# arnold117/PrimeKG-RGCN-LinkPrediction

Hardware: AMD Instinct MI355X
Metric: edges/sec per RGCN layer (fwd+bwd), PrimeKG 30.9k nodes/849k edges/3 rels (higher is better)
Workload: dtype f32; 1 GPU; C2: PrimeKG-shaped synthetic graph, 30926 nodes / 849456 edge columns / 3 relations, encoder 64->128->128, 2 layers fwd+bwd, full graph per step, dropout 0; parallelism=1 GPU, launch=hipGraph replay

## Files before the change

### primekg_rgcn_linkprediction_amd/_lib.py

```python
from __future__ import annotations

import ctypes
import os
from ctypes import c_double, c_float, POINTER, c_char_p, c_int, c_int64, c_size_t, c_void_p

import torch

ABI_VERSION = 38
LIB_NAME = "librgcn_hip.so"
LIB_PATH = os.path.join(os.path.dirname(os.path.abspath(__file__)), LIB_NAME)

RGCN_OK = 0
RGCN_ERR_ARG = -1
RGCN_ERR_RANGE = -2
RGCN_ERR_HIP = -3
RGCN_ERR_UNSUPPORTED = -4
RGCN_ERR_WORKSPACE = -5
RGCN_ERR_ALIGN = -6

_P = c_void_p
_I64 = c_int64

class SlabJob(ctypes.Structure):
    _fields_ = [("slab", c_void_p), ("bias_part", c_void_p), ("splits", ctypes.c_int32), ("K1", ctypes.c_int32),
# ... 126 lines not shown

CLUSTER_PROTOTYPES = {
    "rgcn_kmeans_workspace_bytes": (c_size_t, [_I64, _I64, _I64, _I64]),
    "rgcn_kmeans_assign": (c_int, [_P, _I64, _I64, _P, _I64, _I64,
                                   _P, _P, _P, _P, _P, c_size_t, _P]),
    "rgcn_kmeans_update": (c_int, [_P, _I64, _I64, _P, _I64, _I64,
                                   _P, _P, _P, _P, _P, _P, c_float, _P, c_size_t, _P]),
    "rgcn_kmeans_inertia": (c_int, [_P, _I64, _I64, _P, _I64, _I64, _P, _P, _P, c_size_t, _P]),
    "rgcn_silhouette_workspace_bytes": (c_size_t, [_I64, _I64, _I64, _I64]),
    "rgcn_silhouette_samples": (c_int, [_P, _P, _P, _P, _P, _P, _I64, _I64, _I64, _I64, _I64, _P, _P, _P, c_size_t, _P]),
}

TSNE_PROTOTYPES = {
    "rgcn_knn_refine": (c_int, [_P, _I64, _I64, _P, _I64, _P, _P, _P]),
    "rgcn_tsne_affinities": (c_int, [_P, _I64, _I64, c_double, _P, _P, _P]),
    "rgcn_tsne_workspace_bytes": (c_size_t, [_I64, _I64]),
    "rgcn_tsne_gradient": (c_int, [_P, _I64, _P, _P, _P, _I64, c_float, _I64, c_int,
                                   _P, _P, _P, _P, c_size_t, _P]),
    "rgcn_tsne_update": (c_int, [_P, _I64, c_float, c_float, c_float, _P, _P, _P, _P, _P, c_size_t, _P]),
}

NEIGHBORHOOD_PROTOTYPES = {
    "rgcn_neighborhood_max_nodes": (_I64, []),
    "rgcn_pair_neighborhood": (c_int, [_P, _P, _P, _P, _I64, _I64,
                                       _P, _P, _I64, c_int,
                                       _P, c_int, c_int,
                                       _P, _P, _P, _P, _P, _P, _P, _P]),
}

TRANSE_PROTOTYPES = {
    "rgcn_transe_step_workspace_bytes": (c_size_t, [_I64, _I64, _I64]),
    "rgcn_transe_step": (c_int, [_P, _I64, _P, _I64, _I64,
                                 _P, _P, _P, _I64, c_float, c_float,
                                 _P, _P, _P, _P, c_size_t, _P]),
}

RESAMPLE_PROTOTYPES = {
    "rgcn_resample_weights": (c_int, [_I64, _I64, _I64, _P, _P]),
    "rgcn_resample_curves": (c_int, [_P, _P, _P, _I64, _I64, _I64, _I64, _I64,
                                     _P, _P, _P, _P, _P, _P, _P]),
    "rgcn_resample_ranks": (c_int, [_P, _P, _I64, _P, c_int, _I64, _I64, _I64,
                                    _P, _P, _P, _P, _P]),
}
RESAMPLE_TILE = 1024
RESAMPLE_MAX_SAMPLES = 1 << 28
RESAMPLE_MAX_REPLICATES = 65535
RESAMPLE_MAX_K = 8

COMPLEX_PROTOTYPES = {
    "complex_fwd": (c_int, [_P, _P, _I64, _P, _P, _I64, _P, _P, _I64, _I64, _I64, _P, _P]),
    "complex_bce_fwd": (c_int, [_P, _P, _I64, _P, _P, _I64, _P, _P, _I64, _P, _I64, _I64, _P, _P, _P]),
    "complex_bwd_workspace_bytes": (c_size_t, [_I64, _I64, _I64]),
    "complex_bwd": (c_int, [_P, _P, _P, _I64, _P, _P, _I64, _P, _P, _I64, _I64, _I64, _P, _P, _P, _P, c_size_t, c_int, _P]),
    "complex_bce_bwd": (c_int, [_P, _P, _P, _P, _P, _I64, _P, _P, _I64, _P, _P, _I64, _I64, _I64, _P, _P, _P, _P,
                                c_size_t, c_int, _P]),
    "rgcn_complex_query": (c_int, [c_int, _P, _P, _I64, _P, _P, _I64, _I64, _I64, _P, _P]),
}

SOFTMAX_PROTOTYPES = {
    "rgcn_softmax_workspace_bytes": (c_size_t, [_I64, _I64, _I64, _I64]),
    "rgcn_softmax_lse": (c_int, [_P, _P, _P, _P, _P, _I64, _P, _I64, _I64, _I64, _I64,
                                 _P, _P, _P, _P, _P, _P, c_size_t, _P]),
    "rgcn_softmax_grad": (c_int, [_P, _P, _P, _P, _P, _P, _I64, _P, _P, _I64, _I64, _I64, _I64,
                                  _P, _P, c_int, _P, c_size_t, _P]),
}
SOFTMAX_MAX_D = 256

EDGE_DROPOUT_PROTOTYPES = {
    "rgcn_edge_dropout_create": (c_int, [c_void_p, _P, POINTER(c_void_p)]),
    "rgcn_edge_dropout_destroy": (None, [c_void_p]),
    "rgcn_edge_dropout_graph": (c_void_p, [c_void_p]),
    "rgcn_edge_dropout_kept": (c_void_p, [c_void_p]),
    "rgcn_edge_dropout_kept_export": (c_int, [c_void_p, _P, _P]),
    "rgcn_edge_dropout_draw": (c_int, [c_void_p, c_double, _P, _P, _I64, _P, _P, _P]),
}
EDGE_DROPOUT_STREAM = 0x45444F50

SPARSE_PROTOTYPES = {
    "rgcn_graph_row_mask": (c_void_p, [c_void_p, c_int, POINTER(c_int64)]),
    "rgcn_occupancy_host": (_I64, [_P, _I64, _I64, _P, POINTER(c_int64)]),
}
MODE_SPARSE_ROWS = 2

_lib = None


class RGCNLibraryError(RuntimeError):
    """The HIP library is missing / unloadable / of the wrong ABI."""


def load() -> ctypes.CDLL:
    global _lib
    if _lib is not None:
        return _lib
    if not os.path.exists(LIB_PATH):
        raise RGCNLibraryError(
            f"{LIB_PATH} not found: build it with `python -c 'import __graft_entry__ as g; "
            f"g.build()'` (or `make -C primekg_rgcn_linkprediction_amd/csrc`). There is no "
            f"CPU/PyTorch fallback for the R-GCN path.")
    try:
        lib = ctypes.CDLL(LIB_PATH, mode=ctypes.RTLD_GLOBAL)
    except OSError as exc:
        raise RGCNLibraryError(f"cannot load {LIB_PATH}: {exc}") from exc
    for name, (restype, argtypes) in list(PROTOTYPES.items()) + list(SAMPLING_PROTOTYPES.items()) + list(PATHS_PROTOTYPES.items()) + list(CLUSTER_PROTOTYPES.items()) + list(TSNE_PROTOTYPES.items()) + list(NEIGHBORHOOD_PROTOTYPES.items()) + list(TRANSE_PROTOTYPES.items()) + list(RESAMPLE_PROTOTYPES.items()) + list(COMPLEX_PROTOTYPES.items()) + list(SPARSE_PROTOTYPES.items()) + list(SOFTMAX_PROTOTYPES.items()) + list(EDGE_DROPOUT_PROTOTYPES.items()):
        try:
            fn = getattr(lib, name)
        except AttributeError as exc:
            raise RGCNLibraryError(f"{LIB_PATH} does not export {name}") from exc
        fn.restype = restype
        fn.argtypes = argtypes
    got = lib.rgcn_abi_version()
    if got != ABI_VERSION:
        raise RGCNLibraryError(f"{LIB_PATH} has ABI version {got}, host code expects {ABI_VERSION}")
    _lib = lib
    return lib


def available() -> bool:
    try:
        load()
        return True
    except RGCNLibraryError:
        return False


def strerror(code: int) -> str:
    return load().rgcn_strerror(code).decode()


def check(code: int, what: str) -> None:
    if code == RGCN_OK:
        return
    msg = f"{what}: {strerror(code)} (code {code})"
    if code == RGCN_ERR_RANGE:
        raise IndexError(msg)
    if code in (RGCN_ERR_ARG, RGCN_ERR_UNSUPPORTED):
        raise ValueError(msg)
    if code == RGCN_ERR_ALIGN:
        raise ValueError(f"{what}: a tensor's base address is not aligned: {strerror(code)} (code {code}). Every tensor "
                         f"torch allocates qualifies, and so do row slices of a table whose width is a multiple of 4; a "
                         f"view that starts some elements into a flat buffer does not - pass tensor.clone()")
    raise RuntimeError(msg)
```

### primekg_rgcn_linkprediction_amd/conv.py

```python
from __future__ import annotations

import math
from typing import Optional, Tuple, Union

import torch
import torch.nn as nn
from torch import Tensor

from . import ops


def _glorot(t: Optional[Tensor]) -> None:
    if t is not None:
        bound = math.sqrt(6.0 / (t.size(-2) + t.size(-1)))
        with torch.no_grad():
            t.uniform_(-bound, bound)


def _table(x: Tensor, gather_dtype) -> Tensor:
    if gather_dtype in (None, torch.float32):
        return x
    ops.guard_torch_op("fp16 copy of the feature table")
    return x.to(gather_dtype)


class _BasisCompose(torch.autograd.Function):

    @staticmethod
    def forward(ctx, comp: Tensor, basis: Tensor) -> Tensor:
        comp, basis = comp.contiguous(), basis.contiguous()
        ctx.save_for_backward(comp, basis)
        return ops.basis_compose(comp, basis)

    @staticmethod
    def backward(ctx, gw: Tensor):
        comp, basis = ctx.saved_tensors
        return ops.basis_compose_bwd(gw.contiguous(), comp, basis, ctx.needs_input_grad[0], ctx.needs_input_grad[1])


class _Scales:

    def __init__(self, t: Tensor, slots: int = 2, layers=(), given=None):
        self._own, self._next, self.first = None, 0, None
        self.packed = [None] * len(layers)
        if ops.GEMM_PRECISION == "split":
            if given is not None:
                self.first = given[0]
                if slots > 1:
                    self._own = ops._empty(slots - 1, ops.AMAX_FLOATS, dtype=torch.float32, device=t.device)
                self.packed = ops.split_weights_many(list(layers), amax=list(given[1]), clear=self._own)
                return
            buf = ops._empty(slots, ops.AMAX_FLOATS, dtype=torch.float32, device=t.device)
            self.first, self._own = buf[0], buf[1:slots]
            if layers:
                self.packed = ops.absmax_and_split(t, self.first, self._own, list(layers))
            else:
                ops.absmax(t, self.first, self._own)

    def slot(self) -> Optional[Tensor]:
        if self._own is None:
            return None
        self._next += 1
        return self._own[self._next - 1]


import os as _os
_TRANSFORM_FIRST_RATIO = 2.0


def _fused_backward(graph, g, r, d_in, d_out, g_amax, packed, precision) -> bool:
    fused = _TRAIN_FUSED == "1" or (_TRAIN_FUSED == "auto" and g.size(0) * r * d_out * 4 >= _TRAIN_FUSED_MIN_BYTES)
    return (fused and precision is None and packed is not None and g_amax is not None and not graph.bipartite
            and not graph.edge_dropout
            and ops.GEMM_PRECISION == "split" and ops.fused_bwd_supported(r, d_in, d_out))


def _from_packed(weight: Tensor, packed, precision) -> bool:
    return packed is not None and ops.GEMM_PRECISION == "split" and precision is None and weight.size(2) % 32 == 0


def _transform_first(graph: "ops.BucketedGraph", weight: Tensor, root: Optional[Tensor], packed, precision) -> bool:
    r, d_in, d_out = weight.shape
    ratio = _TRANSFORM_FIRST_RATIO if _from_packed(weight, packed, precision) else max(_TRANSFORM_FIRST_RATIO, 4.0)
    return d_out >= ratio * d_in and root is not None and not graph.bipartite and not graph.edge_dropout


_SPARSE_AGG = True


def _sparse_agg(graph: "ops.BucketedGraph", transposed: bool, half: bool, packed, amax, d: int, precision=None) -> bool:
    return bool(_SPARSE_AGG and not half and packed is not None and amax is not None and ops.GEMM_PRECISION == "split"
                and precision in (None, "half") and d % 64 == 0 and d <= 256 and not graph.bipartite
                and not graph.weighted_shard and graph.num_relations <= 32
                and graph.row_mask_ptr(transposed) is not None)


def _gagg_scale(graph: "ops.BucketedGraph", gagg_amax: Optional[Tensor], g_amax: Optional[Tensor]):
    if gagg_amax is not None:
        return (gagg_amax, g_amax), 1.0
    return (g_amax, g_amax), graph.weight_bound(True)


def _input_grad(graph: "ops.BucketedGraph", g: Tensor, weight: Tensor, root: Optional[Tensor],
                tail: Optional["ops.PendingParamGrads"] = None, g_amax: Optional[Tensor] = None,
                scales: Optional[_Scales] = None, packed: Optional["ops.SplitWeights"] = None,
                precision: Optional[str] = None, t_first: Optional[Tensor] = None, *,
                relu_mask: Optional[Tensor] = None, out_scale: float = 1.0, amax_out: Optional[Tensor] = None,
                lower=None):
    r, d_in, d_out = weight.shape
    extras = relu_mask is not None or amax_out is not None or out_scale != 1.0
    merged = (graph.merged_transposed()
              if not extras and _transform_first(graph, weight, root, packed, precision) else None)
    t = None
    if merged is not None:
        if t_first is None and _from_packed(weight, packed, precision):
            t_first = ops.transform_first(g.contiguous(), packed, g_amax)
        elif t_first is None:
            ops.guard_torch_op("weight concatenation of the transform-first input gradient")
            wcat = torch.cat([weight.reshape(r * d_in, d_out), root]).view(1, (r + 1) * d_in, d_out)
            t_first = ops.transform_bwd_input(g, g, wcat, None, amax=(g_amax, None), precision=precision)
        gx = ops.aggregate(merged, t_first.view(-1, d_in), tail=tail)
    else:
        gagg_amax = scales.slot() if scales is not None else None
        if _fused_backward(graph, g, r, d_in, d_out, g_amax, packed, precision):
            gx = ops.layer_bwd_input_fused(graph, g, packed, relu_mask, g_amax, amax_out=amax_out, tail=tail,
                                           inline_limit=_EVAL_INLINE_LIMIT, out_scale=out_scale, gagg_amax=gagg_amax)
        else:
            sparse = gagg_amax is not None and _sparse_agg(graph, True, False, packed, g_amax, d_out, precision)
            if sparse:
                gagg = ops.aggregate_sparse(graph, g, transposed=True, tail=tail, amax_out=gagg_amax)[0]
            else:
                gagg = ops.aggregate(graph, g, transposed=True, tail=tail, amax_out=gagg_amax)
            amax, mul = _gagg_scale(graph, gagg_amax, g_amax)
            if (lower is not None and packed is not None and g_amax is not None
                    and _from_packed(lower[0], lower[2], precision) and _transform_first(graph, *lower, precision)
                    and ops.chain_supported(weight, lower[0])):
                gx, t = ops.transform_bwd_input_chain(gagg, g, weight, root, relu_mask, packed, lower[2], graph=graph,
                                                      amax=amax, amax_mul=mul, amax_out=amax_out, out_scale=out_scale,
                                                      sparse=sparse)
            else:
                gx = ops.transform_bwd_input(gagg, g, weight, root, relu_mask=relu_mask, graph=graph, amax=amax,
                                             amax_mul=mul, amax_out=amax_out, packed=packed, precision=precision,
                                             out_scale=out_scale, sparse=sparse)
    return (gx, t) if lower is not None else gx


def _backward_scales(g: Tensor, layers: int) -> _Scales:
    return _Scales(g, slots=2 * layers)


def _deferred_params(graph: "ops.BucketedGraph", agg, x, g, x_amax, g_amax, has_root: bool, has_bias: bool, prec,
                     packed=None):
    sparse = _sparse_agg(graph, False, False, packed, x_amax, x.size(1), prec)
    return ops.transform_bwd_params(agg, x, g, graph.num_relations, want_root=has_root, want_bias=has_bias, graph=graph,
                                    defer=True, amax=(x_amax, x_amax, g_amax), precision=prec, sparse=sparse,
                                    amax_mul=_agg_bound(graph))


_TRAIN_FUSED = _os.environ.get("RGCN_TRAIN_FUSED", "auto")
_TRAIN_FUSED_MIN_BYTES = 256 << 20


def _defer_hubs(half: bool, packed, amax, k: int, n_out: int, graph=None) -> bool:
    return (_DEFER_HUBS and not half and packed is not None and amax is not None and ops.GEMM_PRECISION == "split"
            and k in (64, 128) and n_out <= 128 and not (graph is not None and graph.edge_dropout))


_DEFER_HUBS = True


def _agg_bound(graph: "ops.BucketedGraph") -> float:
    return graph.weight_bound(False) if graph.edge_dropout else 1.0


def _train_fused(graph, n, r, d_in, d_out, half) -> bool:
    fused = _TRAIN_FUSED == "1" or (_TRAIN_FUSED == "auto" and n * r * d_in * 4 >= _TRAIN_FUSED_MIN_BYTES)
    return bool(fused and not half and not graph.weighted_shard and n == graph.num_other_nodes
                and ops.GEMM_PRECISION == "split" and ops.fused_supported(r, d_in, d_out))


def _layer_train_forward(graph: "ops.BucketedGraph", x: Tensor, gather_dtype, weight, root, bias, relu: bool,
                         half: bool, x_amax, amax_out, packed):
    n, r, d_in, d_out = x.size(0), graph.num_relations, x.size(1), weight.size(2)
    if (_train_fused(graph, n, r, d_in, d_out, half) and packed is not None and x_amax is not None):
        agg = ops._empty(n, r * d_in, dtype=torch.float32, device=x.device)
        out = ops.layer_fwd_fused(graph, x, packed, bias, relu, x_amax, amax_out, inline_limit=_EVAL_INLINE_LIMIT,
                                  agg_out=agg)
        return agg, out
    sparse = n == graph.num_other_nodes and _sparse_agg(graph, False, half, packed, x_amax, d_in)
    if sparse:
        agg, hubs = ops.aggregate_sparse(graph, x, defer=_defer_hubs(half, packed, x_amax, d_in, d_out, graph))
    elif _defer_hubs(half, packed, x_amax, d_in, d_out, graph):
        agg, hubs = ops.aggregate_deferred(graph, x)
    else:
        agg, hubs = ops.aggregate(graph, _table(x, gather_dtype)), None
    out = ops.transform_fwd(agg, x, weight, root, bias, relu=relu, graph=graph, half=half, amax=(x_amax, x_amax),
                            amax_out=amax_out, packed=packed, hubs=hubs, sparse=sparse, amax_mul=_agg_bound(graph))
    return agg, out


def _packs(bufs, layers):
    return [ops.SplitWeights(b, w, root) if b is not None else None for b, (w, root) in zip(bufs, layers)]


def _conv_forward(x, weight, root, bias, *, graph, relu, gather_dtype, half):
    scales = _Scales(x, slots=1, layers=[(weight, root)])
    x_amax = scales.first
    packed = scales.packed[0]
    agg, out = _layer_train_forward(graph, x, gather_dtype, weight, root, bias, relu, half, x_amax, None,
                                    packed)
    return out, agg, x_amax, (packed.buf if packed is not None else None)


def _conv_backward(x, agg, weight, root, x_amax, pkbuf, g, *, graph, has_root, has_bias, need_x, need_p, prec):
    packed = _packs([pkbuf], [(weight, root)])[0]
    scales = _backward_scales(g, 1)
    pending = (_deferred_params(graph, agg, x, g, x_amax, scales.first, has_root, has_bias, prec, packed)
               if need_p else None)
    gx = _input_grad(graph, g, weight, root, pending, scales.first, scales, packed, prec) if need_x else None
    if pending is None:
        return gx, None, None, None
    pending.finish()
    return (gx, *pending.grads)


_R_CONV_FORWARD = ops.Region("conv.forward", _conv_forward)
_R_CONV_BACKWARD = ops.Region("conv.backward", _conv_backward)


def _contiguous(*tensors):
    return tuple(t.contiguous() if t is not None else None for t in tensors)


def _bwd_precision(gather_dtype, half_backward: bool) -> Optional[str]:
    return "half" if (gather_dtype == torch.float16 and half_backward and ops.GEMM_PRECISION == "split") else None


class _RGCNConvFunction(torch.autograd.Function):

    @staticmethod
    def forward(ctx, x: Tensor, weight: Tensor, root: Optional[Tensor], bias: Optional[Tensor],
                graph: ops.BucketedGraph, relu: bool = False, gather_dtype=None, half_backward: bool = False) -> Tensor:
        x, weight, root, bias = _contiguous(x, weight, root, bias)
        ctx.bwd_precision = _bwd_precision(gather_dtype, half_backward)
        key = (tuple(x.shape), tuple(weight.shape), root is not None, bias is not None, gather_dtype, bool(relu),
               _policy_key())
        out, agg, x_amax, pkbuf = _R_CONV_FORWARD.run(graph, key, (x, weight, root, bias),
                                                      dict(graph=graph, relu=relu, gather_dtype=gather_dtype,
                                                           half=gather_dtype == torch.float16), want={0})
        ctx.graph, ctx.relu, ctx.key = graph, relu, key
        ctx.has_root, ctx.has_bias = root is not None, bias is not None
        ctx.save_for_backward(x, weight, root, out if relu else None)
        ctx.kept = (agg, x_amax, pkbuf)
        return out

    @staticmethod
    def backward(ctx, g: Tensor):
        x, weight, root, out = ctx.saved_tensors
        agg, x_amax, pkbuf = ctx.kept
        if ctx.relu:
            g = g * (out > 0)
        g = g.contiguous()
        need_x, need_w, need_root, need_bias = ctx.needs_input_grad[:4]
        need_p = bool(need_w or (need_root and ctx.has_root) or (need_bias and ctx.has_bias))
        static = dict(graph=ctx.graph, has_root=ctx.has_root, has_bias=ctx.has_bias, need_x=bool(need_x), need_p=need_p,
                      prec=ctx.bwd_precision)
        gx, gw, groot, gbias = _R_CONV_BACKWARD.run(ctx.graph, (ctx.key, bool(need_x), need_p, ctx.bwd_precision),
                                                    (x, agg, weight, root, x_amax, pkbuf, g), static,
                                                    want={0, 1, 2, 3})
        return gx, gw, groot, gbias, None, None, None, None


def _enc2_layer1(x, w1, root1, b1, w2, root2, xa=None, w1a=None, r1a=None, w2a=None, r2a=None, *, graph, gather_dtype, half):
    given = (xa, [(w1a, r1a), (w2a, r2a)]) if xa is not None else None
    scales = _Scales(x, layers=[(w1, root1), (w2, root2)], given=given)
    x_amax, h_amax = scales.first, scales.slot()
    pk1, pk2 = scales.packed
    agg1, h = _layer_train_forward(graph, x, gather_dtype, w1, root1, b1, True, half, x_amax, h_amax, pk1)
    return h, agg1, x_amax, h_amax, (pk1.buf if pk1 is not None else None), (pk2.buf if pk2 is not None else None)


def _enc2_layer2(h, w2, root2, b2, h_amax, pk2buf, *, graph, gather_dtype, half):
    pk2 = _packs([pk2buf], [(w2, root2)])[0]
    agg2, out = _layer_train_forward(graph, h, gather_dtype, w2, root2, b2, False, half, h_amax, None, pk2)
    return out, agg2


def _enc2_forward(x, w1, root1, b1, w2, root2, b2, xa=None, w1a=None, r1a=None, w2a=None, r2a=None, *, graph, gather_dtype,
                  half):
    h, agg1, x_amax, h_amax, pk1buf, pk2buf = _enc2_layer1(x, w1, root1, b1, w2, root2, xa, w1a, r1a, w2a, r2a, graph=graph,
                                                           gather_dtype=gather_dtype, half=half)
    out, agg2 = _enc2_layer2(h, w2, root2, b2, h_amax, pk2buf, graph=graph, gather_dtype=gather_dtype, half=half)
    return out, h, agg1, agg2, x_amax, h_amax, pk1buf, pk2buf


def _enc2_backward(x, agg1, h, agg2, w1, root1, w2, root2, x_amax, h_amax, pk1buf, pk2buf, g, *, graph, flags, p,
                   prec, need_x):
    has_root1, has_b1, has_root2, has_b2 = flags
    pk1, pk2 = _packs([pk1buf, pk2buf], [(w1, root1), (w2, root2)])
    scales = _backward_scales(g, 2)
    g_amax, gz_amax = scales.first, scales.slot()
    red2 = _deferred_params(graph, agg2, h, g, h_amax, g_amax, has_root2, has_b2, prec, pk2)
    gz = _input_grad(graph, g, w2, root2, red2, g_amax, scales, pk2, prec, relu_mask=h,
                     out_scale=1.0 / (1.0 - p) if p > 0 else 1.0, amax_out=gz_amax,
                     lower=(w1, root1, pk1) if need_x else None)
    gz, t_first = gz if need_x else (gz, None)
    red1 = _deferred_params(graph, agg1, x, gz, x_amax, gz_amax, has_root1, has_b1, prec, pk1)
    gx = _input_grad(graph, gz, w1, root1, red1, gz_amax, scales, pk1, prec, t_first) if need_x else None
    red2.finish()
    red1.finish()
    return (gx, *red1.grads, *red2.grads)


_R_LAYER1 = ops.Region("encoder2.layer1", _enc2_layer1)
_R_LAYER2 = ops.Region("encoder2.layer2", _enc2_layer2)
_R_FORWARD = ops.Region("encoder2.forward", _enc2_forward)
_R_BACKWARD = ops.Region("encoder2.backward", _enc2_backward)


def _policy_key():
    return (_TRAIN_FUSED, _DEFER_HUBS, _TRANSFORM_FIRST_RATIO, _EVAL_INLINE_LIMIT, _TRAIN_FUSED_MIN_BYTES, _SPARSE_AGG)


def _enc2_train_forward(graph, params, gather_dtype, half_backward: bool, hints, p: float = 0.0):
    x, w1, root1, b1, w2, root2, b2 = params = _contiguous(*params)
    hinted = hints is not None and ops.GEMM_PRECISION == "split"
    hint_list = list(hints) if hinted else []
    key = (tuple(x.shape), tuple(w1.shape), tuple(w2.shape), root1 is not None, b1 is not None, root2 is not None,
           b2 is not None, gather_dtype, hinted, _policy_key())
    static = dict(graph=graph, gather_dtype=gather_dtype, half=gather_dtype == torch.float16)
    if p > 0:
        h, agg1, x_amax, h_amax, pk1buf, pk2buf = _R_LAYER1.run(graph, key, [x, w1, root1, b1, w2, root2] + hint_list,
                                                                static, want={0, 3})
        h = torch.native_dropout(h, p, True)[0]
        h_amax = ops.materialize(h_amax) * (1.0 / (1.0 - p)) if h_amax is not None else None
        out, agg2 = _R_LAYER2.run(graph, key, (h, w2, root2, b2, h_amax, pk2buf), static, want={0})
    else:
        out, h, agg1, agg2, x_amax, h_amax, pk1buf, pk2buf = _R_FORWARD.run(graph, key, list(params) + hint_list, static,
                                                                            want={0})
    flags = (root1 is not None, b1 is not None, root2 is not None, b2 is not None)
    kept = (agg1, h, agg2, x_amax, h_amax, pk1buf, pk2buf)
    return out, params, (graph, key, flags, p, _bwd_precision(gather_dtype, half_backward), kept)


def _enc2_train_backward(state, inputs, g: Tensor, need_x: bool):
    graph, key, flags, p, prec, (agg1, h, agg2, x_amax, h_amax, pk1buf, pk2buf) = state
    x, w1, root1, w2, root2 = inputs
    return _R_BACKWARD.run(graph, (key, p, need_x, prec),
                           (x, agg1, h, agg2, w1, root1, w2, root2, x_amax, h_amax, pk1buf, pk2buf, g.contiguous()),
                           dict(graph=graph, flags=flags, p=p, prec=prec, need_x=need_x), want={0, 1, 2, 3, 4, 5, 6})


class _Encoder2Function(torch.autograd.Function):

    @staticmethod
    def forward(ctx, x, w1, root1, b1, w2, root2, b2, graph, gather_dtype=None, p: float = 0.0,
                half_backward: bool = False, hints=None):
        out, (x, w1, root1, _, w2, root2, _), ctx.state = _enc2_train_forward(
            graph, (x, w1, root1, b1, w2, root2, b2), gather_dtype, half_backward, hints, p)
        ctx.save_for_backward(x, w1, root1, w2, root2)
        return out

    @staticmethod
    def backward(ctx, g):
        grads = _enc2_train_backward(ctx.state, ctx.saved_tensors, g, bool(ctx.needs_input_grad[0]))
        return (*grads, None, None, None, None, None)


_EVAL_BLOCK_BYTES = 1 << 30


_EVAL_FUSED = _os.environ.get("RGCN_EVAL_FUSED", "auto")


def _eval_fused(n: int, r: int, d_in: int) -> bool:
    if _EVAL_FUSED in (True, "1"):
        return True
    if _EVAL_FUSED in (False, "0"):
        return False
    return n * r * d_in * 4 >= _TRAIN_FUSED_MIN_BYTES
_EVAL_INLINE_LIMIT = 16


def _layer_eval_blocked(graph: "ops.BucketedGraph", x: Tensor, table: Tensor, weight: Tensor, root, bias, relu: bool,
                        half: bool, amax, amax_out, packed) -> Tensor:
    n, r, d_in, d_out = x.size(0), graph.num_relations, x.size(1), weight.size(2)
    if (_eval_fused(n, r, d_in) and not half and packed is not None and amax[1] is not None and not graph.weighted_shard
            and x.size(0) == graph.num_other_nodes and ops.fused_supported(r, d_in, d_out)):
        return ops.layer_fwd_fused(graph, x, packed, bias, relu, amax[1], amax_out, inline_limit=_EVAL_INLINE_LIMIT)
    rows = max(32, _EVAL_BLOCK_BYTES // max(1, r * d_in * 4))
    out = ops._empty(n, d_out, dtype=torch.float32, device=x.device)
    if rows >= n:
        agg = ops.aggregate(graph, table)
        return ops.transform_fwd(agg, x, weight, root, bias, relu=relu, graph=graph, half=half, amax=amax,
                                 amax_out=amax_out, packed=packed, out=out)
    blocks = graph.row_blocks(rows)
    buf = ops._empty(blocks[0][1] - blocks[0][0], r * d_in, dtype=torch.float32, device=x.device)
    for lo, hi, shard in blocks:
        agg = ops.aggregate(shard, table, out=buf[: hi - lo])
        ops.transform_fwd(agg, x[lo:hi], weight, root, bias, relu=relu, graph=shard, half=half, amax=amax,
                          amax_out=amax_out, packed=packed, out=out[lo:hi])
    return out


# ... 203 lines not shown
```

### primekg_rgcn_linkprediction_amd/csrc/rgcn_common.h

```cpp
#pragma once
#include <hip/hip_runtime.h>
#include <stddef.h>
#include <stdint.h>
#include "../../include/rgcn_hip.h"
#include "rgcn_plan.h"

#define RGCN_HIP_TRY(expr)                       \
  do {                                           \
    hipError_t err__ = (expr);                   \
    if (err__ != hipSuccess) return RGCN_ERR_HIP; \
  } while (0)

template <class... P>
static inline bool rgcn_aligned(uintptr_t a, P... p) {
  uintptr_t bits = 0;
  ((bits |= (uintptr_t)(const void*)p), ...);
  return (bits & (a - 1)) == 0;
}
#define RGCN_ALIGN_TRY(a, ...)                                       \
  do {                                                               \
    if (!rgcn_aligned((a), __VA_ARGS__)) return RGCN_ERR_ALIGN;      \
  } while (0)

constexpr int kCUs = 256;

static inline size_t align256(size_t n) { return (n + 255) & ~(size_t)255; }

struct rgcn_slicing {
  int tiles_per_slice, slices;
};
static inline rgcn_slicing rgcn_slice_tiles(int64_t tiles, int64_t want, int64_t cap) {
  const int64_t most = tiles < cap ? tiles : cap;
  want = want < most ? want : most;
  want = want > 1 ? want : 1;
  const int64_t per = (tiles + want - 1) / want;
  return {(int)per, (int)((tiles + per - 1) / per)};
}

template <class K>
static inline int raise_lds(K kernel, int bytes, bool (&raised)[64]) {
  int dev = 0;
  RGCN_HIP_TRY(hipGetDevice(&dev));
  if (dev < 0 || dev >= 64 || !raised[dev]) {
    RGCN_HIP_TRY(hipFuncSetAttribute(reinterpret_cast<const void*>(kernel), hipFuncAttributeMaxDynamicSharedMemorySize, bytes));
    if (dev >= 0 && dev < 64) raised[dev] = true;
  }
  return RGCN_OK;
}

static inline int rgcn_zero_param_grads(float* grad_weight, float* grad_root, float* grad_bias, int64_t R, int64_t d_in,
                                        int64_t d_out, hipStream_t stream) {
  RGCN_HIP_TRY(hipMemsetAsync(grad_weight, 0, (size_t)(R * d_in) * d_out * sizeof(float), stream));
  if (grad_root) RGCN_HIP_TRY(hipMemsetAsync(grad_root, 0, (size_t)d_in * d_out * sizeof(float), stream));
  if (grad_bias) RGCN_HIP_TRY(hipMemsetAsync(grad_bias, 0, (size_t)d_out * sizeof(float), stream));
  return RGCN_OK;
}

constexpr int RGCN_HEAD = 8;

struct rgcn_csr {
  int32_t* rowptr = nullptr;
  int32_t* col = nullptr;
  int64_t* perm = nullptr;
  float* val = nullptr;
  bool weighted = false;
  int64_t n_key = 0;
  int64_t n_other = 0;
  int num_levels = 0;
  int32_t empty_items0 = 0;
  rgcn_item* items[RGCN_MAX_LEVELS] = {};
  int64_t num_items[RGCN_MAX_LEVELS] = {};
  int64_t num_partials = 0;
  int32_t* head_col = nullptr;
  float* head_w = nullptr;
  uint32_t* tile_mask = nullptr;
  int64_t num_row_tiles = 0;
  int32_t* fin_ptr = nullptr;
  int64_t num_fin_tiles = 0;
  float weight_bound = 1.f;
};

static_assert(offsetof(rgcn_csr, items) == offsetof(rgcn_csr, num_levels) + 8, "empty_items0 sits behind num_levels");

constexpr int64_t RGCN_ROW_MASK_PAD = 96;
static inline int64_t rgcn_row_mask_offset(int64_t n_key) { return ((n_key + 31) / 32 + 3) / 4 * 4; }
static inline int64_t rgcn_occupancy_words(int64_t n_key) { return rgcn_row_mask_offset(n_key) + n_key + RGCN_ROW_MASK_PAD; }
static inline void rgcn_fill_occupancy(const int32_t* rowptr, int64_t n_key, int64_t R, uint32_t* words) {
  const int64_t off = rgcn_row_mask_offset(n_key), total = rgcn_occupancy_words(n_key);
  for (int64_t i = 0; i < total; ++i) words[i] = 0u;
  for (int64_t i = 0; i < n_key; ++i) {
    uint32_t m = 0u;
    for (int64_t r = 0; r < R; ++r)
      if (rowptr[i * R + r + 1] > rowptr[i * R + r]) m |= 1u << r;
    words[off + i] = m;
    words[i >> 5] |= m;
  }
}

struct rgcn_graph {
  int64_t E = 0, N = 0, R = 0;
  rgcn_csr dir[2];
};

__attribute__((visibility("hidden"))) int* rgcn_index_error_flag();

constexpr int RGCN_AMAX_SLOTS = 64, RGCN_AMAX_STRIDE = 32;
constexpr int RGCN_AMAX_HEADS = 256, RGCN_AMAX_HEAD_STRIDE = 8;
static_assert(RGCN_AMAX_SLOTS * RGCN_AMAX_STRIDE == RGCN_AMAX_FLOATS, "amax buffer layout (include/rgcn_hip.h)");
static_assert(RGCN_AMAX_HEADS * RGCN_AMAX_HEAD_STRIDE == RGCN_AMAX_FLOATS && RGCN_AMAX_STRIDE % RGCN_AMAX_HEAD_STRIDE == 0,
              "amax buffer layout");

#if defined(__HIPCC__)
__device__ inline int64_t clamp64(int64_t v, int64_t lo, int64_t hi) { return v < lo ? lo : (v > hi ? hi : v); }
__device__ inline int lane_int(int v, int src) { return __builtin_amdgcn_readfirstlane(__shfl(v, src)); }
__device__ inline float lane_float(float v, int src) { return __int_as_float(lane_int(__float_as_int(v), src)); }
__device__ inline int64_t lane_i64(int64_t v, int src) {
  const unsigned lo = (unsigned)lane_int((int)(unsigned)(v & 0xffffffffll), src);
  const int hi = lane_int((int)(v >> 32), src);
  return ((int64_t)hi << 32) | (int64_t)lo;
}
__device__ inline float rgcn_relu(float v) {
  const float r = fmaxf(v, 0.f);
  return v != v ? v : r;
}
extern "C" __device__ unsigned __ockl_wfred_max_u32(unsigned);
__device__ inline unsigned rgcn_amax_peek(const unsigned* __restrict__ amax) {
  return amax ? amax[(blockIdx.x & (RGCN_AMAX_SLOTS - 1)) * RGCN_AMAX_STRIDE] : 0u;
}
__device__ inline void rgcn_amax_publish(unsigned* __restrict__ amax, float lane_max, unsigned seen = 0u) {
  const unsigned m = __ockl_wfred_max_u32(__float_as_uint(fmaxf(lane_max, 0.f)));
  if (m <= seen) return;
  unsigned* slot = amax + (blockIdx.x & (RGCN_AMAX_SLOTS - 1)) * RGCN_AMAX_STRIDE;
  const unsigned long long act = __ballot(1);
  if ((int)(threadIdx.x & 63) == __ffsll((long long)act) - 1) atomicMax(slot, m);
}
__device__ inline float rgcn_amax_value(const float* __restrict__ amax, int lane) {
  float v[RGCN_AMAX_HEADS / 64];
#pragma unroll
  for (int j = 0; j < RGCN_AMAX_HEADS / 64; ++j) v[j] = amax[(lane + 64 * j) * RGCN_AMAX_HEAD_STRIDE];
  float m = v[0];
#pragma unroll
  for (int j = 1; j < RGCN_AMAX_HEADS / 64; ++j) m = fmaxf(m, v[j]);
#pragma unroll
  for (int o = 32; o > 0; o >>= 1) m = fmaxf(m, __shfl_xor(m, o));
  return m;
}
__device__ inline float rgcn_partials_max(const float* __restrict__ p, int count, int lane) {
  float v[4];
#pragma unroll
  for (int j = 0; j < 4; ++j) v[j] = (lane + 64 * j < count) ? p[lane + 64 * j] : 0.f;
  float m = fmaxf(fmaxf(v[0], v[1]), fmaxf(v[2], v[3]));
#pragma unroll
  for (int o = 32; o > 0; o >>= 1) m = fmaxf(m, __shfl_xor(m, o));
  return m;
}
#endif
```

### primekg_rgcn_linkprediction_amd/csrc/rgcn_graph.hip

```cpp
#include <hipcub/hipcub.hpp>

#include <algorithm>
#include <cmath>
#include <new>
#include <vector>

#include "rgcn_common.h"
#include "../../include/rgcn_sparse.h"

namespace {

constexpr int kThreads = 256;

__global__ void k_validate(const int64_t* __restrict__ key_node, const int64_t* __restrict__ other_node,
                           const int64_t* __restrict__ edge_type, int64_t E, int64_t n_key, int64_t n_other,
                           int64_t R, int* __restrict__ flag) {
  int64_t e = (int64_t)blockIdx.x * blockDim.x + threadIdx.x;
  if (e >= E) return;
  int64_t k = key_node[e], o = other_node[e], t = edge_type[e];
  if (k < 0 || k >= n_key || o < 0 || o >= n_other || t < 0 || t >= R) atomicOr(flag, 1);
}

__global__ void k_make_keys(const int64_t* __restrict__ key_node, const int64_t* __restrict__ edge_type,
                            int64_t E, int64_t R, uint32_t* __restrict__ keys, uint32_t* __restrict__ ids) {
  int64_t e = (int64_t)blockIdx.x * blockDim.x + threadIdx.x;
  if (e >= E) return;
  keys[e] = (uint32_t)(key_node[e] * R + edge_type[e]);
  ids[e] = (uint32_t)e;
}

__global__ void k_rowptr(const uint32_t* __restrict__ skeys, int64_t E, int64_t NR,
                         int32_t* __restrict__ rowptr) {
  int64_t e = (int64_t)blockIdx.x * blockDim.x + threadIdx.x;
  if (e > E) return;
  int64_t lo = (e == 0) ? 0 : (int64_t)skeys[e - 1] + 1;
  int64_t hi = (e == E) ? NR : (int64_t)skeys[e];
  for (int64_t k = lo; k <= hi; ++k) rowptr[k] = (int32_t)e;
}

__global__ void k_fill_edges(const int64_t* __restrict__ other_node, int64_t E,
                             const uint32_t* __restrict__ sids, int32_t* __restrict__ col,
                             int64_t* __restrict__ perm) {
  int64_t e = (int64_t)blockIdx.x * blockDim.x + threadIdx.x;
  if (e >= E) return;
  uint32_t p = sids[e];
  perm[e] = (int64_t)p;
  col[e] = (int32_t)other_node[p];
}

__global__ void k_counts(const int32_t* __restrict__ rowptr, int64_t NR, float* __restrict__ cnt) {
  int64_t s = (int64_t)blockIdx.x * blockDim.x + threadIdx.x;
  if (s >= NR) return;
  int deg = rowptr[s + 1] - rowptr[s];
  cnt[s] = (float)(deg < 1 ? 1 : deg);
}

__global__ void k_edge_weights(const uint32_t* __restrict__ skeys_t, const int32_t* __restrict__ col_t,
                               const float* __restrict__ cnt, int64_t E, int64_t R,
                               float* __restrict__ w) {
  int64_t e = (int64_t)blockIdx.x * blockDim.x + threadIdx.x;
  if (e >= E) return;
  int64_t rel = (int64_t)(skeys_t[e] % (uint32_t)R);
  w[e] = 1.0f / cnt[(int64_t)col_t[e] * R + rel];
}

__global__ void k_permute_weights(const float* __restrict__ w_in, const int64_t* __restrict__ perm, int64_t E,
                                  float* __restrict__ w) {
  int64_t e = (int64_t)blockIdx.x * blockDim.x + threadIdx.x;
  if (e < E) w[e] = w_in[perm[e]];
}

inline unsigned grid_for(int64_t n) { return (unsigned)std::max<int64_t>(1, ceil_div64(n, kThreads)); }

int build_plan(const std::vector<int32_t>& rowptr, int64_t NR, int64_t R, rgcn_csr* csr) {
  rgcn_plan plan;
  const int rc = rgcn_build_plan(rowptr, NR, R, csr->n_key, &plan);
  if (rc != RGCN_OK) return rc;
  std::vector<std::vector<rgcn_item>>& levels = plan.levels;
  const std::vector<int32_t>& fin_ptr = plan.fin_ptr;
  const int64_t partial_rows = plan.num_partials;

  csr->num_levels = (int)levels.size();
  csr->num_partials = partial_rows;
  csr->empty_items0 = 0;
  if (!levels.empty()) {
    const std::vector<rgcn_item>& v0 = levels[0];
    size_t live = v0.size();
    while (live > 0 && !(v0[live - 1].flags & RGCN_ITEM_PACK) && v0[live - 1].begin == v0[live - 1].end) --live;
    csr->empty_items0 = (int32_t)(v0.size() - live);
  }
  for (int l = 0; l < csr->num_levels; ++l) {
    auto& v = levels[l];
    csr->num_items[l] = (int64_t)v.size();
    if (v.empty()) continue;
    RGCN_HIP_TRY(hipMalloc((void**)&csr->items[l], v.size() * sizeof(rgcn_item)));
    RGCN_HIP_TRY(hipMemcpy(csr->items[l], v.data(), v.size() * sizeof(rgcn_item), hipMemcpyHostToDevice));
  }
  if (!fin_ptr.empty()) {
    RGCN_HIP_TRY(hipMalloc((void**)&csr->fin_ptr, fin_ptr.size() * sizeof(int32_t)));
    RGCN_HIP_TRY(hipMemcpy(csr->fin_ptr, fin_ptr.data(), fin_ptr.size() * sizeof(int32_t), hipMemcpyHostToDevice));
    csr->num_fin_tiles = (int64_t)fin_ptr.size() - 1;
  }
  return RGCN_OK;
}

void free_csr(rgcn_csr* c) {
  (void)hipFree(c->rowptr);
  (void)hipFree(c->col);
  (void)hipFree(c->perm);
  (void)hipFree(c->val);
  (void)hipFree(c->tile_mask);
  (void)hipFree(c->fin_ptr);
  (void)hipFree(c->head_col);
  (void)hipFree(c->head_w);
  for (int l = 0; l < RGCN_MAX_LEVELS; ++l) (void)hipFree(c->items[l]);
  *c = rgcn_csr();
}

struct Scratch {
  uint32_t *keys = nullptr, *ids = nullptr, *skeys[2] = {nullptr, nullptr}, *sids = nullptr;
  void* sort_tmp = nullptr;
  size_t sort_tmp_bytes = 0;
  int* flag = nullptr;
  int alloc(int64_t E) {
    RGCN_HIP_TRY(hipMalloc((void**)&flag, sizeof(int)));
    if (E <= 0) return RGCN_OK;
    RGCN_HIP_TRY(hipMalloc((void**)&keys, E * sizeof(uint32_t)));
    RGCN_HIP_TRY(hipMalloc((void**)&ids, E * sizeof(uint32_t)));
    RGCN_HIP_TRY(hipMalloc((void**)&skeys[0], E * sizeof(uint32_t)));
    RGCN_HIP_TRY(hipMalloc((void**)&skeys[1], E * sizeof(uint32_t)));
    RGCN_HIP_TRY(hipMalloc((void**)&sids, E * sizeof(uint32_t)));
    return RGCN_OK;
  }
  ~Scratch() {
    (void)hipFree(keys); (void)hipFree(ids); (void)hipFree(skeys[0]); (void)hipFree(skeys[1]);
    (void)hipFree(sids); (void)hipFree(sort_tmp); (void)hipFree(flag);
  }
};

int validate(const int64_t* key_node, const int64_t* other_node, const int64_t* edge_type, int64_t E, int64_t n_key,
             int64_t n_other, int64_t R, Scratch& sc, hipStream_t stream) {
  if (E <= 0) return RGCN_OK;
  RGCN_HIP_TRY(hipMemsetAsync(sc.flag, 0, sizeof(int), stream));
  k_validate<<<grid_for(E), kThreads, 0, stream>>>(key_node, other_node, edge_type, E, n_key, n_other, R, sc.flag);
  int host_flag = 0;
  RGCN_HIP_TRY(hipMemcpyAsync(&host_flag, sc.flag, sizeof(int), hipMemcpyDeviceToHost, stream));
  RGCN_HIP_TRY(hipStreamSynchronize(stream));
  return host_flag ? RGCN_ERR_RANGE : RGCN_OK;
}

int build_structure(const int64_t* key_node, const int64_t* other_node, const int64_t* edge_type, int64_t E,
                    int64_t n_key, int64_t n_other, int64_t R, int slot, Scratch& sc, hipStream_t stream,
                    rgcn_csr* c) {
  const int64_t NR = n_key * R;
  c->n_key = n_key;
  c->n_other = n_other;
  RGCN_HIP_TRY(hipMalloc((void**)&c->rowptr, (NR + 1) * sizeof(int32_t)));
  if (E <= 0) {
    RGCN_HIP_TRY(hipMemsetAsync(c->rowptr, 0, (NR + 1) * sizeof(int32_t), stream));
    return RGCN_OK;
  }
  int end_bit = 1;
  while (end_bit < 32 && ((int64_t)1 << end_bit) < NR) ++end_bit;
  RGCN_HIP_TRY(hipMalloc((void**)&c->col, E * sizeof(int32_t)));
  RGCN_HIP_TRY(hipMalloc((void**)&c->perm, E * sizeof(int64_t)));
  k_make_keys<<<grid_for(E), kThreads, 0, stream>>>(key_node, edge_type, E, R, sc.keys, sc.ids);
  size_t tmp_bytes = 0;
  RGCN_HIP_TRY(hipcub::DeviceRadixSort::SortPairs(nullptr, tmp_bytes, sc.keys, sc.skeys[slot], sc.ids, sc.sids,
                                                   (int)E, 0, end_bit, stream));
  if (tmp_bytes > sc.sort_tmp_bytes) {
    RGCN_HIP_TRY(hipStreamSynchronize(stream));
    (void)hipFree(sc.sort_tmp);
    sc.sort_tmp = nullptr;
    RGCN_HIP_TRY(hipMalloc(&sc.sort_tmp, tmp_bytes + 256));
    sc.sort_tmp_bytes = tmp_bytes;
  }
  RGCN_HIP_TRY(hipcub::DeviceRadixSort::SortPairs(sc.sort_tmp, tmp_bytes, sc.keys, sc.skeys[slot], sc.ids, sc.sids,
                                                   (int)E, 0, end_bit, stream));
  k_rowptr<<<grid_for(E + 1), kThreads, 0, stream>>>(sc.skeys[slot], E, NR, c->rowptr);
  k_fill_edges<<<grid_for(E), kThreads, 0, stream>>>(other_node, E, sc.sids, c->col, c->perm);
  return RGCN_OK;
}

#define TRY_PLAN(expr) do { int rc__ = (expr); if (rc__ != RGCN_OK) return rc__; } while (0)

__global__ void k_item_heads(const rgcn_item* __restrict__ items, int64_t nitems, const int32_t* __restrict__ col,
                             const float* __restrict__ w, int32_t* __restrict__ head_col,
                             float* __restrict__ head_w) {
  const int64_t i = (int64_t)blockIdx.x * blockDim.x + threadIdx.x;
  if (i >= nitems * RGCN_HEAD) return;
  const rgcn_item it = items[i / RGCN_HEAD];
  const int e = it.begin + (int)(i % RGCN_HEAD);
  const bool ok = e < it.end;
  head_col[i] = ok ? col[e] : -1;
  if (head_w) head_w[i] = ok ? w[e] : 0.f;
}

int plan_structure(rgcn_csr* c, int64_t R, hipStream_t stream) {
  const int64_t NR = c->n_key * R;
  std::vector<int32_t> rp((size_t)NR + 1);
  RGCN_HIP_TRY(hipMemcpyAsync(rp.data(), c->rowptr, (NR + 1) * sizeof(int32_t), hipMemcpyDeviceToHost, stream));
  RGCN_HIP_TRY(hipStreamSynchronize(stream));
  if (R <= 32 && c->n_key > 0) {
    c->num_row_tiles = ceil_div64(c->n_key, 32);
    std::vector<uint32_t> mask((size_t)rgcn_occupancy_words(c->n_key));
    rgcn_fill_occupancy(rp.data(), c->n_key, R, mask.data());
    RGCN_HIP_TRY(hipMalloc((void**)&c->tile_mask, mask.size() * sizeof(uint32_t)));
    RGCN_HIP_TRY(hipMemcpy(c->tile_mask, mask.data(), mask.size() * sizeof(uint32_t), hipMemcpyHostToDevice));
  }
  TRY_PLAN(build_plan(rp, NR, R, c));
  c->weight_bound = 1.f;
  if (c->weighted && NR > 0 && rp[(size_t)NR] > 0) {
    std::vector<float> w((size_t)rp[(size_t)NR]);
    RGCN_HIP_TRY(hipMemcpyAsync(w.data(), c->val, w.size() * sizeof(float), hipMemcpyDeviceToHost, stream));
    RGCN_HIP_TRY(hipStreamSynchronize(stream));
    double best = 0.0;
    for (int64_t s = 0; s < NR; ++s) {
      double sum = 0.0;
      for (int32_t e = rp[(size_t)s]; e < rp[(size_t)s + 1]; ++e) sum += std::fabs((double)w[(size_t)e]);
      best = std::max(best, sum);
    }
    c->weight_bound = (float)(best * (1.0 + 1e-6)) + 1e-30f;
  }
  const int64_t n0 = c->num_items[0];
  if (n0 > 0) {
    RGCN_HIP_TRY(hipMalloc((void**)&c->head_col, (size_t)n0 * RGCN_HEAD * sizeof(int32_t)));
    if (c->weighted) RGCN_HIP_TRY(hipMalloc((void**)&c->head_w, (size_t)n0 * RGCN_HEAD * sizeof(float)));
    k_item_heads<<<grid_for(n0 * RGCN_HEAD), kThreads, 0, stream>>>(c->items[0], n0, c->col,
                                                                   c->weighted ? c->val : nullptr, c->head_col,
                                                                   c->head_w);
    RGCN_HIP_TRY(hipGetLastError());
  }
  return RGCN_OK;
}

int mean_counts(rgcn_csr* c, int64_t R, hipStream_t stream) {
  const int64_t NR = c->n_key * R;
  RGCN_HIP_TRY(hipMalloc((void**)&c->val, std::max<int64_t>(NR, 1) * sizeof(float)));
  if (NR > 0) k_counts<<<grid_for(NR), kThreads, 0, stream>>>(c->rowptr, NR, c->val);
  c->weighted = false;
  return RGCN_OK;
}

#define TRY_RC(expr) do { int rc__ = (expr); if (rc__ != RGCN_OK) return rc__; } while (0)

int create_impl(const int64_t* edge_index, const int64_t* edge_type, int64_t E, int64_t N, int64_t R,
                hipStream_t stream, rgcn_graph* g) {
  g->E = E; g->N = N; g->R = R;
  const int64_t* src = edge_index;
  const int64_t* dst = edge_index + E;
  Scratch sc;
  TRY_RC(sc.alloc(E));
  TRY_RC(validate(dst, src, edge_type, E, N, N, R, sc, stream));
  TRY_RC(build_structure(dst, src, edge_type, E, N, N, R, 0, sc, stream, &g->dir[0]));
  TRY_RC(build_structure(src, dst, edge_type, E, N, N, R, 1, sc, stream, &g->dir[1]));
  TRY_RC(mean_counts(&g->dir[0], R, stream));
  g->dir[1].weighted = true;
  if (E > 0) {
    RGCN_HIP_TRY(hipMalloc((void**)&g->dir[1].val, E * sizeof(float)));
    k_edge_weights<<<grid_for(E), kThreads, 0, stream>>>(sc.skeys[1], g->dir[1].col, g->dir[0].val, E, R,
                                                         g->dir[1].val);
  }
  RGCN_HIP_TRY(hipGetLastError());
  TRY_RC(plan_structure(&g->dir[0], R, stream));
  TRY_RC(plan_structure(&g->dir[1], R, stream));
  RGCN_HIP_TRY(hipStreamSynchronize(stream));
  return RGCN_OK;
}

int create_bipartite_impl(const int64_t* key_node, const int64_t* other_node, const int64_t* edge_type, int64_t E,
                          int64_t n_key, int64_t n_other, int64_t R, const float* edge_weight, hipStream_t stream,
                          rgcn_graph* g) {
  g->E = E; g->N = n_key; g->R = R;
  Scratch sc;
  TRY_RC(sc.alloc(E));
  TRY_RC(validate(key_node, other_node, edge_type, E, n_key, n_other, R, sc, stream));
  rgcn_csr* c = &g->dir[0];
  TRY_RC(build_structure(key_node, other_node, edge_type, E, n_key, n_other, R, 0, sc, stream, c));
  if (edge_weight) {
    c->weighted = true;
    if (E > 0) {
      RGCN_HIP_TRY(hipMalloc((void**)&c->val, E * sizeof(float)));
      k_permute_weights<<<grid_for(E), kThreads, 0, stream>>>(edge_weight, c->perm, E, c->val);
    }
  } else {
    TRY_RC(mean_counts(c, R, stream));
  }
  RGCN_HIP_TRY(hipGetLastError());
  TRY_RC(plan_structure(c, R, stream));
  RGCN_HIP_TRY(hipStreamSynchronize(stream));
  return RGCN_OK;
}

// ... 106 lines not shown
}

int rgcn_graph_import(int64_t num_edges, int64_t num_nodes, int64_t num_relations, const int32_t* rowptr,
                      const int32_t* col, const int64_t* perm, const float* cnt, const int32_t* rowptr_t,
                      const int32_t* col_t, const int64_t* perm_t, const float* w_t, void* stream_,
                      rgcn_graph** out) {
  if (!out) return RGCN_ERR_ARG;
  *out = nullptr;
  if (num_edges < 0 || num_nodes < 0 || num_relations <= 0 || !rowptr || !rowptr_t) return RGCN_ERR_ARG;
  if (num_nodes * num_relations > 0 && !cnt) return RGCN_ERR_ARG;
  if (num_edges > 0 && (!col || !perm || !col_t || !perm_t || !w_t)) return RGCN_ERR_ARG;
  if (too_big(num_nodes, num_nodes, num_relations, num_edges)) return RGCN_ERR_UNSUPPORTED;
  RGCN_ALIGN_TRY(8, perm, perm_t);
  RGCN_ALIGN_TRY(4, rowptr, col, cnt, rowptr_t, col_t, w_t);
  hipStream_t stream = (hipStream_t)stream_;
  rgcn_graph* g = new (std::nothrow) rgcn_graph();
  if (!g) return RGCN_ERR_HIP;
  g->E = num_edges; g->N = num_nodes; g->R = num_relations;
  int* flag = nullptr;
  int rc = hipMalloc((void**)&flag, sizeof(int)) == hipSuccess ? RGCN_OK : RGCN_ERR_HIP;
  if (rc == RGCN_OK)
    rc = import_csr(rowptr, col, perm, cnt, false, num_edges, num_nodes, num_relations, flag, stream, &g->dir[0]);
  if (rc == RGCN_OK)
    rc = import_csr(rowptr_t, col_t, perm_t, w_t, true, num_edges, num_nodes, num_relations, flag, stream,
                    &g->dir[1]);
  if (rc == RGCN_OK && hipStreamSynchronize(stream) != hipSuccess) rc = RGCN_ERR_HIP;
  (void)hipFree(flag);
  if (rc != RGCN_OK) {
    rgcn_graph_destroy(g);
    return rc;
  }
  *out = g;
  return RGCN_OK;
}

void rgcn_graph_destroy(rgcn_graph* g) {
  if (!g) return;
  free_csr(&g->dir[0]);
  free_csr(&g->dir[1]);
  delete g;
}

int64_t rgcn_graph_num_edges(const rgcn_graph* g) { return g ? g->E : -1; }
int64_t rgcn_graph_num_nodes(const rgcn_graph* g) { return g ? g->N : -1; }
int64_t rgcn_graph_num_relations(const rgcn_graph* g) { return g ? g->R : -1; }
float rgcn_graph_weight_bound(const rgcn_graph* g, int transposed) {
  if (!g) return 0.f;
  const rgcn_csr* c = &g->dir[transposed ? 1 : 0];
  return c->rowptr ? c->weight_bound : 0.f;
}

int rgcn_graph_num_levels(const rgcn_graph* g, int transposed) {
  return g ? g->dir[transposed ? 1 : 0].num_levels : -1;
}

const uint32_t* rgcn_graph_tile_mask(const rgcn_graph* g, int transposed, int64_t* num_row_tiles) {
  if (!g) return nullptr;
  const rgcn_csr* c = &g->dir[transposed ? 1 : 0];
  if (num_row_tiles) *num_row_tiles = c->num_row_tiles;
  return c->tile_mask;
}

const uint32_t* rgcn_graph_row_mask(const rgcn_graph* g, int transposed, int64_t* num_rows) {
  if (num_rows) *num_rows = 0;
  if (!g) return nullptr;
  const rgcn_csr* c = &g->dir[transposed ? 1 : 0];
  if (!c->tile_mask) return nullptr;
  if (num_rows) *num_rows = c->n_key;
  return c->tile_mask + rgcn_row_mask_offset(c->n_key);
}

int64_t rgcn_occupancy_host(const int32_t* rowptr, int64_t num_rows, int64_t num_relations, uint32_t* words,
                            int64_t* row_offset) {
  if (num_rows < 0 || num_relations <= 0) return -1;
  if (row_offset) *row_offset = rgcn_row_mask_offset(num_rows);
  if (num_relations > 32) return 0;
  if (words) {
    if (!rowptr) return -1;
    rgcn_fill_occupancy(rowptr, num_rows, num_relations, words);
  }
  return rgcn_occupancy_words(num_rows);
}

int rgcn_graph_arrays(const rgcn_graph* g, int transposed, const int32_t** rowptr, const int32_t** col,
                      const int64_t** perm, const float** val) {
  if (!g) return RGCN_ERR_ARG;
  const rgcn_csr* c = &g->dir[transposed ? 1 : 0];
  if (rowptr) *rowptr = c->rowptr;
  if (col) *col = c->col;
  if (perm) *perm = c->perm;
  if (val) *val = c->val;
  return RGCN_OK;
}

int rgcn_graph_export(const rgcn_graph* g, int transposed, int32_t* rowptr, int32_t* col, int64_t* perm,
                      float* val, void* stream_) {
  if (!g) return RGCN_ERR_ARG;
  hipStream_t stream = (hipStream_t)stream_;
  const rgcn_csr* c = &g->dir[transposed ? 1 : 0];
  if (!c->rowptr) return RGCN_ERR_ARG;
  RGCN_ALIGN_TRY(8, perm);
  RGCN_ALIGN_TRY(4, rowptr, col, val);
  const size_t nr = (size_t)(c->n_key * g->R), e = (size_t)g->E;
  if (rowptr) RGCN_HIP_TRY(hipMemcpyAsync(rowptr, c->rowptr, (nr + 1) * sizeof(int32_t), hipMemcpyDeviceToDevice, stream));
  if (col && e) RGCN_HIP_TRY(hipMemcpyAsync(col, c->col, e * sizeof(int32_t), hipMemcpyDeviceToDevice, stream));
  if (perm && e) RGCN_HIP_TRY(hipMemcpyAsync(perm, c->perm, e * sizeof(int64_t), hipMemcpyDeviceToDevice, stream));
  const size_t nval = c->weighted ? e : nr;
  if (val && nval) RGCN_HIP_TRY(hipMemcpyAsync(val, c->val, nval * sizeof(float), hipMemcpyDeviceToDevice, stream));
  return RGCN_OK;
}

}
```

### primekg_rgcn_linkprediction_amd/csrc/rgcn_transform_split.hip

```cpp
#include <algorithm>
#include <cstdlib>
#include <type_traits>

#include <hip/hip_fp16.h>

#include "rgcn_common.h"
#include "rgcn_slab_reduce.h"
#include "rgcn_hub_finish.h"
#include "rgcn_split.h"
#include "rgcn_transform_host.h"

#ifdef RGCN_STAMPS
__device__ unsigned long long g_rgcn_stamps[8192 * 4];
#define RGCN_STAMP(i)                                                                                               \
  do {                                                                                                              \
    if (threadIdx.x == 0) g_rgcn_stamps[((blockIdx.y * gridDim.x + blockIdx.x) & 8191) * 4 + (i)] = __builtin_amdgcn_s_memrealtime(); \
  } while (0)
#else
#define RGCN_STAMP(i)
#endif

#include "rgcn_prep.h"


namespace {

typedef float float2v __attribute__((ext_vector_type(2)));
typedef _Float16 half2v __attribute__((ext_vector_type(2)));

constexpr int kThreads = 256;
constexpr int BK = 32;
constexpr int kMaxSlots = 256;

enum { EPI_NONE = 0, EPI_RELU = 1, EPI_MASK = 2 };
enum { B_KN = 0, B_BLK = 1 };

__device__ inline void glds16(const void* src, void* lds_wave_base) {
  __builtin_amdgcn_global_load_lds((const __attribute__((address_space(1))) void*)src,
                                   (__attribute__((address_space(3))) void*)lds_wave_base, 16, 0, 0);
}

constexpr int kAbsmaxSegs = 4;
struct absmax_job {
  const float* p[kAbsmaxSegs];
  int64_t n[kAbsmaxSegs];
};

__global__ __launch_bounds__(kThreads) void k_absmax(const absmax_job J, float* __restrict__ slots) {
  __shared__ float red[kThreads / 64];
  for (int seg = 0; seg < kAbsmaxSegs; ++seg) {
    float m = 0.f;
    const float* p = J.p[seg];
    if (!p) continue;
    const int64_t n = J.n[seg], n4 = n >> 2;
    const float4* p4 = reinterpret_cast<const float4*>(p);
    for (int64_t i = (int64_t)blockIdx.x * kThreads + threadIdx.x; i < n4; i += (int64_t)gridDim.x * kThreads) {
      const float4 v = p4[i];
      m = fmaxf(fmaxf(m, fmaxf(fabsf(v.x), fabsf(v.y))), fmaxf(fabsf(v.z), fabsf(v.w)));
    }
    if (blockIdx.x == 0 && threadIdx.x < (n & 3)) m = fmaxf(m, fabsf(p[n4 * 4 + threadIdx.x]));
#pragma unroll
    for (int o = 32; o > 0; o >>= 1) m = fmaxf(m, __shfl_xor(m, o));
    if ((threadIdx.x & 63) == 0) red[threadIdx.x >> 6] = m;
    __syncthreads();
    if (threadIdx.x == 0) slots[seg * kMaxSlots + blockIdx.x] = fmaxf(fmaxf(red[0], red[1]), fmaxf(red[2], red[3]));
    __syncthreads();
  }
}

struct amax_ref {
  const float* slots;
  int count;
};
__device__ inline float amax_of(const amax_ref& r, int lane) {
  return r.count == 0 ? rgcn_amax_value(r.slots, lane) : rgcn_partials_max(r.slots, r.count, lane);
}
struct amax_loads {
  float v[4];
};
__device__ inline amax_loads amax_request(const amax_ref& r, int lane) {
  amax_loads q;
  const int stride = r.count == 0 ? RGCN_AMAX_HEAD_STRIDE : 1, last = r.count == 0 ? RGCN_AMAX_HEADS - 1 : r.count - 1;
#pragma unroll
  for (int j = 0; j < 4; ++j) {
    const float* p = r.slots + min(lane + 64 * j, last) * stride;
    asm volatile("global_load_dword %0, %1, off" : "=v"(q.v[j]) : "v"(p) : "memory");
  }
  return q;
}
#define RGCN_AMAX_WAIT(a, b, c, younger)                                                                             \
  asm volatile("s_waitcnt vmcnt(%12)"                                                                                 \
               : "+v"(a.v[0]), "+v"(a.v[1]), "+v"(a.v[2]), "+v"(a.v[3]), "+v"(b.v[0]), "+v"(b.v[1]), "+v"(b.v[2]),     \
                 "+v"(b.v[3]), "+v"(c.v[0]), "+v"(c.v[1]), "+v"(c.v[2]), "+v"(c.v[3])                                  \
               : "n"(younger)                                                                                         \
               : "memory")
#define RGCN_AMAX_WAIT2(a, b, younger)                                                                                \
  asm volatile("s_waitcnt vmcnt(%8)"                                                                                  \
               : "+v"(a.v[0]), "+v"(a.v[1]), "+v"(a.v[2]), "+v"(a.v[3]), "+v"(b.v[0]), "+v"(b.v[1]), "+v"(b.v[2]),     \
                 "+v"(b.v[3])                                                                                         \
               : "n"(younger)                                                                                         \
               : "memory")
__device__ inline float amax_reduce(const amax_loads& q) {
  float m = fmaxf(fmaxf(q.v[0], q.v[1]), fmaxf(q.v[2], q.v[3]));
#pragma unroll
  for (int o = 32; o > 0; o >>= 1) m = fmaxf(m, __shfl_xor(m, o));
  return m;
}

#ifndef RGCN_PACK_THREADS
#define RGCN_PACK_THREADS 512
#endif
#ifndef RGCN_PACK_TILES
#define RGCN_PACK_TILES 1
#endif
#ifndef RGCN_SPLIT_THREADS
#define RGCN_SPLIT_THREADS 256
#endif
#ifndef RGCN_SCAN_THREADS
#define RGCN_SCAN_THREADS 1024
#endif
constexpr int kPackThreads = RGCN_PACK_THREADS, kSplitThreads = RGCN_SPLIT_THREADS, kScanThreads = RGCN_SCAN_THREADS;
constexpr int kPackTiles = RGCN_PACK_TILES;
constexpr int kPackJobs = RGCN_PACK_JOBS, kZeroMax = RGCN_PREP_ZERO_MAX;
constexpr int kPackCapScan = 64, kPackCapGiven = 256;
using pack_job = rgcn_pack_job;
using pack_jobs = rgcn_pack_jobs;

template <int THREADS, bool SCAN, int TILES>
__global__ __launch_bounds__(THREADS) void k_pack_split(const pack_jobs JJ, float* __restrict__ zero, int zero_count) {
  __shared__ __attribute__((aligned(16))) unsigned char lds[rgcn_pack_lds_bytes<TILES>()];
  if (blockIdx.y == 0)
    for (int z = (int)threadIdx.x; z < zero_count; z += THREADS)
      for (int h = (int)blockIdx.x; h < RGCN_AMAX_HEADS; h += (int)gridDim.x)
        zero[(size_t)z * RGCN_AMAX_FLOATS + h * RGCN_AMAX_HEAD_STRIDE] = 0.f;
  rgcn_pack_body<THREADS, SCAN, TILES>(JJ.j[blockIdx.y], lds, (int)blockIdx.x);
}

struct hub_fin {
  const int32_t* ptr;
  const rgcn_item* items;
  const float* cnt;
  float* partial;
  int d, tiles;
};

struct nt_chain {
  const __half* Ch;
  const __half* Cl;
  const float* c_inv_scale;
  float* T;
  int N2;
};

__device__ __attribute__((aligned(16))) float g_zero_row[128];

template <int WM, int WN, int TN, int EPI, bool LO, bool CHAIN = false>
__global__ __launch_bounds__(64 * WM * WN) void k_gemm_nt_split(const float* __restrict__ A1, int K1,
                                                            const float* __restrict__ A2, int K2,
                                                            const __half* __restrict__ Bh,
                                                            const __half* __restrict__ Bl,
                                                            const float* __restrict__ b_inv_scale,
                                                            amax_ref amax1, float a1_mul, amax_ref amax2,
                                                            const float* __restrict__ bias,
                                                            const float* __restrict__ mask, float* __restrict__ C,
                                                            int M, int N, const uint32_t* __restrict__ tile_mask,
                                                            int kseg, unsigned* __restrict__ amax_out,
                                                            const hub_fin fin, float out_scale, const nt_chain chain,
                                                            const uint32_t* __restrict__ row_mask) {
  static_assert(!CHAIN || (WM == 2 && WN == 2 && TN == 2 && LO), "the chained product is built for the 64 x 128 tile");
  constexpr int WAVES = WM * WN;
  constexpr int BM = 32 * WM, BN = 32 * TN * WN, NBUF = WM == 2 ? 3 : 4, D = NBUF - 1;
  constexpr int PARTS = LO ? 2 : 1;
  constexpr int A_BYTES = BM * BK * 4, B_BYTES = BN * BK * 2, BUF_BYTES = A_BYTES + PARTS * B_BYTES;
  constexpr int A_PW = BM / (8 * WAVES);
  constexpr int B_PW = BN / (16 * WAVES);
  constexpr int P = A_PW + PARTS * B_PW;
  static_assert(A_PW >= 1 && B_PW >= 1 && A_PW * 8 * WAVES == BM && B_PW * 16 * WAVES == BN, "tile / wave layout");
  __shared__ __attribute__((aligned(16))) char lds[NBUF * BUF_BYTES];

  const int K = K1 + K2;
  const int m0 = blockIdx.x * BM, n0 = blockIdx.y * BN;
  const int tid = threadIdx.x, lane = tid & 63;
  const int wave = __builtin_amdgcn_readfirstlane(tid >> 6);
  const int wm = wave / WN, wn = wave % WN;
  const int li = lane & 31, lh = lane >> 5;
  RGCN_STAMP(0);
  amax_loads q1 = amax_request(amax1, lane), q2 = amax_request(amax2.slots ? amax2 : amax1, lane);
  const unsigned seen = rgcn_amax_peek(amax_out);
  unsigned rel_mask = 0xffffffffu;
  if (tile_mask) {
    const int t32 = m0 >> 5;
    rel_mask = 0u;
#pragma unroll
    for (int q = 0; q < WM; ++q)
      if ((t32 + q) * 32 < M) rel_mask |= tile_mask[t32 + q];
    rel_mask = __builtin_amdgcn_readfirstlane(rel_mask);
  }
  int a_m[A_PW], a_c4[A_PW];
  unsigned a_rm[A_PW];
#pragma unroll
  for (int j = 0; j < A_PW; ++j) {
    const int row = (wave * A_PW + j) * 8 + (lane >> 3);
    a_m[j] = min(m0 + row, M - 1);
    a_c4[j] = ((lane & 7) ^ ((row >> 1) & 7)) * 4;
    a_rm[j] = row_mask ? row_mask[a_m[j]] : 0xffffffffu;
  }
  const float* a_zero = g_zero_row + (lane & 7) * 4;
  int fin_b = 0, fin_e = 0;
  if (WAVES == 4 && fin.ptr) {
    fin_b = fin.ptr[min(m0 >> 5, fin.tiles)];
    fin_e = fin.ptr[min((m0 >> 5) + WM, fin.tiles)];
  }
  RGCN_AMAX_WAIT2(q1, q2, 0);
  const float amax1_v = amax_reduce(q1) * a1_mul;
  const float amax2_v = amax2.slots ? amax_reduce(q2) : 0.f;

  if (WAVES == 4 && fin.ptr) {
    const int jb = __builtin_amdgcn_readfirstlane(fin_b), je = __builtin_amdgcn_readfirstlane(fin_e);
    if (je > jb) {
      float4* red = reinterpret_cast<float4*>(lds);
      float* agg = const_cast<float*>(A1);
      for (int j = jb; j < je; ++j) {
        float4* scratch = red + ((j - jb) & 1) * 256;
        const rgcn_item it = fin.items[j];
        if (fin.d == 64) rgcn_reduce_item<16>(it, fin.cnt, agg, fin.partial, 64, 0, scratch);
        else if (fin.d == 128) rgcn_reduce_item<32>(it, fin.cnt, agg, fin.partial, 128, 0, scratch);
        else rgcn_reduce_item<64>(it, fin.cnt, agg, fin.partial, 256, 0, scratch);
      }
      __threadfence_block();
      asm volatile("s_waitcnt vmcnt(0)" ::: "memory");
      __syncthreads();
    }
  }

  floatx16 acc[TN];
#pragma unroll
  for (int b = 0; b < TN; ++b)
#pragma unroll
    for (int r = 0; r < 16; ++r) acc[b][r] = 0.f;

  size_t b_off[B_PW];
#pragma unroll
  for (int j = 0; j < B_PW; ++j) {
    const int row = (wave * B_PW + j) * 16 + (lane >> 2);
    const int n = min(n0 + row, N - 1);
    const int chunk = (lane & 3) ^ ((row >> 1) & 3);
    b_off[j] = (size_t)n * K + chunk * 8;
  }

  auto stage = [&](int kt, int buf) {
    char* sA = lds + buf * BUF_BYTES;
    char* sBh = sA + A_BYTES;
    char* sBl = sBh + B_BYTES;
    const bool first = kt < K1;
    const float* abase = first ? A1 + kt : A2 + (kt - K1);
    const int lda = first ? K1 : K2;
    const bool masked = first && row_mask != nullptr;
    const unsigned rbit = masked ? 1u << (kt / kseg) : 0u;
#pragma unroll
    for (int j = 0; j < A_PW; ++j)
      glds16((!masked || (a_rm[j] & rbit)) ? abase + ((size_t)a_m[j] * lda + a_c4[j]) : a_zero, sA + (wave * A_PW + j) * 8 * BK * 4);
#pragma unroll
    for (int j = 0; j < B_PW; ++j) {
      glds16(Bh + kt + b_off[j], sBh + (wave * B_PW + j) * 16 * BK * 2);
      if (LO) glds16(Bl + kt + b_off[j], sBl + (wave * B_PW + j) * 16 * BK * 2);
    }
  };

  auto next_kt = [&](int kt) {
    kt += BK;
    while (kt < K1 && !((rel_mask >> (kt / kseg)) & 1u)) kt = (kt / kseg + 1) * kseg;
    return min(kt, K);
  };
  int ktq[D];
  ktq[0] = next_kt(-BK);
#pragma unroll
  for (int j = 1; j < D; ++j) ktq[j] = ktq[j - 1] < K ? next_kt(ktq[j - 1]) : K;
#pragma unroll
  for (int j = 0; j < D; ++j)
    if (ktq[j] < K) stage(ktq[j], j);

  const int ea1 = scale_exponent(amax1_v);
  const int ea2 = amax2.slots ? scale_exponent(amax2_v) : ea1;
  const float sa1 = pow2f(ea1), sa2 = pow2f(ea2);

  const int arow = wm * 32 + li;
  unsigned a_addr[2][2], b_addr[TN][2];
#pragma unroll
// ... 19 lines not shown
#pragma unroll
    for (int s = 0; s < 2; ++s) {
      asm volatile("ds_read_b128 %0, %1" : "=v"(fa[s][0]) : "v"(a_addr[s][0] + buf));
      asm volatile("ds_read_b128 %0, %1" : "=v"(fa[s][1]) : "v"(a_addr[s][1] + buf));
#pragma unroll
      for (int b = 0; b < TN; ++b) {
        asm volatile("ds_read_b128 %0, %1" : "=v"(fh[s][b]) : "v"(b_addr[b][s] + buf));
        if (LO) asm volatile("ds_read_b128 %0, %1 offset:%2" : "=v"(fl[s][b]) : "v"(b_addr[b][s] + buf), "n"(B_BYTES));
      }
    }
    const int kt_new = ktq[D - 1] < K ? next_kt(ktq[D - 1]) : K;
    if (kt_new < K) stage(kt_new, (t + D) % NBUF);
#pragma unroll
    for (int j = 0; j + 1 < D; ++j) ktq[j] = ktq[j + 1];
    ktq[D - 1] = kt_new;
    ++t;
#pragma unroll
    for (int s = 0; s < 2; ++s) {
      constexpr int kStepReads = 2 + PARTS * TN;
      if constexpr (TN == 4) {
        if (s == 0) asm volatile("s_waitcnt lgkmcnt(%6)" : "+v"(fa[0][0]), "+v"(fa[0][1]), "+v"(fh[0][0]), "+v"(fh[0][1]), "+v"(fh[0][2]), "+v"(fh[0][3]) : "n"(kStepReads));
        else asm volatile("s_waitcnt lgkmcnt(0)" : "+v"(fa[1][0]), "+v"(fa[1][1]), "+v"(fh[1][0]), "+v"(fh[1][1]), "+v"(fh[1][2]), "+v"(fh[1][3]));
        if (LO) asm volatile("" : "+v"(fl[s][0]), "+v"(fl[s][1]), "+v"(fl[s][2]), "+v"(fl[s][3]));
      } else if constexpr (TN > 1) {
        static_assert(TN <= 2 || TN == 4, "every fragment register must be tied to its wait");
        if (s == 0) asm volatile("s_waitcnt lgkmcnt(%4)" : "+v"(fa[0][0]), "+v"(fa[0][1]), "+v"(fh[0][0]), "+v"(fh[0][TN - 1]) : "n"(kStepReads));
        else asm volatile("s_waitcnt lgkmcnt(0)" : "+v"(fa[1][0]), "+v"(fa[1][1]), "+v"(fh[1][0]), "+v"(fh[1][TN - 1]));
        if (LO) asm volatile("" : "+v"(fl[s][0]), "+v"(fl[s][TN - 1]));
      } else {
        if (s == 0) asm volatile("s_waitcnt lgkmcnt(%3)" : "+v"(fa[0][0]), "+v"(fa[0][1]), "+v"(fh[0][0]) : "n"(kStepReads));
        else asm volatile("s_waitcnt lgkmcnt(0)" : "+v"(fa[1][0]), "+v"(fa[1][1]), "+v"(fh[1][0]));
        if (LO) asm volatile("" : "+v"(fl[s][0]));
      }
      half8 ah, al;
#pragma unroll
      for (int q = 0; q < 2; ++q)
#pragma unroll
        for (int c = 0; c < 4; ++c) {
          const float v = fa[s][q][c] * sa;
          const _Float16 h = (_Float16)v;
          ah[4 * q + c] = h;
          if (LO) al[4 * q + c] = (_Float16)(v - (float)h);
        }
      if (LO) {
#pragma unroll
        for (int b = 0; b < TN; ++b)
          acc[b] = __builtin_amdgcn_mfma_f32_32x32x16_f16(al, __builtin_bit_cast(half8, fh[s][b]), acc[b], 0, 0, 0);
#pragma unroll
        for (int b = 0; b < TN; ++b)
          acc[b] = __builtin_amdgcn_mfma_f32_32x32x16_f16(ah, __builtin_bit_cast(half8, fl[s][b]), acc[b], 0, 0, 0);
      }
#pragma unroll
      for (int b = 0; b < TN; ++b)
        acc[b] = __builtin_amdgcn_mfma_f32_32x32x16_f16(ah, __builtin_bit_cast(half8, fh[s][b]), acc[b], 0, 0, 0);
    }
  };
  RGCN_STAMP(1);
  while (ktq[0] < K1) k_tile(sa1);
  if (K2 > 0) {
    const float down = pow2f(-ea1);
#pragma unroll
    for (int b = 0; b < TN; ++b)
#pragma unroll
      for (int r = 0; r < 16; ++r) acc[b][r] = acc[b][r] * down * sa2;
    while (ktq[0] < K) k_tile(sa2);
  }

  RGCN_STAMP(2);
  const float ia = pow2f(K2 > 0 ? -ea2 : -ea1) * out_scale, ib = b_inv_scale[0];
  float cmax = 0.f;
  if constexpr (CHAIN) {
    constexpr int W = 64, RPR = 4, NV = 8;
    constexpr unsigned IMG = 40 * 1024, IMG_LO = IMG + 16 * 1024;
    static_assert(IMG_LO + 16 * 1024 <= NBUF * BUF_BYTES, "LDS budget of the chained product");
    __builtin_amdgcn_s_barrier();
    float* tr = reinterpret_cast<float*>(lds) + wave * (32 * W);
#pragma unroll
    for (int b = 0; b < TN; ++b)
#pragma unroll
      for (int r = 0; r < 16; ++r) tr[((r & 3) + 8 * (r >> 2) + 4 * lh) * W + b * 32 + li] = acc[b][r];
    const int trow = lane >> 4, tc4 = (lane & 15) * 4;
    const int nq = wn * W + tc4;
    float4 mk4[NV];
    if (EPI == EPI_MASK) {
#pragma unroll
      for (int q = 0; q < NV; ++q) {
        const int m = m0 + wm * 32 + q * RPR + trow;
        mk4[q] = m < M ? *reinterpret_cast<const float4*>(mask + (size_t)m * N + nq) : make_float4(0.f, 0.f, 0.f, 0.f);
      }
    }
#pragma unroll
    for (int q = 0; q < NV; ++q) {
      const int m = m0 + wm * 32 + q * RPR + trow;
      const float4 a = *reinterpret_cast<const float4*>(tr + (q * RPR + trow) * W + tc4);
      float4 v;
      v.x = a.x * ia * ib; v.y = a.y * ia * ib; v.z = a.z * ia * ib; v.w = a.w * ia * ib;
      if (EPI == EPI_MASK) {
        v.x = mk4[q].x > 0.f ? v.x : 0.f; v.y = mk4[q].y > 0.f ? v.y : 0.f;
        v.z = mk4[q].z > 0.f ? v.z : 0.f; v.w = mk4[q].w > 0.f ? v.w : 0.f;
      }
      if (m < M) *reinterpret_cast<float4*>(C + (size_t)m * N + nq) = v;
      else v = make_float4(0.f, 0.f, 0.f, 0.f);
      cmax = fmaxf(cmax, fmaxf(fmaxf(fabsf(v.x), fabsf(v.y)), fmaxf(fabsf(v.z), fabsf(v.w))));
      *reinterpret_cast<float4*>(tr + (q * RPR + trow) * W + tc4) = v;
    }
    float* wmax = reinterpret_cast<float*>(lds + 32 * 1024);
    {
      const unsigned mw = __ockl_wfred_max_u32(__float_as_uint(cmax));
      if (lane == 0) wmax[wave] = __uint_as_float(mw);
    }
    __syncthreads();
    const float tile_max = fmaxf(fmaxf(wmax[0], wmax[1]), fmaxf(wmax[2], wmax[3]));
    const int e2 = scale_exponent(tile_max);
    const float s2 = pow2f(e2);
#pragma unroll
    for (int q = 0; q < NV; ++q) {
      const int rl = wm * 32 + q * RPR + trow, col = wn * W + tc4;
      const float4 v = *reinterpret_cast<const float4*>(tr + (q * RPR + trow) * W + tc4);
      const float u[4] = {v.x * s2, v.y * s2, v.z * s2, v.w * s2};
      half4v h, l;
#pragma unroll
      for (int c = 0; c < 4; ++c) {
        const _Float16 hh = (_Float16)u[c];
        h[c] = hh;
        l[c] = (_Float16)(u[c] - (float)hh);
      }
      const unsigned at = (unsigned)(rl * 256 + ((((col >> 3) ^ (rl & 15)) << 4) | ((col & 4) << 1)));
      *reinterpret_cast<float2v*>(lds + IMG + at) = __builtin_bit_cast(float2v, h);
      *reinterpret_cast<float2v*>(lds + IMG_LO + at) = __builtin_bit_cast(float2v, l);
    }
    __syncthreads();
    const __half* __restrict__ Ch = chain.Ch;
    const __half* __restrict__ Cl = chain.Cl;
    const int N2 = chain.N2, KC = N;
    constexpr int SLOT2 = 2 * B_BYTES, NS2 = 4, D2 = NS2 - 1, P2 = 2 * B_PW, KT2 = 4;
    static_assert(NS2 * SLOT2 <= NBUF * BUF_BYTES, "B2 ring");
    f32x4 fah[8], fal[8];
#pragma unroll
    for (int ks = 0; ks < 8; ++ks) {
      const unsigned aa = (unsigned)(arow * 256 + (((2 * ks + lh) ^ (arow & 15)) << 4));
      asm volatile("ds_read_b128 %0, %1 offset:%2" : "=v"(fah[ks]) : "v"(aa), "n"(IMG));
      asm volatile("ds_read_b128 %0, %1 offset:%2" : "=v"(fal[ks]) : "v"(aa), "n"(IMG_LO));
    }
    asm volatile("s_waitcnt lgkmcnt(0)"
                 : "+v"(fah[0]), "+v"(fah[1]), "+v"(fah[2]), "+v"(fah[3]), "+v"(fah[4]), "+v"(fah[5]), "+v"(fah[6]), "+v"(fah[7]),
                   "+v"(fal[0]), "+v"(fal[1]), "+v"(fal[2]), "+v"(fal[3]), "+v"(fal[4]), "+v"(fal[5]), "+v"(fal[6]), "+v"(fal[7]));
    __builtin_amdgcn_s_barrier();
    const int col_blocks = (N2 + BN - 1) / BN, rounds = col_blocks * KT2;
    auto stage2 = [&](int r) {
      const int cb = r / KT2, kt = (r % KT2) * BK;
      char* dst = lds + (r % NS2) * SLOT2;
#pragma unroll
      for (int j = 0; j < B_PW; ++j) {
        const int row = (wave * B_PW + j) * 16 + (lane >> 2);
        const int n = min(cb * BN + row, N2 - 1);
        const int chunk = (lane & 3) ^ ((row >> 1) & 3);
        const size_t off = (size_t)n * KC + kt + chunk * 8;
        glds16(Ch + off, dst + (wave * B_PW + j) * 16 * BK * 2);
        glds16(Cl + off, dst + B_BYTES + (wave * B_PW + j) * 16 * BK * 2);
      }
    };
    unsigned b2_addr[TN][2];
#pragma unroll
    for (int s2i = 0; s2i < 2; ++s2i)
#pragma unroll
      for (int b = 0; b < TN; ++b) {
        const int brow = (wn * TN + b) * 32 + li;
        b2_addr[b][s2i] = (unsigned)(brow * BK * 2 + (((2 * s2i + lh) ^ ((brow >> 1) & 3)) << 4));
      }
    const float i2 = pow2f(-e2), ic = chain.c_inv_scale[0];
#pragma unroll
    for (int r = 0; r < D2; ++r)
      if (r < rounds) stage2(r);
    floatx16 acc2[TN];
#pragma unroll
    for (int b = 0; b < TN; ++b)
#pragma unroll
      for (int q = 0; q < 16; ++q) acc2[b][q] = 0.f;
    for (int cb2 = 0; cb2 < col_blocks; ++cb2)
#pragma unroll
    for (int kq = 0; kq < KT2; ++kq) {
      const int r = cb2 * KT2 + kq;
      if (r + 2 < rounds) asm volatile("s_waitcnt vmcnt(%0)" ::"n"(2 * P2) : "memory");
      else if (r + 1 < rounds) asm volatile("s_waitcnt vmcnt(%0)" ::"n"(P2) : "memory");
      else asm volatile("s_waitcnt vmcnt(0)" ::: "memory");
      __builtin_amdgcn_s_barrier();
      const unsigned slot = (unsigned)((r % NS2) * SLOT2);
      f32x4 fbh[2][TN], fbl[2][TN];
#pragma unroll
      for (int s2i = 0; s2i < 2; ++s2i)
#pragma unroll
        for (int b = 0; b < TN; ++b) {
          asm volatile("ds_read_b128 %0, %1" : "=v"(fbh[s2i][b]) : "v"(b2_addr[b][s2i] + slot));
          asm volatile("ds_read_b128 %0, %1 offset:%2" : "=v"(fbl[s2i][b]) : "v"(b2_addr[b][s2i] + slot), "n"(B_BYTES));
        }
      if (r + D2 < rounds) stage2(r + D2);
      asm volatile("s_waitcnt lgkmcnt(0)"
                   : "+v"(fbh[0][0]), "+v"(fbl[0][0]), "+v"(fbh[0][1]), "+v"(fbl[0][1]), "+v"(fbh[1][0]), "+v"(fbl[1][0]),
                     "+v"(fbh[1][1]), "+v"(fbl[1][1]));
#pragma unroll
      for (int s2i = 0; s2i < 2; ++s2i) {
        const half8 ah = __builtin_bit_cast(half8, fah[2 * kq + s2i]), al = __builtin_bit_cast(half8, fal[2 * kq + s2i]);
#pragma unroll
        for (int b = 0; b < TN; ++b)
          acc2[b] = __builtin_amdgcn_mfma_f32_32x32x16_f16(al, __builtin_bit_cast(half8, fbh[s2i][b]), acc2[b], 0, 0, 0);
#pragma unroll
        for (int b = 0; b < TN; ++b)
          acc2[b] = __builtin_amdgcn_mfma_f32_32x32x16_f16(ah, __builtin_bit_cast(half8, fbl[s2i][b]), acc2[b], 0, 0, 0);
#pragma unroll
        for (int b = 0; b < TN; ++b)
          acc2[b] = __builtin_amdgcn_mfma_f32_32x32x16_f16(ah, __builtin_bit_cast(half8, fbh[s2i][b]), acc2[b], 0, 0, 0);
      }
      if (kq == KT2 - 1) {
        const int cb = cb2;
#pragma unroll
        for (int b = 0; b < TN; ++b) {
          const int n = cb * BN + (wn * TN + b) * 32 + li;
#pragma unroll
          for (int q = 0; q < 16; ++q) {
            const int m = m0 + wm * 32 + (q & 3) + 8 * (q >> 2) + 4 * lh;
            if (m < M && n < N2) chain.T[(size_t)m * N2 + n] = acc2[b][q] * i2 * ic;
            acc2[b][q] = 0.f;
          }
        }
      }
    }
  } else if (m0 + BM <= M && n0 + BN <= N) {
    constexpr int W = 32 * TN;
    constexpr int RPR = 64 / (W / 4);
    constexpr int NV = 32 / RPR;
    __builtin_amdgcn_s_barrier();
    float* tr = reinterpret_cast<float*>(lds) + wave * (32 * W);
#pragma unroll
    for (int b = 0; b < TN; ++b)
#pragma unroll
      for (int r = 0; r < 16; ++r) tr[((r & 3) + 8 * (r >> 2) + 4 * lh) * W + b * 32 + li] = acc[b][r];
    const int trow = lane / (W / 4), tc4 = (lane % (W / 4)) * 4;
    const int nq = n0 + wn * W + tc4;
    float4 bv4 = make_float4(0.f, 0.f, 0.f, 0.f);
    if (bias) bv4 = *reinterpret_cast<const float4*>(bias + nq);
    float4 mk4[NV];
    if (EPI == EPI_MASK) {
#pragma unroll
      for (int q = 0; q < NV; ++q)
        mk4[q] = *reinterpret_cast<const float4*>(mask + (size_t)(m0 + wm * 32 + q * RPR + trow) * N + nq);
    }
#pragma unroll
    for (int q = 0; q < NV; ++q) {
      const float4 a = *reinterpret_cast<const float4*>(tr + (q * RPR + trow) * W + tc4);
      float4 v;
      v.x = a.x * ia * ib + bv4.x; v.y = a.y * ia * ib + bv4.y; v.z = a.z * ia * ib + bv4.z; v.w = a.w * ia * ib + bv4.w;
      if (EPI == EPI_RELU) { v.x = rgcn_relu(v.x); v.y = rgcn_relu(v.y); v.z = rgcn_relu(v.z); v.w = rgcn_relu(v.w); }
      if (EPI == EPI_MASK) {
        v.x = mk4[q].x > 0.f ? v.x : 0.f; v.y = mk4[q].y > 0.f ? v.y : 0.f;
        v.z = mk4[q].z > 0.f ? v.z : 0.f; v.w = mk4[q].w > 0.f ? v.w : 0.f;
      }
      cmax = fmaxf(cmax, fmaxf(fmaxf(fabsf(v.x), fabsf(v.y)), fmaxf(fabsf(v.z), fabsf(v.w))));
      *reinterpret_cast<float4*>(C + (size_t)(m0 + wm * 32 + q * RPR + trow) * N + nq) = v;
    }
  } else {
#pragma unroll
    for (int b = 0; b < TN; ++b) {
      const int n = n0 + (wn * TN + b) * 32 + li;
      if (n >= N) continue;
      const float bv = bias ? bias[n] : 0.f;
#pragma unroll
      for (int r = 0; r < 16; ++r) {
        const int m = m0 + wm * 32 + (r & 3) + 8 * (r >> 2) + 4 * lh;
        if (m < M) {
          float v = acc[b][r] * ia * ib + bv;
          if (EPI == EPI_RELU) v = rgcn_relu(v);
          if (EPI == EPI_MASK) v = mask[(size_t)m * N + n] > 0.f ? v : 0.f;
          cmax = fmaxf(cmax, fabsf(v));
          C[(size_t)m * N + n] = v;
        }
      }
    }
  }
  if (amax_out) rgcn_amax_publish(amax_out, cmax, seen);
#ifdef RGCN_STAMPS
  asm volatile("s_waitcnt vmcnt(0)" ::: "memory");
#endif
  RGCN_STAMP(3);
}

constexpr int kPrepTensors = RGCN_PREP_TENSORS;
using absmax_multi_job = rgcn_absmax_multi_job;
template <int THREADS, bool CLAMPED>
__device__ inline void absmax_body(const absmax_multi_job& J, float* __restrict__ zero, int zero_count, float* red,
                                   int bid, int nblocks) {
  rgcn_absmax_body<THREADS, CLAMPED>(J, zero, zero_count, red, bid, nblocks);
}

__global__ __launch_bounds__(kScanThreads) void k_absmax_multi(const absmax_multi_job J, float* __restrict__ zero,
                                                               int zero_count) {
  __shared__ float red[kScanThreads / 64];
  absmax_body<kScanThreads, false>(J, zero, zero_count, red, (int)blockIdx.x, (int)gridDim.x);
}

__global__ __launch_bounds__(kPackThreads) void k_absmax_pack(const absmax_multi_job J, float* __restrict__ zero,
                                                              int zero_count, const pack_jobs JJ, int pack_blocks,
                                                              int layers) {
  __shared__ __attribute__((aligned(16))) unsigned char lds[rgcn_pack_lds_bytes<kPackTiles>()];
  const int b = (int)blockIdx.x, npack = pack_blocks * layers;
  RGCN_STAMP(0);
  if (b < npack) rgcn_pack_body<kPackThreads, true, kPackTiles>(JJ.j[b / pack_blocks], lds, b % pack_blocks);
  else absmax_body<kPackThreads, true>(J, zero, zero_count, reinterpret_cast<float*>(lds), b - npack, RGCN_AMAX_HEADS);
#ifdef RGCN_STAMPS
  if (b >= npack) { RGCN_STAMP(1); RGCN_STAMP(2); }
  asm volatile("s_waitcnt vmcnt(0)" ::: "memory");
#endif
  RGCN_STAMP(3);
}

constexpr int TN_TKC = 128;
template <bool LO>
__global__ __launch_bounds__(2 * kThreads) void k_gemm_tn_coop(const float* __restrict__ A1, int K1,
                                                               const float* __restrict__ A2, int K2,
                                                               const float* __restrict__ G, int M, int N,
                                                               int n_tiles, int rows_per_split,
                                                               amax_ref amax1, float a1_mul, amax_ref amax2, amax_ref gmax,
                                                               float* __restrict__ slab,
                                                               float* __restrict__ bias_part,
                                                               const uint32_t* __restrict__ tile_mask, int kseg,
                                                               const uint32_t* __restrict__ row_mask) {
  constexpr int TKC = TN_TKC, RING = 3, A_FLOATS = 32 * TKC, G_FLOATS = 32 * 128;
  constexpr int SLOT_BYTES = (A_FLOATS + G_FLOATS) * 4;
  constexpr int PLANE = 4 * 128 * 16;
  constexpr int PBUF_BYTES = 4 * PLANE;
  constexpr int A_PW = 2, G_PW = 2, P = A_PW + G_PW;
  __shared__ __attribute__((aligned(16))) char lds[RING * SLOT_BYTES + 2 * PBUF_BYTES];
  const int Kc = K1 + K2;
  int bx = blockIdx.x, split = blockIdx.y;
  {
    const int gx = (int)gridDim.x, full = ((int)gridDim.y >> 3) << 3;
    const int lin = blockIdx.y * gx + blockIdx.x;
    if (lin < gx * full) {
      const int q = lin >> 3;
      bx = q % gx;
      split = (q / gx) * 8 + (lin & 7);
    }
  }
  const int kc_tile = bx / n_tiles, kc_tiles = (int)gridDim.x / n_tiles;
  const int kc0 = kc_tile * TKC, n0 = (bx % n_tiles) * 128;
  const int mbeg = split * rows_per_split;
  const int mend = min(M, mbeg + rows_per_split);
  const int tid = threadIdx.x, lane = tid & 63;
  const int wave = __builtin_amdgcn_readfirstlane(tid >> 6);
  const int wk = wave >> 1, wn = wave & 1;
  const int li = lane & 31, lh = lane >> 5;
  const bool bias_block = (bias_part != nullptr) && (kc_tile == (K2 > 0 ? kc_tiles - 1 : 0));
  const bool do_bias = bias_block && (tid < 128);
  RGCN_STAMP(0);
  amax_loads q1 = amax_request(amax1, lane), q2 = amax_request(amax2.slots ? amax2 : amax1, lane),
             qg = amax_request(gmax, lane);
  unsigned rel_bits = 0u;
  if (tile_mask != nullptr && !bias_block && kc0 + TKC <= K1)
// ... 224 lines not shown
};
size_t packed_bytes(int64_t R, int64_t d_in, int64_t d_out) {
  return 10 * align256((size_t)(R + 1) * d_in * d_out * sizeof(__half)) + 256 + 2 * kMaxSlots * sizeof(float);
}
PackedWeights packed_view(void* base, int64_t R, int64_t d_in, int64_t d_out) {
  const size_t img = align256((size_t)(R + 1) * d_in * d_out * sizeof(__half));
  char* p = (char*)base;
  PackedWeights v;
  v.Bh_f = (__half*)p;
  v.Bl_f = (__half*)(p + img);
  v.Bh_b = (__half*)(p + 2 * img);
  v.Bl_b = (__half*)(p + 3 * img);
  v.Fh_f = (__half*)(p + 4 * img);
  v.Fl_f = (__half*)(p + 5 * img);
  v.Fh_b = (__half*)(p + 6 * img);
  v.Fl_b = (__half*)(p + 7 * img);
  v.Bh_n = (__half*)(p + 8 * img);
  v.Bl_n = (__half*)(p + 9 * img);
  v.inv_scale = (float*)(p + 10 * img);
  v.partials = v.inv_scale + 64;
  return v;
}

pack_job make_pack_job(const float* weight, const float* root, int64_t R, int64_t d_in, int64_t d_out, void* packed,
                       const float* w_amax, const float* r_amax) {
  const PackedWeights v = packed_view(packed, R, d_in, d_out);
  pack_job j{};
  j.W = weight; j.Rt = root;
  j.R = (int)R; j.d_in = (int)d_in; j.d_out = (int)d_out;
  j.w_amax = w_amax; j.r_amax = root ? r_amax : nullptr;
  if (root && !r_amax) j.w_amax = nullptr;
  j.Bh_f = v.Bh_f; j.Bl_f = v.Bl_f; j.Bh_b = v.Bh_b; j.Bl_b = v.Bl_b;
  j.Fh_f = v.Fh_f; j.Fl_f = v.Fl_f; j.Fh_b = v.Fh_b; j.Fl_b = v.Fl_b;
  j.Bh_n = v.Bh_n; j.Bl_n = v.Bl_n;
  j.scale_out = v.inv_scale;
  return j;
}

int plan_pack_jobs(pack_jobs* JJ, int count, int threads, int tiles, int cap) {
  int most = 1;
  for (int l = 0; l < count; ++l) {
    rgcn_pack_plan(&JJ->j[l], threads, tiles, cap);
    most = std::max(most, JJ->j[l].nblocks);
  }
  return most;
}
void launch_pack_split(pack_jobs& JJ, int count, float* zero, int zero_count, hipStream_t stream) {
  bool given = true;
  for (int l = 0; l < count; ++l) given = given && JJ.j[l].w_amax;
  if (given) {
    const dim3 grid((unsigned)plan_pack_jobs(&JJ, count, kSplitThreads, 1, kPackCapGiven), (unsigned)count);
    k_pack_split<kSplitThreads, false, 1><<<grid, kSplitThreads, 0, stream>>>(JJ, zero, zero_count);
  } else {
    const dim3 grid((unsigned)plan_pack_jobs(&JJ, count, kPackThreads, kPackTiles, kPackCapScan), (unsigned)count);
    k_pack_split<kPackThreads, true, kPackTiles><<<grid, kPackThreads, 0, stream>>>(JJ, zero, zero_count);
  }
}

int pack_weights(const float* weight, const float* root, int64_t R, int64_t d_in, int64_t d_out, void* packed,
                 hipStream_t stream) {
  pack_jobs JJ{};
  JJ.j[0] = make_pack_job(weight, root, R, d_in, d_out, packed, nullptr, nullptr);
  launch_pack_split(JJ, 1, nullptr, 0, stream);
  RGCN_HIP_TRY(hipGetLastError());
  return RGCN_OK;
}

size_t nt_workspace_bytes(int64_t R, int64_t d_in, int64_t d_out) {
  return packed_bytes(R, d_in, d_out) + 2 * kMaxSlots * sizeof(float);
}

struct nt_call {
  const float *A1 = nullptr, *A2 = nullptr;
  int K1 = 0, K2 = 0;
  const __half *Bh = nullptr, *Bl = nullptr;
  const float* b_inv = nullptr;
  const float *bias = nullptr, *mask = nullptr;
  int epi = EPI_NONE;
  float* C = nullptr;
  int M = 0, N = 0;
  const uint32_t* tile_mask = nullptr;
  int kseg = 0;
  const uint32_t* row_mask = nullptr;
  const float *a1_amax = nullptr, *a2_amax = nullptr;
  float a1_mul = 1.f, out_scale = 1.f;
  float* c_amax = nullptr;
  float* scan_slots = nullptr;
  bool half = false;
  hub_fin fin{};
  bool chained = false;
  nt_chain chain{};
  hipStream_t stream = nullptr;
  amax_ref r1{}, r2{};
};

template <int TN, int EPI, bool LO, bool CHAIN>
void nt_launch(const nt_call& c) {
  const dim3 grid((unsigned)ceil_div64(c.M, 64), CHAIN ? 1u : (unsigned)ceil_div64(c.N, 64 * TN));
  k_gemm_nt_split<2, 2, TN, EPI, LO, CHAIN><<<grid, 256, 0, c.stream>>>(
      c.A1, c.K1, c.A2, c.K2, c.Bh, c.Bl, c.b_inv, c.r1, c.a1_mul, c.r2, c.bias, c.mask, c.C, c.M, c.N, c.tile_mask, c.kseg,
      reinterpret_cast<unsigned*>(c.c_amax), c.fin, c.out_scale, CHAIN ? c.chain : nt_chain{}, c.row_mask);
}

int launch_nt_split(nt_call c) {
  const nt_chain& chain = c.chain;
  if (c.chained && (c.half || c.N != 128 || c.bias || c.epi == EPI_RELU || !chain.Ch || !chain.Cl || !chain.c_inv_scale ||
                    !chain.T || chain.N2 <= 0 || (chain.N2 & 3)))
    return RGCN_ERR_UNSUPPORTED;
  const hub_fin& fin = c.fin;
  if (fin.ptr && fin.d != 64 && fin.d != 128 && fin.d != 256) return RGCN_ERR_UNSUPPORTED;
  if (fin.ptr && (!c.a1_amax || fin.d != c.kseg)) return RGCN_ERR_ARG;
  if (c.row_mask && (!c.a1_amax || c.kseg <= 0 || c.kseg % BK != 0)) return RGCN_ERR_ARG;
  const int K1 = c.K1, K2 = c.K2;
  if (K1 % BK || K2 % BK || K1 + K2 <= 0) return RGCN_ERR_UNSUPPORTED;
  const bool scan1 = K1 && !c.a1_amax, scan2 = K2 && !c.a2_amax;
  if (scan1 || scan2) {
    absmax_job J{};
    if (scan1) { J.p[0] = c.A1; J.n[0] = (int64_t)c.M * K1; }
    if (scan2) { J.p[1] = c.A2; J.n[1] = (int64_t)c.M * K2; }
    k_absmax<<<kMaxSlots, kThreads, 0, c.stream>>>(J, c.scan_slots);
  }
  c.r1 = !K1 ? amax_ref{nullptr, 0} : (scan1 ? amax_ref{c.scan_slots, kMaxSlots} : amax_ref{c.a1_amax, 0});
  c.r2 = !K2 ? amax_ref{nullptr, 0} : (scan2 ? amax_ref{c.scan_slots + kMaxSlots, kMaxSlots} : amax_ref{c.a2_amax, 0});
  if (scan1 || !(c.a1_mul > 0.f)) c.a1_mul = 1.f;
  if (!c.r1.slots) { c.r1 = c.r2; c.r2 = amax_ref{nullptr, 0}; c.a1_mul = 1.f; }
  if (c.kseg <= 0 || c.kseg % BK != 0) c.tile_mask = nullptr;
  auto with_epi = [&](auto launch) {
    if (c.epi == EPI_RELU) launch(std::integral_constant<int, EPI_RELU>{});
    else if (c.epi == EPI_MASK) launch(std::integral_constant<int, EPI_MASK>{});
    else launch(std::integral_constant<int, EPI_NONE>{});
  };
  auto plain = [&](auto tn) {
    with_epi([&](auto epi) {
      if (c.half) nt_launch<decltype(tn)::value, decltype(epi)::value, false, false>(c);
      else nt_launch<decltype(tn)::value, decltype(epi)::value, true, false>(c);
    });
  };
  if (c.chained)
    with_epi([&](auto epi) {
      if constexpr (decltype(epi)::value != EPI_RELU) nt_launch<2, decltype(epi)::value, true, true>(c);
    });
  else if (c.N <= 64) plain(std::integral_constant<int, 1>{});
  else plain(std::integral_constant<int, 2>{});
  RGCN_HIP_TRY(hipGetLastError());
  return RGCN_OK;
}

int make_hub_fin(const rgcn_graph* g, int transposed, float* partial, int64_t N, int64_t R, int64_t d, hub_fin* out) {
  *out = hub_fin{};
  if (!g) return 0;
  const rgcn_csr& c = g->dir[transposed ? 1 : 0];
  if (!c.rowptr || c.n_key != N || g->R != R) return RGCN_ERR_ARG;
  if (c.num_levels < 2) return 0;
  if (!c.fin_ptr || c.num_levels != 2 || !partial) return RGCN_ERR_ARG;
  out->ptr = c.fin_ptr;
  out->items = c.items[1];
  out->cnt = c.weighted ? nullptr : c.val;
  out->partial = partial;
  out->d = (int)d;
  out->tiles = (int)c.num_fin_tiles;
  return 1;
}

int nt_prepare(nt_call* c, PackedWeights* w, const float* weight, const float* root, const void* packed, int64_t N,
               int64_t R, int64_t d_in, int64_t d_out, int64_t dk, void* workspace, size_t workspace_bytes,
               const rgcn_graph* hub_graph, int hub_transposed, float* hub_partial, void* stream, bool operands_aligned) {
  if (!workspace || workspace_bytes < nt_workspace_bytes(R, d_in, d_out)) return RGCN_ERR_WORKSPACE;
  const int hrc = make_hub_fin(hub_graph, hub_transposed, hub_partial, N, R, dk, &c->fin);
  if (hrc < 0) return hrc;
  if (!operands_aligned || !rgcn_aligned(16, weight, root, packed, workspace, hub_partial)) return RGCN_ERR_ALIGN;
  c->stream = (hipStream_t)stream;
  if (!packed) {
    const int rc = pack_weights(weight, root, R, d_in, d_out, workspace, c->stream);
    if (rc != RGCN_OK) return rc;
    packed = workspace;
  }
  *w = packed_view(const_cast<void*>(packed), R, d_in, d_out);
  c->scan_slots = (float*)((char*)workspace + packed_bytes(R, d_in, d_out));
  c->K1 = (int)(R * dk);
  c->K2 = root ? (int)dk : 0;
  c->kseg = (int)dk;
  c->M = (int)N;
  return RGCN_OK;
}

constexpr int kTnBlocks = 256;
size_t tn_workspace_bytes(const rgcn_slab_layout& lay) {
  return align256(lay.bytes()) + kAbsmaxSegs * kMaxSlots * sizeof(float);
}

}

rgcn_split_frag_view rgcn_split_fragment_images(const void* packed, int64_t R, int64_t d_in, int64_t d_out) {
  const PackedWeights v = packed_view(const_cast<void*>(packed), R, d_in, d_out);
  return rgcn_split_frag_view{v.Fh_f, v.Fl_f, v.Fh_b, v.Fl_b, v.inv_scale};
}
size_t rgcn_split_packed_bytes(int64_t R, int64_t d_in, int64_t d_out) { return packed_bytes(R, d_in, d_out); }

int rgcn_prep_fill(const float* x, int64_t numel, float* x_amax, float* zero_buffers, int zero_count, int count,
                   const float* const* weights, const float* const* roots, const int64_t* R, const int64_t* d_in,
                   const int64_t* d_out, void* const* packed, const size_t* packed_bytes_, int threads, rgcn_prep* out) {
  if (numel < 0 || !x_amax || (numel > 0 && !x) || zero_count < 0 || zero_count > kZeroMax ||
      (zero_count > 0 && !zero_buffers) || !out)
    return RGCN_ERR_ARG;
  if (count < 1 || count > kPackJobs || !weights || !roots || !R || !d_in || !d_out || !packed || !packed_bytes_)
    return RGCN_ERR_ARG;
  *out = rgcn_prep{};
  out->J.count = 1;
  out->J.p[0] = x; out->J.n[0] = numel; out->J.out[0] = x_amax;
  out->zero = zero_buffers;
  out->zero_count = zero_count;
  for (int l = 0; l < count; ++l) {
    const int rc = rgcn_pack_layer_check(R[l], d_in[l], d_out[l], 4, weights[l], packed[l], packed_bytes_[l],
                                         packed_bytes(R[l], d_in[l], d_out[l]));
    if (rc != RGCN_OK) return rc;
    out->JJ.j[l] = make_pack_job(weights[l], roots[l], R[l], d_in[l], d_out[l], packed[l], nullptr, nullptr);
  }
  out->pack_blocks = plan_pack_jobs(&out->JJ, count, threads, kPackTiles, kPackCapScan);
  out->layers = count;
  return RGCN_OK;
}

extern "C" {
// ... 11 lines not shown
  }
  for (int t = 0; t < count; ++t) {
    RGCN_ALIGN_TRY(16, tensors[t]);
    RGCN_ALIGN_TRY(4, outs[t]);
  }
  RGCN_ALIGN_TRY(4, zero_buffers);
  k_absmax_multi<<<RGCN_AMAX_HEADS, kScanThreads, 0, (hipStream_t)stream_>>>(J, zero_buffers, zero_count);
  RGCN_HIP_TRY(hipGetLastError());
  return RGCN_OK;
}

int rgcn_absmax_pack(const float* x, int64_t numel, float* x_amax, float* zero_buffers, int zero_count, int count,
                     const float* const* weights, const float* const* roots, const int64_t* R, const int64_t* d_in,
                     const int64_t* d_out, void* const* packed, const size_t* packed_bytes_, void* stream_) {
  rgcn_prep p;
  const int rc = rgcn_prep_fill(x, numel, x_amax, zero_buffers, zero_count, count, weights, roots, R, d_in, d_out, packed,
                                packed_bytes_, kPackThreads, &p);
  if (rc != RGCN_OK) return rc;
  RGCN_ALIGN_TRY(16, x);
  RGCN_ALIGN_TRY(4, x_amax, zero_buffers);
  for (int l = 0; l < count; ++l) RGCN_ALIGN_TRY(16, weights[l], roots[l], packed[l]);
  k_absmax_pack<<<(unsigned)(p.pack_blocks * p.layers + RGCN_AMAX_HEADS), kPackThreads, 0, (hipStream_t)stream_>>>(
      p.J, p.zero, p.zero_count, p.JJ, p.pack_blocks, p.layers);
  RGCN_HIP_TRY(hipGetLastError());
  return RGCN_OK;
}

int rgcn_absmax(const float* x, int64_t n, float* out, float* zero_buffers, int zero_count, void* stream_) {
  return rgcn_absmax_multi(1, &x, &n, &out, zero_buffers, zero_count, stream_);
}

size_t rgcn_weights_split_bytes(int64_t R, int64_t d_in, int64_t d_out) {
  if (R <= 0 || d_in <= 0 || d_out <= 0) return 0;
  return packed_bytes(R, d_in, d_out);
}

int rgcn_weights_split_pack(const float* weight, const float* root, int64_t R, int64_t d_in, int64_t d_out,
                            void* packed, size_t packed_bytes_, void* stream_) {
  const int rc = rgcn_pack_layer_check(R, d_in, d_out, 1, weight, packed, packed_bytes_, packed_bytes(R, d_in, d_out));
  if (rc != RGCN_OK) return rc;
  RGCN_ALIGN_TRY(16, weight, root, packed);
  return pack_weights(weight, root, R, d_in, d_out, packed, (hipStream_t)stream_);
}

int rgcn_weights_split_pack_multi(int count, const float* const* weights, const float* const* roots,
                                  const int64_t* R, const int64_t* d_in, const int64_t* d_out,
                                  const float* const* w_amax, const float* const* r_amax, void* const* packed,
                                  const size_t* packed_bytes_, float* zero_buffers, int zero_count, void* stream_) {
  if (count < 1 || count > kPackJobs || !weights || !roots || !R || !d_in || !d_out || !packed || !packed_bytes_)
    return RGCN_ERR_ARG;
  if (zero_count < 0 || zero_count > kZeroMax || (zero_count > 0 && !zero_buffers)) return RGCN_ERR_ARG;
  pack_jobs JJ{};
  for (int l = 0; l < count; ++l) {
    const int rc = rgcn_pack_layer_check(R[l], d_in[l], d_out[l], 4, weights[l], packed[l], packed_bytes_[l],
                                         packed_bytes(R[l], d_in[l], d_out[l]));
    if (rc != RGCN_OK) return rc;
    JJ.j[l] = make_pack_job(weights[l], roots[l], R[l], d_in[l], d_out[l], packed[l], w_amax ? w_amax[l] : nullptr,
                            r_amax ? r_amax[l] : nullptr);
  }
  for (int l = 0; l < count; ++l) {
    RGCN_ALIGN_TRY(16, weights[l], roots[l], packed[l]);
    RGCN_ALIGN_TRY(4, w_amax ? w_amax[l] : nullptr, r_amax ? r_amax[l] : nullptr);
  }
  RGCN_ALIGN_TRY(4, zero_buffers);
  launch_pack_split(JJ, count, zero_buffers, zero_count, (hipStream_t)stream_);
  RGCN_HIP_TRY(hipGetLastError());
  return RGCN_OK;
}

size_t rgcn_transform_split_workspace_bytes(int64_t R, int64_t d_in, int64_t d_out) {
  if (R <= 0 || d_in <= 0 || d_out <= 0) return 0;
  return nt_workspace_bytes(R, d_in, d_out);
}

int rgcn_transform_fwd_split(const float* agg, const float* x, const float* weight, const float* root,
                             const void* packed, const float* bias, int relu, const uint32_t* tile_mask, int64_t N,
                             int64_t R, int64_t d_in, int64_t d_out, const float* agg_amax, float agg_amax_mul,
                             const float* x_amax, int half, float* out, float* out_amax, void* workspace,
                             size_t workspace_bytes, void* stream_, const rgcn_graph* hub_graph, int hub_transposed,
                             float* hub_partial) {
  if (rgcn_layer_bad_dims(N, R, d_in, d_out) || !out) return RGCN_ERR_ARG;
  if (N == 0) return RGCN_OK;
  if (!agg || !x || !weight || ((half & RGCN_MODE_SPARSE_ROWS) && !tile_mask)) return RGCN_ERR_ARG;
  if (d_in % BK) return RGCN_ERR_UNSUPPORTED;
  if (rgcn_gemm_out_of_range(N, (R + 1) * d_in, d_out)) return RGCN_ERR_UNSUPPORTED;
  nt_call c;
  PackedWeights v;
  const bool aligned = rgcn_aligned(16, agg, x, bias, out) && rgcn_aligned(4, tile_mask, agg_amax, x_amax, out_amax);
  const int rc = nt_prepare(&c, &v, weight, root, packed, N, R, d_in, d_out, d_in, workspace, workspace_bytes, hub_graph,
                            hub_transposed, hub_partial, stream_, aligned);
  if (rc != RGCN_OK) return rc;
  c.A1 = agg; c.a1_amax = agg_amax; c.a1_mul = agg_amax_mul; c.tile_mask = tile_mask;
  if (half & RGCN_MODE_SPARSE_ROWS) c.row_mask = tile_mask + rgcn_row_mask_offset(N);
  c.A2 = x; c.a2_amax = x_amax;
  c.Bh = v.Bh_f; c.Bl = v.Bl_f; c.b_inv = v.inv_scale;
  c.bias = bias; c.epi = relu ? EPI_RELU : EPI_NONE;
  c.C = out; c.N = (int)d_out; c.c_amax = out_amax;
  c.half = (half & 1) != 0;
  return launch_nt_split(c);
}

int rgcn_transform_bwd_input_split(const float* gagg, const float* g, const float* weight, const float* root,
                                   const void* packed, const float* relu_mask, const uint32_t* tile_mask, int64_t N,
                                   int64_t R, int64_t d_in, int64_t d_out, const float* gagg_amax,
                                   float gagg_amax_mul, const float* g_amax, int half, float* grad_x,
                                   float* grad_x_amax, void* workspace, size_t workspace_bytes, void* stream_,
                                   const rgcn_graph* hub_graph, int hub_transposed, float* hub_partial,
                                   float out_scale) {
  if (rgcn_layer_bad_dims(N, R, d_in, d_out) || !grad_x || !(out_scale > 0.f)) return RGCN_ERR_ARG;
  if (N == 0) return RGCN_OK;
  if (!gagg || !g || !weight || ((half & RGCN_MODE_SPARSE_ROWS) && !tile_mask)) return RGCN_ERR_ARG;
  if (d_out % BK) return RGCN_ERR_UNSUPPORTED;
  if (rgcn_gemm_out_of_range(N, (R + 1) * d_out, d_in)) return RGCN_ERR_UNSUPPORTED;
  nt_call c;
  PackedWeights v;
  const bool aligned = rgcn_aligned(16, gagg, g, relu_mask, grad_x) && rgcn_aligned(4, tile_mask, gagg_amax, g_amax, grad_x_amax);
  const int rc = nt_prepare(&c, &v, weight, root, packed, N, R, d_in, d_out, d_out, workspace, workspace_bytes, hub_graph,
                            hub_transposed, hub_partial, stream_, aligned);
  if (rc != RGCN_OK) return rc;
  c.A1 = gagg; c.a1_amax = gagg_amax; c.a1_mul = gagg_amax_mul; c.tile_mask = tile_mask;
  if (half & RGCN_MODE_SPARSE_ROWS) c.row_mask = tile_mask + rgcn_row_mask_offset(N);
  c.A2 = g; c.a2_amax = g_amax;
  c.Bh = v.Bh_b; c.Bl = v.Bl_b; c.b_inv = v.inv_scale;
  c.mask = relu_mask; c.epi = relu_mask ? EPI_MASK : EPI_NONE;
  c.C = grad_x; c.N = (int)d_in; c.c_amax = grad_x_amax; c.out_scale = out_scale;
  c.half = (half & 1) != 0;
  return launch_nt_split(c);
}

int rgcn_transform_bwd_input_chain_supported(int64_t R, int64_t d_in, int64_t d_out, int64_t R1, int64_t d_in1) {
  if (R <= 0 || R1 <= 0 || d_in != 128 || d_out <= 0 || (d_out % BK) || d_in1 <= 0 || (d_in1 & 3)) return 0;
  return 1;
}

int rgcn_transform_bwd_input_chain_split(const float* gagg, const float* g, const float* weight, const float* root,
                                         const void* packed, const float* relu_mask, const uint32_t* tile_mask, int64_t N,
                                         int64_t R, int64_t d_in, int64_t d_out, const float* gagg_amax,
                                         float gagg_amax_mul, const float* g_amax, float* grad_x, float* grad_x_amax,
                                         void* workspace, size_t workspace_bytes, void* stream_,
                                         const rgcn_graph* hub_graph, int hub_transposed, float* hub_partial,
                                         float out_scale, const void* packed1, int has_root1, int64_t R1, int64_t d_in1,
                                         float* t_out) {
  if (rgcn_layer_bad_dims(N, R, d_in, d_out) || !grad_x || !t_out || !packed || !packed1 || !(out_scale > 0.f))
    return RGCN_ERR_ARG;
  if (!rgcn_transform_bwd_input_chain_supported(R, d_in, d_out, R1, d_in1)) return RGCN_ERR_UNSUPPORTED;
  if (N == 0) return RGCN_OK;
  if (!gagg || !g || !weight || !gagg_amax || !g_amax) return RGCN_ERR_ARG;
  const bool sparse = (has_root1 & RGCN_MODE_SPARSE_ROWS) != 0;
  has_root1 &= 1;
  if (sparse && !tile_mask) return RGCN_ERR_ARG;
  if (rgcn_gemm_out_of_range(N, (R + 1) * d_out, (R1 + 1) * d_in1)) return RGCN_ERR_UNSUPPORTED;
  nt_call c;
  PackedWeights v;
  const bool aligned = rgcn_aligned(16, gagg, g, relu_mask, grad_x, packed1, t_out) &&
                       rgcn_aligned(4, tile_mask, gagg_amax, g_amax, grad_x_amax);
  const int rc = nt_prepare(&c, &v, weight, root, packed, N, R, d_in, d_out, d_out, workspace, workspace_bytes, hub_graph,
                            hub_transposed, hub_partial, stream_, aligned);
  if (rc != RGCN_OK) return rc;
  const PackedWeights v1 = packed_view(const_cast<void*>(packed1), R1, d_in1, d_in);
  c.A1 = gagg; c.a1_amax = gagg_amax; c.a1_mul = gagg_amax_mul; c.tile_mask = tile_mask;
  if (sparse) c.row_mask = tile_mask + rgcn_row_mask_offset(N);
  c.A2 = g; c.a2_amax = g_amax;
  c.Bh = v.Bh_b; c.Bl = v.Bl_b; c.b_inv = v.inv_scale;
  c.mask = relu_mask; c.epi = relu_mask ? EPI_MASK : EPI_NONE;
  c.C = grad_x; c.N = (int)d_in; c.c_amax = grad_x_amax; c.out_scale = out_scale;
  c.chained = true;
  c.chain = nt_chain{v1.Bh_n, v1.Bl_n, v1.inv_scale, t_out, (int)((R1 + (has_root1 ? 1 : 0)) * d_in1)};
  return launch_nt_split(c);
}

int rgcn_transform_first_split(const float* g, const void* packed, int has_root, int64_t N, int64_t R, int64_t d_in,
                               int64_t d_out, const float* g_amax, int half, float* t_out, void* workspace,
                               size_t workspace_bytes, void* stream_) {
  if (rgcn_layer_bad_dims(N, R, d_in, d_out) || !t_out || !packed) return RGCN_ERR_ARG;
  if (N == 0) return RGCN_OK;
  if (!g) return RGCN_ERR_ARG;
  if (d_out % BK) return RGCN_ERR_UNSUPPORTED;
  const int64_t cols = (R + (has_root ? 1 : 0)) * d_in;
  if (rgcn_gemm_out_of_range(N, d_out, cols)) return RGCN_ERR_UNSUPPORTED;
  if (!workspace || workspace_bytes < 2 * kMaxSlots * sizeof(float)) return RGCN_ERR_WORKSPACE;
  RGCN_ALIGN_TRY(16, g, packed, t_out, workspace);
  RGCN_ALIGN_TRY(4, g_amax);
  const PackedWeights v = packed_view(const_cast<void*>(packed), R, d_in, d_out);
  nt_call c;
  c.A1 = g; c.K1 = (int)d_out; c.a1_amax = g_amax;
  c.Bh = v.Bh_n; c.Bl = v.Bl_n; c.b_inv = v.inv_scale;
  c.C = t_out; c.M = (int)N; c.N = (int)cols;
  c.scan_slots = (float*)workspace;
  c.half = half != 0;
  c.stream = (hipStream_t)stream_;
  return launch_nt_split(c);
}

size_t rgcn_transform_bwd_params_split_workspace_bytes(int64_t N, int64_t R, int64_t d_in, int64_t d_out) {
  if (N < 0 || R <= 0 || d_in <= 0 || d_out <= 0) return 0;
  const int64_t Kc = (R + 1) * d_in;
  return tn_workspace_bytes(rgcn_slab_layout_of(rgcn_tn_plan(N, Kc, d_out, TN_TKC, kTnBlocks), Kc, d_out));
}

int rgcn_transform_bwd_params_split_begin(const float* agg, const float* x, const float* g,
                                          const uint32_t* tile_mask, int64_t N, int64_t R, int64_t d_in,
                                          int64_t d_out, const float* agg_amax, float agg_amax_mul,
                                          const float* x_amax, const float* g_amax, int half, float* grad_weight,
                                          float* grad_root,
                                          float* grad_bias, void* workspace, size_t workspace_bytes, void* stream_,
                                          rgcn_slab_job* job) {
  const int rc = rgcn_params_begin_check(job, agg, x, g, N, R, d_in, d_out, grad_weight, 64);
  if (rc != RGCN_OK) return rc;
  if ((half & RGCN_MODE_SPARSE_ROWS) && (!tile_mask || !agg_amax)) return RGCN_ERR_ARG;
  rgcn_tn_split p = rgcn_tn_plan(N, (R + 1) * d_in, d_out, TN_TKC, kTnBlocks);
  const rgcn_slab_layout lay = rgcn_slab_layout_of(p, (R + 1) * d_in, d_out);
  if (!workspace || workspace_bytes < tn_workspace_bytes(lay)) return RGCN_ERR_WORKSPACE;
  RGCN_ALIGN_TRY(16, agg, x, g, grad_weight, grad_root, grad_bias, workspace);
  RGCN_ALIGN_TRY(4, tile_mask, agg_amax, x_amax, g_amax);
  hipStream_t stream = (hipStream_t)stream_;
  if (N == 0) return rgcn_zero_param_grads(grad_weight, grad_root, grad_bias, R, d_in, d_out, stream);
  const int K1 = (int)(R * d_in), K2 = grad_root ? (int)d_in : 0, Kc = K1 + K2;
  p.kc_tiles = (int)ceil_div64(Kc, TN_TKC);
  float* slab = (float*)workspace;
  float* bias_part = slab + lay.slab_floats;
  float* slots = (float*)((char*)workspace + align256(lay.bytes()));
  absmax_job J{};
  const bool scan1 = !agg_amax, scan2 = K2 && !x_amax, scang = !g_amax;
  if (scan1) { J.p[0] = agg; J.n[0] = N * (int64_t)K1; }
  if (scan2) { J.p[1] = x; J.n[1] = N * (int64_t)K2; }
  if (scang) { J.p[2] = g; J.n[2] = N * d_out; }
  if (scan1 || scan2 || scang) k_absmax<<<kMaxSlots, kThreads, 0, stream>>>(J, slots);
  const amax_ref r1 = scan1 ? amax_ref{slots, kMaxSlots} : amax_ref{agg_amax, 0};
  const amax_ref r2 = !K2 ? amax_ref{nullptr, 0} : (scan2 ? amax_ref{slots + kMaxSlots, kMaxSlots} : amax_ref{x_amax, 0});
  const amax_ref rg = scang ? amax_ref{slots + 2 * kMaxSlots, kMaxSlots} : amax_ref{g_amax, 0};
  const float a1_mul = (scan1 || !(agg_amax_mul > 0.f)) ? 1.f : agg_amax_mul;
  dim3 grid((unsigned)(p.kc_tiles * p.n_tiles), (unsigned)p.splits);
  const uint32_t* tmask = (d_in % 64 == 0) ? tile_mask : nullptr;
  float* bp = grad_bias ? bias_part : nullptr;
  const uint32_t* rmask = (half & RGCN_MODE_SPARSE_ROWS) ? tile_mask + rgcn_row_mask_offset(N) : nullptr;
#define RGCN_TN_LAUNCH(KERNEL, LO_)                                                                              \
  KERNEL<LO_><<<grid, 2 * kThreads, 0, stream>>>(agg, K1, x, K2, g, (int)N, (int)d_out, p.n_tiles, p.rows_per_split, \
                                                 r1, a1_mul, r2, rg, slab, bp, tmask, (int)d_in, rmask)
  if (half & 1) RGCN_TN_LAUNCH(k_gemm_tn_coop, false);
  else RGCN_TN_LAUNCH(k_gemm_tn_coop, true);
#undef RGCN_TN_LAUNCH
  RGCN_HIP_TRY(hipGetLastError());
  rgcn_slab_job_fill(job, workspace, lay, p.splits, K1, Kc, d_out, grad_weight, grad_root, grad_bias);
  return RGCN_OK;
}

}
```

### primekg_rgcn_linkprediction_amd/ops.py

```python
from __future__ import annotations

import ctypes
import os
import pickle
import time
from collections import OrderedDict
from typing import NamedTuple, Optional, Tuple

import torch

from . import _lib


_raw_stream = getattr(torch._C, "_cuda_getCurrentRawStream", None)
_REC = None


def _empty(*shape, dtype, device) -> torch.Tensor:
    if _REC is None:
        return torch.empty(*shape, dtype=dtype, device=device)
    return _REC.alloc(shape[0] if len(shape) == 1 and isinstance(shape[0], (tuple, list, torch.Size)) else shape, dtype, device)


def _L():
# ... 373 lines not shown
                                                 ctypes.byref(handle))
        _lib.check(rc, "rgcn_graph_create_bipartite")
        self._handle = handle
        return self

    SIDECAR_FORMAT = "rgcn-bucketed-v1"

    def state(self) -> dict:
        if self.bipartite:
            raise ValueError("only whole graphs are persisted, not shard structures")
        fwd, bwd = self.arrays(False), self.arrays(True)
        names = ("rowptr", "col", "perm", "cnt"), ("rowptr_t", "col_t", "perm_t", "w_t")
        out = {"format": self.SIDECAR_FORMAT, "num_edges": self.num_edges, "num_nodes": self.num_nodes,
               "num_relations": self.num_relations}
        for keys, arrs in zip(names, (fwd, bwd)):
            out.update({k: a.cpu() for k, a in zip(keys, arrs)})
        return out

    @classmethod
    def from_state(cls, state: dict, device) -> "BucketedGraph":
        if state.get("format") != cls.SIDECAR_FORMAT:
            raise ValueError(f"not a {cls.SIDECAR_FORMAT} file")
        device = torch.device(device)
        if device.type != "cuda":
            raise RuntimeError("BucketedGraph lives on an MI355X device; no CPU fallback")
        e, n, r = int(state["num_edges"]), int(state["num_nodes"]), int(state["num_relations"])
        want = {"rowptr": (torch.int32, n * r + 1), "col": (torch.int32, e), "perm": (torch.int64, e),
                "cnt": (torch.float32, n * r), "rowptr_t": (torch.int32, n * r + 1), "col_t": (torch.int32, e),
                "perm_t": (torch.int64, e), "w_t": (torch.float32, e)}
        dev = {}
        for k, (dt, size) in want.items():
            t = state[k]
            if t.dtype != dt or t.dim() != 1 or t.numel() != size:
                raise ValueError(f"{k} must be {dt}[{size}], got {t.dtype}{tuple(t.shape)}")
            dev[k] = t.to(device).contiguous()
        self = cls.__new__(cls)
        self._handle = None
        self.device = device
        self.num_nodes, self.num_relations, self.num_other_nodes, self.num_edges = n, r, n, e
        self.bipartite = self.weighted_shard = False
        handle = ctypes.c_void_p()
        with _on(device):
            rc = _L().rgcn_graph_import(e, n, r, *(_ptr(dev[k]) for k in want), _stream(),
                                               ctypes.byref(handle))
        _lib.check(rc, "rgcn_graph_import")
        self._handle = handle
        return self

    def save(self, path) -> None:
        torch.save(self.state(), path)

    @classmethod
    def load(cls, path, device) -> "BucketedGraph":
        return cls.from_state(torch.load(path, weights_only=True), device)

    @property
    def handle(self) -> ctypes.c_void_p:
        if self._handle is None:
            raise RuntimeError("BucketedGraph was destroyed")
        return self._handle

    @property
    def alive(self) -> bool:
        return self._handle is not None

    def tile_mask_ptr(self, transposed: bool) -> Optional[int]:
        if self.bipartite and transposed:
            raise ValueError("a shard structure has one direction only (transposed=False)")
        handle = self.handle
        cache = self.__dict__.setdefault("_mask_ptrs", {})
        if transposed not in cache:
            cache[transposed] = _L().rgcn_graph_tile_mask(handle, int(transposed), None) or None
        return cache[transposed]

    def row_mask_ptr(self, transposed: bool) -> Optional[int]:
        if self.bipartite and transposed:
            raise ValueError("a shard structure has one direction only (transposed=False)")
        handle = self.handle
        cache = self.__dict__.setdefault("_row_mask_ptrs", {})
        if transposed not in cache:
            cache[transposed] = _L().rgcn_graph_row_mask(handle, int(transposed), None) or None
        return cache[transposed]

    def workspace_bytes(self, transposed: bool, d: int) -> int:
        handle = self.handle
        cache = self.__dict__.setdefault("_ws_bytes", {})
        key = (bool(transposed), int(d))
        if key not in cache:
            cache[key] = _L().rgcn_aggregate_workspace_bytes(handle, int(transposed), int(d))
        return cache[key]

    def num_levels(self, transposed: bool) -> int:
        handle = self.handle
        cache = self.__dict__.setdefault("_levels", {})
        if transposed not in cache:
            cache[transposed] = _L().rgcn_graph_num_levels(handle, int(transposed))
        return cache[transposed]

    def deferrable(self, transposed: bool, d: int) -> bool:
        handle = self.handle
        cache = self.__dict__.setdefault("_deferrable", {})
        key = (bool(transposed), int(d))
        if key not in cache:
            cache[key] = bool(_L().rgcn_aggregate_deferrable(handle, int(transposed), int(d)))
        return cache[key]

    def weight_bound(self, transposed: bool) -> float:
        handle = self.handle
        cache = self.__dict__.setdefault("_wbound", {})
        key = bool(transposed and not self.bipartite)
        if key not in cache:
            cache[key] = float(_L().rgcn_graph_weight_bound(handle, int(key)))
        return cache[key]

    def arrays(self, transposed: bool) -> Tuple[torch.Tensor, torch.Tensor, torch.Tensor, torch.Tensor]:
        lib = _L()
        nr, e = self.num_nodes * self.num_relations, self.num_edges
        with _on(self.device):
            rowptr = _empty(nr + 1, dtype=torch.int32, device=self.device)
            col = _empty(e, dtype=torch.int32, device=self.device)
            perm = _empty(e, dtype=torch.int64, device=self.device)
            val = _empty(e if transposed or self.weighted_shard else nr, dtype=torch.float32, device=self.device)
            rc = lib.rgcn_graph_export(self.handle, int(transposed), _ptr(rowptr), _ptr(col), _ptr(perm),
                                       _ptr(val), _stream())
        _lib.check(rc, "rgcn_graph_export")
        return rowptr, col, perm, val

    def row_blocks(self, block_rows: int):
        if self.bipartite:
            raise ValueError("row blocks are cut from a whole graph")
        block_rows = max(32, (int(block_rows) + 31) // 32 * 32)
        cache = self.__dict__.setdefault("_row_blocks", {})
        if block_rows not in cache:
            n, r = self.num_nodes, self.num_relations
            rowptr, col, _, _ = self.arrays(False)
            rp = rowptr.long()
            blocks = []
            for lo in range(0, n, block_rows):
                hi = min(n, lo + block_rows)
                e0, e1 = int(rp[lo * r]), int(rp[hi * r])
                counts = rp[lo * r + 1: hi * r + 1] - rp[lo * r: hi * r]
                seg = torch.repeat_interleave(torch.arange((hi - lo) * r, device=self.device), counts)
                shard = BucketedGraph.from_shard(seg // r, col[e0:e1].long(), seg % r, hi - lo, n, r)
                blocks.append((lo, hi, shard))
            cache[block_rows] = blocks
        return cache[block_rows]

    def fused_plan(self, inline_limit: int = 16, transposed: bool = False) -> "FusedPlan":
        if self.weighted_shard:
            raise ValueError("the fused layer covers whole graphs and mean shards only")
        if transposed and self.bipartite:
            raise ValueError("a shard structure has one direction only (transposed=False)")
        limit = int(inline_limit)
        if not 1 <= limit <= 64:
            raise ValueError("inline_limit must be in [1, 64] (a longer walk is cut into runs by the gather)")
        cache = self.__dict__.setdefault("_fused_plans", {})
        key = (limit, bool(transposed))
        if key not in cache:
            rowptr, col, _, val = self.arrays(transposed)
            weight = val if transposed else None
            rp = rowptr.long()
            lens = rp[1:] - rp[:-1]
            long_seg = lens > limit
            hubs = int(long_seg.sum())
            if hubs == 0:
                cache[key] = FusedPlan(limit, rowptr, col, weight, None, 0, 0)
            else:
                hub_row = torch.cumsum(long_seg.long(), 0) - 1
                seg_of_edge = torch.repeat_interleave(torch.arange(lens.numel(), device=self.device), lens)
                in_hub = long_seg[seg_of_edge]
                hub = BucketedGraph.from_shard(hub_row[seg_of_edge[in_hub]], col[in_hub].long(),
                                               torch.zeros(int(in_hub.sum()), dtype=torch.int64, device=self.device),
                                               hubs, self.num_other_nodes, 1,
                                               edge_weight=weight[in_hub].contiguous() if transposed else None)
                first = torch.zeros_like(in_hub)
                first[rp[:-1][long_seg]] = True
                keep = ~in_hub | first
                new_col = torch.where(in_hub, -(hub_row[seg_of_edge] + 1), col.long())[keep].int()
                new_w = torch.where(in_hub, torch.ones_like(weight), weight)[keep].contiguous() if transposed else None
                new_lens = torch.where(long_seg, torch.ones_like(lens), lens)
                new_rowptr = torch.zeros(lens.numel() + 1, dtype=torch.int64, device=self.device)
                new_rowptr[1:] = torch.cumsum(new_lens, 0)
                cache[key] = FusedPlan(limit, new_rowptr.int(), new_col.contiguous(), new_w, hub, hubs,
                                       int(in_hub.sum()))
        return cache[key]

    def merged_transposed(self) -> Optional["BucketedGraph"]:
        if self.bipartite:
            raise ValueError("a shard structure has no merged form")
        if getattr(self, "_merged", None) is None:
            n, r, e = self.num_nodes, self.num_relations, self.num_edges
            if n * (r + 1) >= 2 ** 31 - 1 or e + n >= 2 ** 31 - 1:
                return None
            rowptr_t, col_t, _, w_t = self.arrays(True)
            counts = (rowptr_t[1:] - rowptr_t[:-1]).long()
            seg = torch.repeat_interleave(torch.arange(n * r, device=self.device), counts)
            nodes = torch.arange(n, device=self.device)
            key = torch.cat([seg // r, nodes])
            other = torch.cat([col_t.long() * (r + 1) + seg % r, nodes * (r + 1) + r])
            weight = torch.cat([w_t, torch.ones(n, device=self.device)])
            self._merged = BucketedGraph.from_shard(key, other, torch.zeros_like(key), n, n * (r + 1), 1, weight)
        return self._merged

    def destroy(self) -> None:
        for memo in ("_regions", "_mask_ptrs", "_row_mask_ptrs"):
            self.__dict__.pop(memo, None)
        for key in [k for k, hit in _GRAPH_CACHE.items() if hit[0] is self]:
            del _GRAPH_CACHE[key]
        merged = getattr(self, "_merged", None)
        if merged is not None:
            merged.destroy()
            self._merged = None
        for blocks in self.__dict__.pop("_row_blocks", {}).values():
            for _, _, shard in blocks:
                shard.destroy()
        for plan in self.__dict__.pop("_fused_plans", {}).values():
            if plan.hub is not None:
                plan.hub.destroy()
        if self._handle is not None:
            try:
                _L().rgcn_graph_destroy(self._handle)
            finally:
                self._handle = None

    def __del__(self):
        try:
            self.destroy()
        except Exception:
            pass


_GRAPH_CACHE: "OrderedDict[tuple, tuple]" = OrderedDict()
_GRAPH_CACHE_SIZE = 8


def _sidecar_matches(g: BucketedGraph, edge_index: torch.Tensor, edge_type: torch.Tensor) -> bool:
    rowptr, col, perm, _ = g.arrays(False)
    e = g.num_edges
    if e == 0:
        return True
    if int(torch.bincount(perm, minlength=e).max()) != 1:
        return False
    seg = edge_index[1].index_select(0, perm) * g.num_relations + edge_type.index_select(0, perm)
    k = torch.arange(e, device=perm.device)
    lo, hi = rowptr[:-1].long().index_select(0, seg), rowptr[1:].long().index_select(0, seg)
    ok = (edge_index[0].index_select(0, perm) == col.long()).all() & ((k >= lo) & (k < hi)).all()
    ok &= (perm[1:] > perm[:-1])[seg[1:] == seg[:-1]].all()
    return bool(ok)


def bucket(edge_index: torch.Tensor, edge_type: torch.Tensor, num_nodes: int,
           num_relations: int, sidecar=None) -> BucketedGraph:
    key = (edge_index.data_ptr(), edge_type.data_ptr(), edge_index._version, edge_type._version,
           tuple(edge_index.shape), int(num_nodes), int(num_relations), str(edge_index.device))
    hit = _GRAPH_CACHE.get(key)
    if hit is not None:
        if hit[0].alive:
            _GRAPH_CACHE.move_to_end(key)
            return hit[0]
        del _GRAPH_CACHE[key]
    g = None
    if sidecar is not None and os.path.exists(sidecar):
        _need_gpu("edge_index", edge_index, torch.int64)
        _need_gpu("edge_type", edge_type, torch.int64)
        try:
            cand = BucketedGraph.load(sidecar, edge_index.device)
            if ((cand.num_edges, cand.num_nodes, cand.num_relations)
                    == (edge_index.size(1), int(num_nodes), int(num_relations))
                    and _sidecar_matches(cand, edge_index, edge_type)):
                g = cand
        except (ValueError, IndexError, KeyError, RuntimeError, EOFError, pickle.UnpicklingError):
            g = None
    if g is None:
        g = BucketedGraph(edge_index, edge_type, num_nodes, num_relations)
        if sidecar is not None:
            g.save(sidecar)
    _GRAPH_CACHE[key] = (g, edge_index, edge_type)
    while len(_GRAPH_CACHE) > _GRAPH_CACHE_SIZE:
        _GRAPH_CACHE.popitem(last=False)
    return g


def clear_graph_cache() -> None:
    _GRAPH_CACHE.clear()


class _EdgeDropoutView(BucketedGraph):

    edge_dropout = True

    def _stale(self, what: str):
        raise ValueError(f"{what} copies edge weights out of the structure when it is built; the weights of an edge-dropout "
                         f"view change with every draw - use the parent graph")

    def state(self) -> dict:
        self._stale("state() / save()")

    def row_blocks(self, block_rows: int):
        self._stale("row_blocks()")

    def fused_plan(self, inline_limit: int = 16, transposed: bool = False):
        self._stale("fused_plan() (the one-kernel layers)")

    def merged_transposed(self):
        self._stale("merged_transposed() (the transform-first input gradient)")

    @property
    def handle(self) -> ctypes.c_void_p:
        if self._handle is None:
            raise RuntimeError("BucketedGraph was destroyed")
        if not self.parent.alive:
            raise RuntimeError("the parent BucketedGraph of this edge-dropout view was destroyed")
        return self._handle

    @property
    def alive(self) -> bool:
        return self._handle is not None and self.parent.alive

    def destroy(self) -> None:
        for memo in ("_regions", "_mask_ptrs", "_row_mask_ptrs"):
            self.__dict__.pop(memo, None)
        self._handle = None

    def __del__(self):
        pass


class EdgeDropout:

    def __init__(self, graph: BucketedGraph):
        self._handle = None
        if not isinstance(graph, BucketedGraph) or graph.bipartite or graph.weighted_shard or graph.edge_dropout:
            raise ValueError("edge dropout views a whole graph (not a shard structure, not another view)")
        handle = ctypes.c_void_p()
        with _on(graph.device):
            rc = _lib.load().rgcn_edge_dropout_create(graph.handle, _stream(), ctypes.byref(handle))
        _lib.check(rc, "rgcn_edge_dropout_create")
        self._handle, self.graph, self.device = handle, graph, graph.device
        view = _EdgeDropoutView.__new__(_EdgeDropoutView)
        view.device = graph.device
        view.num_nodes, view.num_relations, view.num_other_nodes = graph.num_nodes, graph.num_relations, graph.num_nodes
        view.num_edges = graph.num_edges
        view.bipartite, view.weighted_shard = False, True
        view.parent = graph
        view._handle = ctypes.c_void_p(_lib.load().rgcn_edge_dropout_graph(handle))
        self.view = view

    @property
    def handle(self) -> ctypes.c_void_p:
        if self._handle is None:
            raise RuntimeError("EdgeDropout was destroyed")
        if not self.graph.alive:
            raise RuntimeError("the parent BucketedGraph of this EdgeDropout was destroyed")
        return self._handle

    def draw(self, p: float, rng: torch.Tensor, cursor: Optional[torch.Tensor] = None, batch: int = 0,
             position: Optional[torch.Tensor] = None, stats: Optional[torch.Tensor] = None) -> None:
        handle = self.handle
        if not 0.0 <= float(p) < 1.0:
            raise ValueError(f"edge dropout p must be in [0, 1), got {p}")
        for name, t, n in (("rng", rng, 2), ("cursor", cursor, 1), ("position", position, self.graph.num_edges),
                           ("stats", stats, 2)):
            if t is None:
                if name == "rng":
                    raise ValueError("rng (int64[2] = {seed, epoch} on the device) is required")
                continue
            _need_gpu(name, t, torch.int64)
            if t.numel() != n or t.device != self.device:
                raise ValueError(f"{name} must be int64[{n}] on the graph's device")
        if int(batch) < 0:
            raise ValueError("batch must be >= 0")
        with _on(self.device):
            rc = _lib.load().rgcn_edge_dropout_draw(handle, float(p), _ptr(rng), _ptr(cursor), int(batch),
                                                    _ptr(position), _ptr(stats), _stream())
        _lib.check(rc, "rgcn_edge_dropout_draw")

    def kept_counts(self) -> torch.Tensor:
        handle = self.handle
        nr = self.graph.num_nodes * self.graph.num_relations
        with _on(self.device):
            out = _empty(nr, dtype=torch.int32, device=self.device)
            rc = _lib.load().rgcn_edge_dropout_kept_export(handle, _ptr(out), _stream())
        _lib.check(rc, "rgcn_edge_dropout_kept_export")
        return out

    def destroy(self) -> None:
        view = self.__dict__.get("view")
        if view is not None:
            view.destroy()
        if self._handle is not None:
            try:
                _lib.load().rgcn_edge_dropout_destroy(self._handle)
            finally:
                self._handle = None

    def __del__(self):
        try:
            self.destroy()
        except Exception:
            pass


GATHER_EVENTS = None
# ... 211 lines not shown

    def __init__(self, graph: BucketedGraph, transposed: bool, partial: torch.Tensor):
        self.graph, self.transposed, self.partial = graph, bool(transposed), partial


def aggregate_deferred(graph: BucketedGraph, x: torch.Tensor, transposed: bool = False,
                       tail: Optional[PendingParamGrads] = None):
    d = x.size(1) if x.dim() == 2 else 0
    deferrable = (x.dtype == torch.float32 and GATHER_EVENTS is None and graph.num_levels(transposed) == 2
                  and graph.deferrable(transposed, d))
    if not deferrable:
        return aggregate(graph, x, transposed, tail=tail), None
    out, ws = _gather(graph, x, transposed, tail, None, None, levels=(0, 1))
    return out, DeferredHubs(graph, transposed, ws)


def _hub_args(hubs: Optional[DeferredHubs], n: int, r: int):
    if hubs is None:
        return None, 0, None
    if hubs.graph.num_nodes != n or hubs.graph.num_relations != r:
        raise ValueError("hubs do not belong to this aggregate")
    return hubs.graph.handle, int(hubs.transposed), _ptr(hubs.partial)


def _check_layer(agg, x, weight, root, bias):
    _need_gpu("x", x, torch.float32)
    _need_gpu("agg", agg, torch.float32)
    _need_gpu("weight", weight, torch.float32)
    if weight.dim() != 3:
        raise ValueError("weight must be [R, d_in, d_out]")
    r, d_in, d_out = weight.shape
    n = x.size(0)
    if x.dim() != 2 or x.size(1) != d_in:
        raise ValueError(f"x must be [N, {d_in}], got {tuple(x.shape)}")
    if tuple(agg.shape) != (n, r * d_in):
        raise ValueError(f"agg must be [{n}, {r * d_in}], got {tuple(agg.shape)}")
    if root is not None:
        _need_gpu("root", root, torch.float32)
        if tuple(root.shape) != (d_in, d_out):
            raise ValueError(f"root must be [{d_in}, {d_out}]")
    if bias is not None:
        _need_gpu("bias", bias, torch.float32)
        if tuple(bias.shape) != (d_out,):
            raise ValueError(f"bias must be [{d_out}]")
    if d_in % 4 or d_out % 4:
        raise ValueError("in/out channels must be multiples of 4")
    return n, r, d_in, d_out


def _check_bwd_input(gagg, g, weight, root, relu_mask):
    _need_gpu("g", g, torch.float32)
    _need_gpu("gagg", gagg, torch.float32)
    _need_gpu("weight", weight, torch.float32)
    r, d_in, d_out = weight.shape
    n = g.size(0)
    if tuple(g.shape) != (n, d_out) or tuple(gagg.shape) != (n, r * d_out):
        raise ValueError("g must be [N, d_out] and gagg [N, R*d_out]")
    if root is not None:
        _need_gpu("root", root, torch.float32)
    if relu_mask is not None:
        _need_gpu("relu_mask", relu_mask, torch.float32)
        if tuple(relu_mask.shape) != (n, d_in):
            raise ValueError(f"relu_mask must be [{n}, {d_in}]")
    return n, r, d_in, d_out


def _mask_for(graph: Optional[BucketedGraph], transposed: bool, n: int, r: int) -> Optional[int]:
    if graph is None:
        return None
    if graph.num_nodes != n or graph.num_relations != r:
        raise ValueError("graph does not match the operand shapes")
    return graph.tile_mask_ptr(transposed and not graph.bipartite)


def _sparse_bit(sparse: bool, graph: Optional[BucketedGraph], transposed: bool, split, amax) -> int:
    if not sparse:
        return 0
    if not split or graph is None or graph.bipartite or graph.row_mask_ptr(transposed) is None or amax is None:
        raise ValueError("a sparse aggregate needs the split-precision transform, the graph it was gathered over "
                         "(<= 32 relations, not a shard) and the operand's amax buffer (it cannot be scanned)")
    return _lib.MODE_SPARSE_ROWS


def transform_fwd(agg, x, weight, root=None, bias=None, relu: bool = False,
                  graph: Optional[BucketedGraph] = None, half: bool = False, amax=None,
                  amax_out: Optional[torch.Tensor] = None, precision: Optional[str] = None,
                  packed: Optional[SplitWeights] = None, amax_mul: float = 1.0,
                  out: Optional[torch.Tensor] = None, hubs: Optional[DeferredHubs] = None,
                  sparse: bool = False) -> torch.Tensor:
    n, r, d_in, d_out = _check_layer(agg, x, weight, root, bias)
    lib = _L()
    _check_amax("amax_out", amax_out, x.device)
    if out is not None:
        _need_gpu("out", out, torch.float32)
        if tuple(out.shape) != (n, d_out) or out.device != x.device:
            raise ValueError(f"out must be [{n}, {d_out}] on x's device")
    split = 0 if half else _use_split(precision, d_in, 32)
    if not n:
        split = 0
    if split:
        a1, a2 = _pair(amax, 2)
        _check_amax("agg_amax", a1, x.device)
        _check_amax("x_amax", a2, x.device)
        if packed is not None and not packed.matches(weight, root):
            raise ValueError("packed does not belong to these weights")
    elif hubs is not None:
        raise ValueError("deferred hub tails need the split-precision transform (finish them with aggregate instead)")
    mode = _sparse_bit(sparse, graph, False, split, _pair(amax, 2)[0] if split else None)
    k = (r + (root is not None)) * d_in
    with _on(x.device):
        if out is None:
            out = _empty(n, d_out, dtype=torch.float32, device=x.device)
        if split:
            name = "rgcn_transform_fwd_split"
            nbytes = _query("rgcn_transform_split_workspace_bytes", r, d_in, d_out)
            ws = _workspace(nbytes, x.device)
            with _GemmBracket("fwd", n, k, d_out, _split_label(split)):
                rc = lib.rgcn_transform_fwd_split(_ptr(agg), _ptr(x), _ptr(weight), _ptr(root),
                                                  _ptr(packed.buf) if packed is not None else None, _ptr(bias),
                                                  int(relu), _mask_for(graph, False, n, r), n, r, d_in, d_out,
                                                  _ptr(a1), float(amax_mul), _ptr(a2), int(split == 2) | mode, _ptr(out),
                                                  _ptr(amax_out), _ptr(ws), nbytes, _stream(), *_hub_args(hubs, n, r))
        elif half and d_in % 32 == 0:
            name = "rgcn_transform_fwd_f16"
            nbytes = lib.rgcn_transform_fwd_f16_workspace_bytes(r, d_in, d_out)
            ws = _workspace(nbytes, x.device)
            with _GemmBracket("fwd", n, k, d_out, "f16"):
                rc = lib.rgcn_transform_fwd_f16(_ptr(agg), _ptr(x), _ptr(weight), _ptr(root), _ptr(bias), int(relu),
                                                _mask_for(graph, False, n, r), n, r, d_in, d_out, _ptr(out), _ptr(ws),
                                                nbytes, _stream())
        else:
            name = "rgcn_transform_fwd"
            with _GemmBracket("fwd", n, k, d_out, "fp32"):
                rc = lib.rgcn_transform_fwd(_ptr(agg), _ptr(x), _ptr(weight), _ptr(root), _ptr(bias), int(relu),
                                            _mask_for(graph, False, n, r), n, r, d_in, d_out, _ptr(out), _stream())
    _lib.check(rc, name)
    if not split and amax_out is not None:
        absmax(out, amax_out)
    return out


def transform_bwd_input(gagg, g, weight, root=None, relu_mask=None,
                        graph: Optional[BucketedGraph] = None, amax=None, amax_out: Optional[torch.Tensor] = None,
                        precision: Optional[str] = None, packed: Optional[SplitWeights] = None,
                        amax_mul: float = 1.0, hubs: Optional[DeferredHubs] = None,
                        out_scale: float = 1.0, sparse: bool = False) -> torch.Tensor:
    n, r, d_in, d_out = _check_bwd_input(gagg, g, weight, root, relu_mask)
    lib = _L()
    _check_amax("amax_out", amax_out, g.device)
    if d_in % 4 or d_out % 4:
        raise ValueError("in/out channels must be multiples of 4")
    split = _use_split(precision, d_out, 32)
    mode = _sparse_bit(sparse, graph, True, split and n > 0, _pair(amax, 2)[0])
    if split and n > 0:
        a1, a2 = _pair(amax, 2)
        _check_amax("gagg_amax", a1, g.device)
        _check_amax("g_amax", a2, g.device)
        if packed is not None and not packed.matches(weight, root):
            raise ValueError("packed does not belong to these weights")
        with _on(g.device):
            gx = _empty(n, d_in, dtype=torch.float32, device=g.device)
            nbytes = _query("rgcn_transform_split_workspace_bytes", r, d_in, d_out)
            ws = _workspace(nbytes, g.device)
            with _GemmBracket("bwd_input", n, (r + (root is not None)) * d_out, d_in, _split_label(split)):
                rc = lib.rgcn_transform_bwd_input_split(_ptr(gagg), _ptr(g), _ptr(weight), _ptr(root),
                                                        _ptr(packed.buf) if packed is not None else None,
                                                        _ptr(relu_mask), _mask_for(graph, True, n, r), n, r, d_in,
                                                        d_out, _ptr(a1), float(amax_mul), _ptr(a2),
                                                        int(split == 2) | mode, _ptr(gx), _ptr(amax_out), _ptr(ws), nbytes, _stream(),
                                                        *_hub_args(hubs, n, r), float(out_scale))
        _lib.check(rc, "rgcn_transform_bwd_input_split")
        return gx
    if hubs is not None:
        raise ValueError("deferred hub tails need the split-precision transform (finish them with aggregate instead)")
    if out_scale != 1.0:
        weight = weight * out_scale
        root = root * out_scale if root is not None else None
    with _on(g.device):
        gx = _empty(n, d_in, dtype=torch.float32, device=g.device)
        with _GemmBracket("bwd_input", n, (r + (root is not None)) * d_out, d_in, "fp32"):
            rc = lib.rgcn_transform_bwd_input(_ptr(gagg), _ptr(g), _ptr(weight), _ptr(root), _ptr(relu_mask),
                                              _mask_for(graph, True, n, r), n, r, d_in, d_out, _ptr(gx), _stream())
    _lib.check(rc, "rgcn_transform_bwd_input")
    if amax_out is not None:
        absmax(gx, amax_out)
    return gx


def chain_supported(weight: torch.Tensor, weight1: torch.Tensor) -> bool:
    r, d_in, d_out = weight.shape
    r1, d_in1, d_out1 = weight1.shape
    return bool(GEMM_PRECISION == "split" and d_out1 == d_in and
                _query("rgcn_transform_bwd_input_chain_supported", r, d_in, d_out, r1, d_in1))


def transform_bwd_input_chain(gagg, g, weight, root, relu_mask, packed: SplitWeights, packed1: SplitWeights,
                              graph: Optional[BucketedGraph] = None, amax=None, amax_out: Optional[torch.Tensor] = None,
                              amax_mul: float = 1.0, hubs: Optional[DeferredHubs] = None, out_scale: float = 1.0,
                              sparse: bool = False):
    n, r, d_in, d_out = _check_bwd_input(gagg, g, weight, root, relu_mask)
    r1, d_in1, _ = packed1.shape
    if not packed.matches(weight, root) or packed1.shape[2] != d_in:
        raise ValueError("packed / packed1 do not belong to these layers")
    a1, a2 = _pair(amax, 2)
    _check_amax("gagg_amax", a1, g.device)
    _check_amax("g_amax", a2, g.device)
    _check_amax("amax_out", amax_out, g.device)
    if a1 is None or a2 is None:
        raise ValueError("the chained transform needs the operand maxima (amax=)")
    mode = _sparse_bit(sparse, graph, True, True, a1)
    lib = _L()
    cols = (r1 + (1 if packed1.has_root else 0)) * d_in1
    with _on(g.device):
        gz = _empty(n, d_in, dtype=torch.float32, device=g.device)
        t = _empty(n, cols, dtype=torch.float32, device=g.device)
        nbytes = _query("rgcn_transform_split_workspace_bytes", r, d_in, d_out)
        ws = _workspace(nbytes, g.device)
        with _GemmBracket("bwd_input_chain", n, (r + (root is not None)) * d_out + cols, d_in, "split"):
            rc = lib.rgcn_transform_bwd_input_chain_split(_ptr(gagg), _ptr(g), _ptr(weight), _ptr(root), _ptr(packed.buf),
                                                          _ptr(relu_mask), _mask_for(graph, True, n, r), n, r, d_in, d_out,
                                                          _ptr(a1), float(amax_mul), _ptr(a2), _ptr(gz), _ptr(amax_out), _ptr(ws),
                                                          nbytes, _stream(), *_hub_args(hubs, n, r), float(out_scale),
                                                          _ptr(packed1.buf), int(packed1.has_root) | mode, r1, d_in1, _ptr(t))
    _lib.check(rc, "rgcn_transform_bwd_input_chain_split")
    return gz, t


def transform_first(g: torch.Tensor, packed: SplitWeights, amax: Optional[torch.Tensor] = None,
                    precision: Optional[str] = None) -> torch.Tensor:
    _need_gpu("g", g, torch.float32)
    r, d_in, d_out = packed.shape
    if g.dim() != 2 or g.size(1) != d_out or not g.is_contiguous() or g.device != packed.buf.device:
        raise ValueError(f"g must be a contiguous [N, {d_out}] on the weights' device")
    split = _use_split(precision, d_out, 32)
    if not split:
        raise ValueError("transform_first runs in split precision only")
    _check_amax("amax", amax, g.device)
    lib = _L()
    n = g.size(0)
    with _on(g.device):
        t = _empty(n, (r + int(packed.has_root)) * d_in, dtype=torch.float32, device=g.device)
        ws = _workspace(2048, g.device)
        with _GemmBracket("bwd_input", n, d_out, t.size(1), _split_label(split)):
            rc = lib.rgcn_transform_first_split(_ptr(g), _ptr(packed.buf), int(packed.has_root), n, r, d_in, d_out,
                                                _ptr(amax), int(split == 2), _ptr(t), _ptr(ws), 2048, _stream())
    _lib.check(rc, "rgcn_transform_first_split")
    return t


def transform_bwd_params(agg, x, g, num_relations: int, want_root: bool = True, want_bias: bool = True,
                         graph: Optional[BucketedGraph] = None, defer: bool = False, amax=None,
                         precision: Optional[str] = None, amax_mul: float = 1.0, sparse: bool = False):
    _need_gpu("x", x, torch.float32)
    _need_gpu("agg", agg, torch.float32)
    _need_gpu("g", g, torch.float32)
    n, d_in = x.shape
    d_out = g.size(1)
    r = int(num_relations)
    if tuple(agg.shape) != (n, r * d_in) or g.size(0) != n:
        raise ValueError("agg must be [N, R*d_in] and g [N, d_out]")
    lib = _L()
    with _on(x.device):
        gw = _empty(r, d_in, d_out, dtype=torch.float32, device=x.device)
        groot = _empty(d_in, d_out, dtype=torch.float32, device=x.device) if want_root else None
        gbias = _empty(d_out, dtype=torch.float32, device=x.device) if want_bias else None
        split = _use_split(precision, d_in, 64)
        mode = _sparse_bit(sparse, graph, False, split and n > 0, _pair(amax, 3)[0])
        if split and n > 0:
            a1, a2, a3 = _pair(amax, 3)
            for nm, t in (("agg_amax", a1), ("x_amax", a2), ("g_amax", a3)):
                _check_amax(nm, t, x.device)
            nbytes = _query("rgcn_transform_bwd_params_split_workspace_bytes", n, r, d_in, d_out)
            ws = _workspace(nbytes, x.device)
            job = _lib.SlabJob()
            with _GemmBracket("bwd_params", (r + want_root) * d_in, n, d_out, _split_label(split)):
                rc = lib.rgcn_transform_bwd_params_split_begin(_ptr(agg), _ptr(x), _ptr(g),
                                                               _mask_for(graph, False, n, r), n, r, d_in, d_out,
                                                               _ptr(a1), float(amax_mul), _ptr(a2), _ptr(a3),
                                                               int(split == 2) | mode, _ptr(gw), _ptr(groot),
                                                               _ptr(gbias), _ptr(ws), nbytes, _stream(),
                                                               ctypes.byref(job))
            _lib.check(rc, "rgcn_transform_bwd_params_split_begin")
            pending = PendingParamGrads((gw, groot, gbias), job, ws)
            if defer:
                return pending
            pending.finish()
            return gw, groot, gbias
        nbytes = lib.rgcn_transform_bwd_params_workspace_bytes(n, r, d_in, d_out)
        ws = _workspace(nbytes, x.device)
        if defer:
            job = _lib.SlabJob()
            with _GemmBracket("bwd_params", (r + want_root) * d_in, n, d_out, "fp32"):
                rc = lib.rgcn_transform_bwd_params_begin(_ptr(agg), _ptr(x), _ptr(g), _mask_for(graph, False, n, r), n,
# ... 1676 lines not shown
        if timings is not None:
            torch.cuda.synchronize(dev)
            clock.append(time.perf_counter())
            timings[stage] = clock[-1] - clock[-2]

    with _on(dev):
        ids, sqdist = knn(x, k)
        lap("neighbours")
        cond_p, _ = tsne_affinities(sqdist, perplexity)
        rowptr, col, val = tsne_joint(ids, cond_p)
        lap("affinities")
        y = _empty((m, 2), dtype=torch.float32, device=dev)
        if isinstance(init, torch.Tensor):
            y.copy_(init)
        elif init == "pca":
            y.copy_(tsne_pca_init(x))
        else:
            gen = torch.Generator().manual_seed(int(seed))
            y.copy_(torch.randn(m, 2, generator=gen, dtype=torch.float32) * 1e-4)
        lap("init")
        update = _empty((m, 2), dtype=torch.float32, device=dev).zero_()
        gains = _empty((m, 2), dtype=torch.float32, device=dev).fill_(1.0)
        grad = _empty((m, 2), dtype=torch.float32, device=dev)
        z = _empty(1, dtype=torch.float64, device=dev)
        stats = _empty(2, dtype=torch.float64, device=dev).zero_()
        ws = tsne_workspace(m, slices, dev)
        explore = min(TSNE_EXPLORATION_ITERS, max_iter)
        stages = [(explore, float(early_exaggeration), 0.5, TSNE_EXPLORATION_ITERS),
                  (max_iter, 1.0, 0.8, int(n_iter_without_progress))]
        error, norm2, it = float("nan"), float("inf"), 0
        for last, exaggeration, momentum, patience in stages:
            first = it
            best_error, best_iter = float("inf"), first
            for i in range(first, last):
                check = (i + 1) % TSNE_CHECK_EVERY == 0
                want_error = check or i == last - 1
                tsne_gradient(y, rowptr, col, val, exaggeration, slices, want_error, grad, z, stats[0:1], ws)
                tsne_update(grad, y, update, gains, momentum, lr, 0.01, stats[1:2], ws)
                it = i + 1
                if want_error:
                    error, norm2 = stats.cpu().tolist()
                if check:
                    if error < best_error:
                        best_error, best_iter = error, i
                    elif i - best_iter > patience:
                        break
                    if norm2 ** 0.5 <= float(min_grad_norm):
                        break
        lap("iterations")
    return TSNEResult(y, float(error), it)


def distmult_score_all_tails(head: torch.Tensor, rel: torch.Tensor, rel_idx: Optional[torch.Tensor],
                             emb: torch.Tensor):
    _need_gpu("head", head, torch.float32)
    _need_gpu("rel", rel, torch.float32)
    _need_gpu("emb", emb, torch.float32)
    b, d = head.shape
    if emb.dim() != 2 or emb.size(1) != d or rel.dim() != 2 or rel.size(1) != d:
        raise ValueError("head [B, d], rel [R, d], emb [N, d] expected")
    if rel_idx is not None:
        _need_gpu("rel_idx", rel_idx, torch.int64)
        if rel_idx.shape != (b,):
            raise ValueError("rel_idx [B] expected")
    elif rel.size(0) != b:
        raise ValueError("rel must hold one row per head row when no relation ids are given")
    if d % 32:
        raise ValueError("embedding dim must be a multiple of 32 for the score kernel")
    lib = _L()
    with _on(head.device):
        hr = _empty((b, d), dtype=torch.float32, device=head.device)
        scores = _empty((b, emb.size(0)), dtype=torch.float32, device=head.device)
        rc = lib.distmult_score_all_tails(_ptr(head), _ptr(rel), _ptr(rel_idx), rel.size(0), _ptr(emb), b, emb.size(0),
                                          d, _ptr(hr), _ptr(scores), _stream())
    _lib.check(rc, "distmult_score_all_tails")
    return scores, hr


class _NotRecordable(Exception):
    pass


_SEQ_INDEX = {name: i for i, name in enumerate(_lib.SEQ_FUNCTIONS)}
_SEQ_PURE = ("rgcn_graph_tile_mask", "rgcn_graph_row_mask", "rgcn_graph_num_levels", "rgcn_graph_weight_bound", "rgcn_aggregate_deferrable",
             "rgcn_graph_num_edges", "rgcn_graph_num_nodes", "rgcn_graph_num_relations", "rgcn_abi_version", "rgcn_strerror")
REGIONS = True


def guard_torch_op(what: str) -> None:
    if _REC is not None:
        raise _NotRecordable(what)


def _strides(shape):
    st, acc = [], 1
    for n in reversed(shape):
        st.append(acc)
        acc *= n
    return tuple(reversed(st))


def _nbytes(shape, dtype) -> int:
    n = 1
    for s in shape:
        n *= s
    return n * torch.empty((), dtype=dtype).element_size()


class Lazy:
    __slots__ = ("arena", "offset", "shape", "dtype", "_t", "alias")

    def __init__(self, arena, offset, shape, dtype, alias=None):
        self.arena, self.offset, self.shape, self.dtype, self._t, self.alias = arena, offset, shape, dtype, None, alias

    def data_ptr(self) -> int:
        return self.arena.data_ptr() + self.offset

    def tensor(self) -> torch.Tensor:
        if self._t is None:
            if self.dtype == torch.float32 and self.alias is not None and self.offset % 4 == 0:
                self._t = torch.as_strided(self.alias, self.shape, _strides(self.shape), self.offset // 4)
            else:
                nbytes = _nbytes(self.shape, self.dtype)
                self._t = self.arena[self.offset: self.offset + nbytes].view(self.dtype).view(self.shape)
        return self._t


def materialize(t):
    return t.tensor() if isinstance(t, Lazy) else t


def _signature(t):
    if t is None:
        return None
    if isinstance(t, Lazy):
        return (t.dtype, tuple(t.shape), t.arena.get_device())
    return (t.dtype, tuple(t.shape), t.get_device())


def _overlaps(ptrs, sizes) -> tuple:
    spans = sorted((p, p + n, k) for k, (p, n) in enumerate(zip(ptrs, sizes)) if n)
    reach = 0
    for lo, hi, _ in spans:
        if lo < reach:
            break
        reach = hi
    else:
        return ()
    pairs = []
    for a, (_, hi, i) in enumerate(spans):
        for lo, _, j in spans[a + 1:]:
            if lo >= hi:
                break
            pairs.append((i, j, ptrs[j] - ptrs[i]) if i < j else (j, i, ptrs[i] - ptrs[j]))
    return tuple(sorted(pairs))


class _Proxy:
    def __init__(self, rec):
        self._rec, self._real = rec, _lib.load()

    def __getattr__(self, name):
        fn = getattr(self._real, name)
        if name in _SEQ_PURE or name.endswith(("_bytes", "_supported")):
            return fn
        if name not in _SEQ_INDEX:
            raise _NotRecordable(f"{name} is not an entry point the native runner forwards to")
# ... 330 lines not shown
```

Baseline: 7.085 billion edges/s.

## Reorder GEMM rows by relation-occupancy pattern to group similar rows into tiles

Builds, at graph construction, a permutation of node rows sorted by how many relations each row uses and by its occupancy bitmask, plus per-tile occupancy words and hub-finish items re-bucketed by permuted tile. The split-precision NT GEMM kernels for forward, backward-input and the chained backward gather A rows and scatter C rows through this permutation, so each 64-row tile's relation mask is tighter and more K segments can be skipped. It is on by default through RGCN_NT_ROW_ORDER. The cost is indirect, non-contiguous row access for loads and stores, and extra host preprocessing. The diff also adds per-CU stamp recording under the RGCN_STAMPS debug flag.

```diff
diff --git a/include/rgcn_row_order.h b/include/rgcn_row_order.h
--- /dev/null
+++ b/include/rgcn_row_order.h
@@ -0,0 +1,28 @@
+#ifndef RGCN_ROW_ORDER_H
+#define RGCN_ROW_ORDER_H
+
+#include "rgcn_hip.h"
+
+#ifdef __cplusplus
+extern "C" {
+#endif
+
+#define RGCN_MODE_ROW_ORDER 4
+
+typedef struct rgcn_row_order_layout {
+  int64_t padded_rows;
+  int64_t perm, row_words, tile_words, fin_ptr, items;
+  int64_t num_items;
+  int64_t total_words;
+} rgcn_row_order_layout;
+
+const int32_t* rgcn_graph_row_order(const rgcn_graph* g, int transposed, int64_t* padded_rows);
+
+int64_t rgcn_row_order_host(const int32_t* rowptr, int64_t num_rows, int64_t num_relations, uint32_t* words,
+                            rgcn_row_order_layout* layout);
+
+#ifdef __cplusplus
+}
+#endif
+
+#endif
diff --git a/primekg_rgcn_linkprediction_amd/_lib.py b/primekg_rgcn_linkprediction_amd/_lib.py
--- a/primekg_rgcn_linkprediction_amd/_lib.py
+++ b/primekg_rgcn_linkprediction_amd/_lib.py
@@ -232,6 +232,18 @@
 }
 MODE_SPARSE_ROWS = 2
 
+
+class RowOrderLayout(ctypes.Structure):
+    _fields_ = [(name, c_int64) for name in ("padded_rows", "perm", "row_words", "tile_words", "fin_ptr", "items",
+                                              "num_items", "total_words")]
+
+
+ROW_ORDER_PROTOTYPES = {
+    "rgcn_graph_row_order": (c_void_p, [c_void_p, c_int, POINTER(c_int64)]),
+    "rgcn_row_order_host": (_I64, [_P, _I64, _I64, _P, POINTER(RowOrderLayout)]),
+}
+MODE_ROW_ORDER = 4
+
 _lib = None
 
 
@@ -252,7 +264,7 @@
         lib = ctypes.CDLL(LIB_PATH, mode=ctypes.RTLD_GLOBAL)
     except OSError as exc:
         raise RGCNLibraryError(f"cannot load {LIB_PATH}: {exc}") from exc
-    for name, (restype, argtypes) in list(PROTOTYPES.items()) + list(SAMPLING_PROTOTYPES.items()) + list(PATHS_PROTOTYPES.items()) + list(CLUSTER_PROTOTYPES.items()) + list(TSNE_PROTOTYPES.items()) + list(NEIGHBORHOOD_PROTOTYPES.items()) + list(TRANSE_PROTOTYPES.items()) + list(RESAMPLE_PROTOTYPES.items()) + list(COMPLEX_PROTOTYPES.items()) + list(SPARSE_PROTOTYPES.items()) + list(SOFTMAX_PROTOTYPES.items()) + list(EDGE_DROPOUT_PROTOTYPES.items()):
+    for name, (restype, argtypes) in list(PROTOTYPES.items()) + list(SAMPLING_PROTOTYPES.items()) + list(PATHS_PROTOTYPES.items()) + list(CLUSTER_PROTOTYPES.items()) + list(TSNE_PROTOTYPES.items()) + list(NEIGHBORHOOD_PROTOTYPES.items()) + list(TRANSE_PROTOTYPES.items()) + list(RESAMPLE_PROTOTYPES.items()) + list(COMPLEX_PROTOTYPES.items()) + list(SPARSE_PROTOTYPES.items()) + list(ROW_ORDER_PROTOTYPES.items()) + list(SOFTMAX_PROTOTYPES.items()) + list(EDGE_DROPOUT_PROTOTYPES.items()):
         try:
             fn = getattr(lib, name)
         except AttributeError as exc:
diff --git a/primekg_rgcn_linkprediction_amd/conv.py b/primekg_rgcn_linkprediction_amd/conv.py
--- a/primekg_rgcn_linkprediction_amd/conv.py
+++ b/primekg_rgcn_linkprediction_amd/conv.py
@@ -86,6 +86,8 @@
 
 
 _SPARSE_AGG = True
+
+_NT_ROW_ORDER = _os.environ.get("RGCN_NT_ROW_ORDER", "1") != "0"
 
 
 def _sparse_agg(graph: "ops.BucketedGraph", transposed: bool, half: bool, packed, amax, d: int, precision=None) -> bool:
@@ -137,11 +139,12 @@
                     and ops.chain_supported(weight, lower[0])):
                 gx, t = ops.transform_bwd_input_chain(gagg, g, weight, root, relu_mask, packed, lower[2], graph=graph,
                                                       amax=amax, amax_mul=mul, amax_out=amax_out, out_scale=out_scale,
-                                                      sparse=sparse)
+                                                      sparse=sparse, row_order=_NT_ROW_ORDER)
             else:
                 gx = ops.transform_bwd_input(gagg, g, weight, root, relu_mask=relu_mask, graph=graph, amax=amax,
                                              amax_mul=mul, amax_out=amax_out, packed=packed, precision=precision,
-                                             out_scale=out_scale, sparse=sparse)
+                                             out_scale=out_scale, sparse=sparse,
+                                             row_order=_NT_ROW_ORDER)
     return (gx, t) if lower is not None else gx
 
 
@@ -195,7 +198,8 @@
     else:
         agg, hubs = ops.aggregate(graph, _table(x, gather_dtype)), None
     out = ops.transform_fwd(agg, x, weight, root, bias, relu=relu, graph=graph, half=half, amax=(x_amax, x_amax),
-                            amax_out=amax_out, packed=packed, hubs=hubs, sparse=sparse, amax_mul=_agg_bound(graph))
+                            amax_out=amax_out, packed=packed, hubs=hubs, sparse=sparse, amax_mul=_agg_bound(graph),
+                            row_order=_NT_ROW_ORDER)
     return agg, out
 
 
@@ -319,7 +323,8 @@
 
 
 def _policy_key():
-    return (_TRAIN_FUSED, _DEFER_HUBS, _TRANSFORM_FIRST_RATIO, _EVAL_INLINE_LIMIT, _TRAIN_FUSED_MIN_BYTES, _SPARSE_AGG)
+    return (_TRAIN_FUSED, _DEFER_HUBS, _TRANSFORM_FIRST_RATIO, _EVAL_INLINE_LIMIT, _TRAIN_FUSED_MIN_BYTES, _SPARSE_AGG,
+            _NT_ROW_ORDER)
 
 
 def _enc2_train_forward(graph, params, gather_dtype, half_backward: bool, hints, p: float = 0.0):
diff --git a/primekg_rgcn_linkprediction_amd/csrc/rgcn_common.h b/primekg_rgcn_linkprediction_amd/csrc/rgcn_common.h
--- a/primekg_rgcn_linkprediction_amd/csrc/rgcn_common.h
+++ b/primekg_rgcn_linkprediction_amd/csrc/rgcn_common.h
@@ -97,6 +97,57 @@
   }
 }
 
+struct rgcn_order_offsets {
+  int64_t P, perm, rows, tiles, fin, items;
+};
+static inline rgcn_order_offsets rgcn_order_offsets_of(int64_t n_key) {
+  rgcn_order_offsets o;
+  o.P = (n_key + 63) / 64 * 64;
+  const int64_t t32 = o.P / 32;
+  o.perm = (rgcn_occupancy_words(n_key) + 3) / 4 * 4;
+  o.rows = o.perm + o.P;
+  o.tiles = o.rows + o.P;
+  o.fin = o.tiles + (t32 + 3) / 4 * 4;
+  o.items = o.fin + (t32 + 1 + 3) / 4 * 4;
+  return o;
+}
+static inline void rgcn_fill_row_order(int64_t n_key, int64_t R, const rgcn_item* level1, int64_t num_level1,
+                                       std::vector<uint32_t>& words) {
+  const rgcn_order_offsets o = rgcn_order_offsets_of(n_key);
+  const uint32_t* row = words.data() + rgcn_row_mask_offset(n_key);
+  std::vector<uint64_t> key((size_t)n_key);
+  std::vector<int32_t> perm((size_t)n_key), pos((size_t)n_key);
+  for (int64_t i = 0; i < n_key; ++i) {
+    key[(size_t)i] = ((uint64_t)(32 - __builtin_popcount(row[i])) << 32) | row[i];
+    perm[(size_t)i] = (int32_t)i;
+  }
+  std::stable_sort(perm.begin(), perm.end(), [&](int32_t a, int32_t b) { return key[(size_t)a] < key[(size_t)b]; });
+  for (int64_t p = 0; p < n_key; ++p) pos[(size_t)perm[(size_t)p]] = (int32_t)p;
+  words.resize((size_t)(o.items + 4 * num_level1), 0u);
+  row = words.data() + rgcn_row_mask_offset(n_key);
+  for (int64_t p = 0; p < o.P; ++p) {
+    const int32_t src = perm[(size_t)(p < n_key ? p : n_key - 1)];
+    const uint32_t m = p < n_key ? row[src] : 0u;
+    words[(size_t)(o.perm + p)] = (uint32_t)src;
+    words[(size_t)(o.rows + p)] = m;
+    words[(size_t)(o.tiles + (p >> 5))] |= m;
+  }
+  if (num_level1 > 0) {
+    const int64_t t32 = o.P / 32;
+    auto tile_of = [&](const rgcn_item& it) { return (int64_t)(pos[(size_t)(it.dst / R)] >> 5); };
+    std::vector<rgcn_item> items(level1, level1 + num_level1);
+    std::stable_sort(items.begin(), items.end(), [&](const rgcn_item& a, const rgcn_item& b) { return tile_of(a) < tile_of(b); });
+    uint32_t* fin = words.data() + o.fin;
+    for (const rgcn_item& it : items) ++fin[tile_of(it) + 1];
+    for (int64_t t = 0; t < t32; ++t) fin[t + 1] += fin[t];
+    for (int64_t j = 0; j < num_level1; ++j) {
+      const rgcn_item& it = items[(size_t)j];
+      uint32_t* w = words.data() + o.items + 4 * j;
+      w[0] = (uint32_t)it.begin; w[1] = (uint32_t)it.end; w[2] = (uint32_t)it.dst; w[3] = (uint32_t)it.flags;
+    }
+  }
+}
+
 struct rgcn_graph {
   int64_t E = 0, N = 0, R = 0;
   rgcn_csr dir[2];
diff --git a/primekg_rgcn_linkprediction_amd/csrc/rgcn_graph.hip b/primekg_rgcn_linkprediction_amd/csrc/rgcn_graph.hip
--- a/primekg_rgcn_linkprediction_amd/csrc/rgcn_graph.hip
+++ b/primekg_rgcn_linkprediction_amd/csrc/rgcn_graph.hip
@@ -7,6 +7,7 @@
 
 #include "rgcn_common.h"
 #include "../../include/rgcn_sparse.h"
+#include "../../include/rgcn_row_order.h"
 
 namespace {
 
@@ -72,7 +73,7 @@
 
 inline unsigned grid_for(int64_t n) { return (unsigned)std::max<int64_t>(1, ceil_div64(n, kThreads)); }
 
-int build_plan(const std::vector<int32_t>& rowptr, int64_t NR, int64_t R, rgcn_csr* csr) {
+int build_plan(const std::vector<int32_t>& rowptr, int64_t NR, int64_t R, rgcn_csr* csr, std::vector<rgcn_item>* fin_items) {
   rgcn_plan plan;
   const int rc = rgcn_build_plan(rowptr, NR, R, csr->n_key, &plan);
   if (rc != RGCN_OK) return rc;
@@ -100,6 +101,7 @@
     RGCN_HIP_TRY(hipMalloc((void**)&csr->fin_ptr, fin_ptr.size() * sizeof(int32_t)));
     RGCN_HIP_TRY(hipMemcpy(csr->fin_ptr, fin_ptr.data(), fin_ptr.size() * sizeof(int32_t), hipMemcpyHostToDevice));
     csr->num_fin_tiles = (int64_t)fin_ptr.size() - 1;
+    *fin_items = levels[1];
   }
   return RGCN_OK;
 }
@@ -201,14 +203,16 @@
   std::vector<int32_t> rp((size_t)NR + 1);
   RGCN_HIP_TRY(hipMemcpyAsync(rp.data(), c->rowptr, (NR + 1) * sizeof(int32_t), hipMemcpyDeviceToHost, stream));
   RGCN_HIP_TRY(hipStreamSynchronize(stream));
+  std::vector<rgcn_item> fin_items;
+  TRY_PLAN(build_plan(rp, NR, R, c, &fin_items));
   if (R <= 32 && c->n_key > 0) {
     c->num_row_tiles = ceil_div64(c->n_key, 32);
     std::vector<uint32_t> mask((size_t)rgcn_occupancy_words(c->n_key));
     rgcn_fill_occupancy(rp.data(), c->n_key, R, mask.data());
+    rgcn_fill_row_order(c->n_key, R, fin_items.data(), (int64_t)fin_items.size(), mask);
     RGCN_HIP_TRY(hipMalloc((void**)&c->tile_mask, mask.size() * sizeof(uint32_t)));
     RGCN_HIP_TRY(hipMemcpy(c->tile_mask, mask.data(), mask.size() * sizeof(uint32_t), hipMemcpyHostToDevice));
   }
-  TRY_PLAN(build_plan(rp, NR, R, c));
   c->weight_bound = 1.f;
   if (c->weighted && NR > 0 && rp[(size_t)NR] > 0) {
     std::vector<float> w((size_t)rp[(size_t)NR]);
@@ -481,6 +485,38 @@
   return rgcn_occupancy_words(num_rows);
 }
 
+const int32_t* rgcn_graph_row_order(const rgcn_graph* g, int transposed, int64_t* padded_rows) {
+  if (padded_rows) *padded_rows = 0;
+  if (!g) return nullptr;
+  const rgcn_csr* c = &g->dir[transposed ? 1 : 0];
+  if (!c->tile_mask) return nullptr;
+  const rgcn_order_offsets o = rgcn_order_offsets_of(c->n_key);
+  if (padded_rows) *padded_rows = o.P;
+  return reinterpret_cast<const int32_t*>(c->tile_mask + o.perm);
+}
+
+int64_t rgcn_row_order_host(const int32_t* rowptr, int64_t num_rows, int64_t num_relations, uint32_t* words,
+                            rgcn_row_order_layout* layout) {
+  if (layout) *layout = rgcn_row_order_layout{};
+  if (num_rows < 0 || num_relations <= 0 || !rowptr) return -1;
+  if (num_relations > 32 || num_rows == 0) return 0;
+  if (num_rows > INT32_MAX / num_relations) return -1;
+  const int64_t NR = num_rows * num_relations;
+  std::vector<int32_t> rp(rowptr, rowptr + NR + 1);
+  rgcn_plan plan;
+  if (rgcn_build_plan(rp, NR, num_relations, num_rows, &plan) != RGCN_OK) return -1;
+  std::vector<rgcn_item> none;
+  const std::vector<rgcn_item>& level1 = plan.fin_ptr.empty() ? none : plan.levels[1];
+  std::vector<uint32_t> image((size_t)rgcn_occupancy_words(num_rows));
+  rgcn_fill_occupancy(rowptr, num_rows, num_relations, image.data());
+  rgcn_fill_row_order(num_rows, num_relations, level1.data(), (int64_t)level1.size(), image);
+  const rgcn_order_offsets o = rgcn_order_offsets_of(num_rows);
+  if (layout)
+    *layout = rgcn_row_order_layout{o.P, o.perm, o.rows, o.tiles, o.fin, o.items, (int64_t)level1.size(), (int64_t)image.size()};
+  if (words) std::copy(image.begin(), image.end(), words);
+  return (int64_t)image.size();
+}
+
 int rgcn_graph_arrays(const rgcn_graph* g, int transposed, const int32_t** rowptr, const int32_t** col,
                       const int64_t** perm, const float** val) {
   if (!g) return RGCN_ERR_ARG;
diff --git a/primekg_rgcn_linkprediction_amd/csrc/rgcn_transform_split.hip b/primekg_rgcn_linkprediction_amd/csrc/rgcn_transform_split.hip
--- a/primekg_rgcn_linkprediction_amd/csrc/rgcn_transform_split.hip
+++ b/primekg_rgcn_linkprediction_amd/csrc/rgcn_transform_split.hip
@@ -9,12 +9,19 @@
 #include "rgcn_hub_finish.h"
 #include "rgcn_split.h"
 #include "rgcn_transform_host.h"
+#include "../../include/rgcn_row_order.h"
 
 #ifdef RGCN_STAMPS
 __device__ unsigned long long g_rgcn_stamps[8192 * 4];
+__device__ unsigned g_rgcn_stamp_cu[8192];
 #define RGCN_STAMP(i)                                                                                               \
   do {                                                                                                              \
-    if (threadIdx.x == 0) g_rgcn_stamps[((blockIdx.y * gridDim.x + blockIdx.x) & 8191) * 4 + (i)] = __builtin_amdgcn_s_memrealtime(); \
+    if (threadIdx.x == 0) {                                                                                         \
+      const unsigned wg_ = (blockIdx.y * gridDim.x + blockIdx.x) & 8191;                                            \
+      g_rgcn_stamps[wg_ * 4 + (i)] = __builtin_amdgcn_s_memrealtime();                                              \
+      if ((i) == 0)                     \
+        g_rgcn_stamp_cu[wg_] = (__builtin_amdgcn_s_getreg(20 | 31 << 11) << 16) | (__builtin_amdgcn_s_getreg(4 | 31 << 11) & 0xffffu); \
+    }                                                                                                               \
   } while (0)
 #else
 #define RGCN_STAMP(i)
@@ -154,7 +161,7 @@
 
 __device__ __attribute__((aligned(16))) float g_zero_row[128];
 
-template <int WM, int WN, int TN, int EPI, bool LO, bool CHAIN = false>
+template <int WM, int WN, int TN, int EPI, bool LO, bool CHAIN = false, bool ORDER = false>
 __global__ __launch_bounds__(64 * WM * WN) void k_gemm_nt_split(const float* __restrict__ A1, int K1,
                                                             const float* __restrict__ A2, int K2,
                                                             const __half* __restrict__ Bh,
@@ -166,8 +173,10 @@
                                                             int M, int N, const uint32_t* __restrict__ tile_mask,
                                                             int kseg, unsigned* __restrict__ amax_out,
                                                             const hub_fin fin, float out_scale, const nt_chain chain,
-                                                            const uint32_t* __restrict__ row_mask) {
+                                                            const uint32_t* __restrict__ row_mask,
+                                                            const int* __restrict__ row_perm) {
   static_assert(!CHAIN || (WM == 2 && WN == 2 && TN == 2 && LO), "the chained product is built for the 64 x 128 tile");
+  static_assert(!ORDER || WM == 2, "a wave holds the rows of one 64-position tile, one per lane");
   constexpr int WAVES = WM * WN;
   constexpr int BM = 32 * WM, BN = 32 * TN * WN, NBUF = WM == 2 ? 3 : 4, D = NBUF - 1;
   constexpr int PARTS = LO ? 2 : 1;
@@ -196,14 +205,25 @@
       if ((t32 + q) * 32 < M) rel_mask |= tile_mask[t32 + q];
     rel_mask = __builtin_amdgcn_readfirstlane(rel_mask);
   }
+  int pv = 0;
+  if constexpr (ORDER) pv = row_perm[m0 + lane];
+  auto row_at = [&](int m) {
+    if constexpr (ORDER) return __shfl(pv, m - m0);
+    else return m;
+  };
+  auto row_of = [&](const int* rows, int q, int m) {
+    if constexpr (ORDER) return rows[q];
+    else return m;
+  };
   int a_m[A_PW], a_c4[A_PW];
   unsigned a_rm[A_PW];
 #pragma unroll
   for (int j = 0; j < A_PW; ++j) {
     const int row = (wave * A_PW + j) * 8 + (lane >> 3);
-    a_m[j] = min(m0 + row, M - 1);
+    if constexpr (ORDER) a_m[j] = row_at(m0 + row);
+    else a_m[j] = min(m0 + row, M - 1);
     a_c4[j] = ((lane & 7) ^ ((row >> 1) & 7)) * 4;
-    a_rm[j] = row_mask ? row_mask[a_m[j]] : 0xffffffffu;
+    a_rm[j] = row_mask ? row_mask[ORDER ? m0 + row : a_m[j]] : 0xffffffffu;
   }
   const float* a_zero = g_zero_row + (lane & 7) * 4;
   int fin_b = 0, fin_e = 0;
@@ -389,11 +409,16 @@
     const int trow = lane >> 4, tc4 = (lane & 15) * 4;
     const int nq = wn * W + tc4;
     float4 mk4[NV];
+    [[maybe_unused]] int mrow[ORDER ? NV : 1];
+    if constexpr (ORDER) {
+#pragma unroll
+      for (int q = 0; q < NV; ++q) mrow[q] = row_at(m0 + wm * 32 + q * RPR + trow);
+    }
     if (EPI == EPI_MASK) {
 #pragma unroll
       for (int q = 0; q < NV; ++q) {
         const int m = m0 + wm * 32 + q * RPR + trow;
-        mk4[q] = m < M ? *reinterpret_cast<const float4*>(mask + (size_t)m * N + nq) : make_float4(0.f, 0.f, 0.f, 0.f);
+        mk4[q] = m < M ? *reinterpret_cast<const float4*>(mask + (size_t)row_of(mrow, q, m) * N + nq) : make_float4(0.f, 0.f, 0.f, 0.f);
       }
     }
 #pragma unroll
@@ -406,7 +431,7 @@
         v.x = mk4[q].x > 0.f ? v.x : 0.f; v.y = mk4[q].y > 0.f ? v.y : 0.f;
         v.z = mk4[q].z > 0.f ? v.z : 0.f; v.w = mk4[q].w > 0.f ? v.w : 0.f;
       }
-      if (m < M) *reinterpret_cast<float4*>(C + (size_t)m * N + nq) = v;
+      if (m < M) *reinterpret_cast<float4*>(C + (size_t)row_of(mrow, q, m) * N + nq) = v;
       else v = make_float4(0.f, 0.f, 0.f, 0.f);
       cmax = fmaxf(cmax, fmaxf(fmaxf(fabsf(v.x), fabsf(v.y)), fmaxf(fabsf(v.z), fabsf(v.w))));
       *reinterpret_cast<float4*>(tr + (q * RPR + trow) * W + tc4) = v;
@@ -520,13 +545,18 @@
       }
       if (kq == KT2 - 1) {
         const int cb = cb2;
+        [[maybe_unused]] int trows[ORDER ? 16 : 1];
+        if constexpr (ORDER) {
+#pragma unroll
+          for (int q = 0; q < 16; ++q) trows[q] = row_at(m0 + wm * 32 + (q & 3) + 8 * (q >> 2) + 4 * lh);
+        }
 #pragma unroll
         for (int b = 0; b < TN; ++b) {
           const int n = cb * BN + (wn * TN + b) * 32 + li;
 #pragma unroll
           for (int q = 0; q < 16; ++q) {
             const int m = m0 + wm * 32 + (q & 3) + 8 * (q >> 2) + 4 * lh;
-            if (m < M && n < N2) chain.T[(size_t)m * N2 + n] = acc2[b][q] * i2 * ic;
+            if (m < M && n < N2) chain.T[(size_t)row_of(trows, q, m) * N2 + n] = acc2[b][q] * i2 * ic;
             acc2[b][q] = 0.f;
           }
         }
@@ -547,10 +577,15 @@
     float4 bv4 = make_float4(0.f, 0.f, 0.f, 0.f);
     if (bias) bv4 = *reinterpret_cast<const float4*>(bias + nq);
     float4 mk4[NV];
+    [[maybe_unused]] int mrow[ORDER ? NV : 1];
+    if constexpr (ORDER) {
+#pragma unroll
+      for (int q = 0; q < NV; ++q) mrow[q] = row_at(m0 + wm * 32 + q * RPR + trow);
+    }
     if (EPI == EPI_MASK) {
 #pragma unroll
       for (int q = 0; q < NV; ++q)
-        mk4[q] = *reinterpret_cast<const float4*>(mask + (size_t)(m0 + wm * 32 + q * RPR + trow) * N + nq);
+        mk4[q] = *reinterpret_cast<const float4*>(mask + (size_t)row_of(mrow, q, m0 + wm * 32 + q * RPR + trow) * N + nq);
     }
 #pragma unroll
     for (int q = 0; q < NV; ++q) {
@@ -563,9 +598,14 @@
         v.z = mk4[q].z > 0.f ? v.z : 0.f; v.w = mk4[q].w > 0.f ? v.w : 0.f;
       }
       cmax = fmaxf(cmax, fmaxf(fmaxf(fabsf(v.x), fabsf(v.y)), fmaxf(fabsf(v.z), fabsf(v.w))));
-      *reinterpret_cast<float4*>(C + (size_t)(m0 + wm * 32 + q * RPR + trow) * N + nq) = v;
+      *reinterpret_cast<float4*>(C + (size_t)row_of(mrow, q, m0 + wm * 32 + q * RPR + trow) * N + nq) = v;
     }
   } else {
+    [[maybe_unused]] int erows[ORDER ? 16 : 1];
+    if constexpr (ORDER) {
+#pragma unroll
+      for (int r = 0; r < 16; ++r) erows[r] = row_at(m0 + wm * 32 + (r & 3) + 8 * (r >> 2) + 4 * lh);
+    }
 #pragma unroll
     for (int b = 0; b < TN; ++b) {
       const int n = n0 + (wn * TN + b) * 32 + li;
@@ -577,9 +617,9 @@
         if (m < M) {
           float v = acc[b][r] * ia * ib + bv;
           if (EPI == EPI_RELU) v = rgcn_relu(v);
-          if (EPI == EPI_MASK) v = mask[(size_t)m * N + n] > 0.f ? v : 0.f;
+          if (EPI == EPI_MASK) v = mask[(size_t)row_of(erows, r, m) * N + n] > 0.f ? v : 0.f;
           cmax = fmaxf(cmax, fabsf(v));
-          C[(size_t)m * N + n] = v;
+          C[(size_t)row_of(erows, r, m) * N + n] = v;
         }
       }
     }
@@ -970,6 +1010,7 @@
   const uint32_t* tile_mask = nullptr;
   int kseg = 0;
   const uint32_t* row_mask = nullptr;
+  const int* row_perm = nullptr;
   const float *a1_amax = nullptr, *a2_amax = nullptr;
   float a1_mul = 1.f, out_scale = 1.f;
   float* c_amax = nullptr;
@@ -982,12 +1023,29 @@
   amax_ref r1{}, r2{};
 };
 
-template <int TN, int EPI, bool LO, bool CHAIN>
+template <int TN, int EPI, bool LO, bool CHAIN, bool ORDER = false>
 void nt_launch(const nt_call& c) {
   const dim3 grid((unsigned)ceil_div64(c.M, 64), CHAIN ? 1u : (unsigned)ceil_div64(c.N, 64 * TN));
-  k_gemm_nt_split<2, 2, TN, EPI, LO, CHAIN><<<grid, 256, 0, c.stream>>>(
+  k_gemm_nt_split<2, 2, TN, EPI, LO, CHAIN, ORDER><<<grid, 256, 0, c.stream>>>(
       c.A1, c.K1, c.A2, c.K2, c.Bh, c.Bl, c.b_inv, c.r1, c.a1_mul, c.r2, c.bias, c.mask, c.C, c.M, c.N, c.tile_mask, c.kseg,
-      reinterpret_cast<unsigned*>(c.c_amax), c.fin, c.out_scale, CHAIN ? c.chain : nt_chain{}, c.row_mask);
+      reinterpret_cast<unsigned*>(c.c_amax), c.fin, c.out_scale, CHAIN ? c.chain : nt_chain{}, c.row_mask, c.row_perm);
+}
+
+int nt_row_order(nt_call* c, const uint32_t* occupancy, int64_t N, const rgcn_graph* hub_graph, int hub_transposed) {
+  if (c->fin.ptr && hub_graph->dir[hub_transposed ? 1 : 0].tile_mask != occupancy) return RGCN_ERR_ARG;
+  const rgcn_order_offsets o = rgcn_order_offsets_of(N);
+  c->row_perm = reinterpret_cast<const int*>(occupancy + o.perm);
+  c->tile_mask = occupancy + o.tiles;
+  if (c->row_mask) c->row_mask = occupancy + o.rows;
+  if (c->fin.ptr) {
+    c->fin.ptr = reinterpret_cast<const int32_t*>(occupancy + o.fin);
+    c->fin.items = reinterpret_cast<const rgcn_item*>(occupancy + o.items);
+    c->fin.tiles = (int)(o.P / 32);
+  }
+  return RGCN_OK;
+}
+inline bool nt_row_order_bad(int mode, const uint32_t* tile_mask, int64_t R) {
+  return (mode & RGCN_MODE_ROW_ORDER) && (!tile_mask || R > 32);
 }
 
 int launch_nt_split(nt_call c) {
@@ -999,6 +1057,7 @@
   if (fin.ptr && fin.d != 64 && fin.d != 128 && fin.d != 256) return RGCN_ERR_UNSUPPORTED;
   if (fin.ptr && (!c.a1_amax || fin.d != c.kseg)) return RGCN_ERR_ARG;
   if (c.row_mask && (!c.a1_amax || c.kseg <= 0 || c.kseg % BK != 0)) return RGCN_ERR_ARG;
+  if (c.row_perm && c.half) return RGCN_ERR_UNSUPPORTED;
   const int K1 = c.K1, K2 = c.K2;
   if (K1 % BK || K2 % BK || K1 + K2 <= 0) return RGCN_ERR_UNSUPPORTED;
   const bool scan1 = K1 && !c.a1_amax, scan2 = K2 && !c.a2_amax;
@@ -1021,12 +1080,16 @@
   auto plain = [&](auto tn) {
     with_epi([&](auto epi) {
       if (c.half) nt_launch<decltype(tn)::value, decltype(epi)::value, false, false>(c);
+      else if (c.row_perm) nt_launch<decltype(tn)::value, decltype(epi)::value, true, false, true>(c);
       else nt_launch<decltype(tn)::value, decltype(epi)::value, true, false>(c);
     });
   };
   if (c.chained)
     with_epi([&](auto epi) {
-      if constexpr (decltype(epi)::value != EPI_RELU) nt_launch<2, decltype(epi)::value, true, true>(c);
+      if constexpr (decltype(epi)::value != EPI_RELU) {
+        if (c.row_perm) nt_launch<2, decltype(epi)::value, true, true, true>(c);
+        else nt_launch<2, decltype(epi)::value, true, true>(c);
+      }
     });
   else if (c.N <= 64) plain(std::integral_constant<int, 1>{});
   else plain(std::integral_constant<int, 2>{});
@@ -1204,6 +1267,7 @@
   if (rgcn_layer_bad_dims(N, R, d_in, d_out) || !out) return RGCN_ERR_ARG;
   if (N == 0) return RGCN_OK;
   if (!agg || !x || !weight || ((half & RGCN_MODE_SPARSE_ROWS) && !tile_mask)) return RGCN_ERR_ARG;
+  if (nt_row_order_bad(half, tile_mask, R)) return RGCN_ERR_ARG;
   if (d_in % BK) return RGCN_ERR_UNSUPPORTED;
   if (rgcn_gemm_out_of_range(N, (R + 1) * d_in, d_out)) return RGCN_ERR_UNSUPPORTED;
   nt_call c;
@@ -1219,6 +1283,10 @@
   c.bias = bias; c.epi = relu ? EPI_RELU : EPI_NONE;
   c.C = out; c.N = (int)d_out; c.c_amax = out_amax;
   c.half = (half & 1) != 0;
+  if (half & RGCN_MODE_ROW_ORDER) {
+    const int orc = nt_row_order(&c, tile_mask, N, hub_graph, hub_transposed);
+    if (orc != RGCN_OK) return orc;
+  }
   return launch_nt_split(c);
 }
 
@@ -1232,6 +1300,7 @@
   if (rgcn_layer_bad_dims(N, R, d_in, d_out) || !grad_x || !(out_scale > 0.f)) return RGCN_ERR_ARG;
   if (N == 0) return RGCN_OK;
   if (!gagg || !g || !weight || ((half & RGCN_MODE_SPARSE_ROWS) && !tile_mask)) return RGCN_ERR_ARG;
+  if (nt_row_order_bad(half, tile_mask, R)) return RGCN_ERR_ARG;
   if (d_out % BK) return RGCN_ERR_UNSUPPORTED;
   if (rgcn_gemm_out_of_range(N, (R + 1) * d_out, d_in)) return RGCN_ERR_UNSUPPORTED;
   nt_call c;
@@ -1247,6 +1316,10 @@
   c.mask = relu_mask; c.epi = relu_mask ? EPI_MASK : EPI_NONE;
   c.C = grad_x; c.N = (int)d_in; c.c_amax = grad_x_amax; c.out_scale = out_scale;
   c.half = (half & 1) != 0;
+  if (half & RGCN_MODE_ROW_ORDER) {
+    const int orc = nt_row_order(&c, tile_mask, N, hub_graph, hub_transposed);
+    if (orc != RGCN_OK) return orc;
+  }
   return launch_nt_split(c);
 }
 
@@ -1269,6 +1342,8 @@
   if (N == 0) return RGCN_OK;
   if (!gagg || !g || !weight || !gagg_amax || !g_amax) return RGCN_ERR_ARG;
   const bool sparse = (has_root1 & RGCN_MODE_SPARSE_ROWS) != 0;
+  const bool ordered = (has_root1 & RGCN_MODE_ROW_ORDER) != 0;
+  if (nt_row_order_bad(has_root1, tile_mask, R)) return RGCN_ERR_ARG;
   has_root1 &= 1;
   if (sparse && !tile_mask) return RGCN_ERR_ARG;
   if (rgcn_gemm_out_of_range(N, (R + 1) * d_out, (R1 + 1) * d_in1)) return RGCN_ERR_UNSUPPORTED;
@@ -1288,6 +1363,10 @@
   c.C = grad_x; c.N = (int)d_in; c.c_amax = grad_x_amax; c.out_scale = out_scale;
   c.chained = true;
   c.chain = nt_chain{v1.Bh_n, v1.Bl_n, v1.inv_scale, t_out, (int)((R1 + (has_root1 ? 1 : 0)) * d_in1)};
+  if (ordered) {
+    const int orc = nt_row_order(&c, tile_mask, N, hub_graph, hub_transposed);
+    if (orc != RGCN_OK) return orc;
+  }
   return launch_nt_split(c);
 }
 
diff --git a/primekg_rgcn_linkprediction_amd/ops.py b/primekg_rgcn_linkprediction_amd/ops.py
--- a/primekg_rgcn_linkprediction_amd/ops.py
+++ b/primekg_rgcn_linkprediction_amd/ops.py
@@ -479,6 +479,15 @@
             cache[transposed] = _L().rgcn_graph_row_mask(handle, int(transposed), None) or None
         return cache[transposed]
 
+    def row_order_ptr(self, transposed: bool) -> Optional[int]:
+        if self.bipartite and transposed:
+            raise ValueError("a shard structure has one direction only (transposed=False)")
+        handle = self.handle
+        cache = self.__dict__.setdefault("_row_order_ptrs", {})
+        if transposed not in cache:
+            cache[transposed] = _L().rgcn_graph_row_order(handle, int(transposed), None) or None
+        return cache[transposed]
+
     def workspace_bytes(self, transposed: bool, d: int) -> int:
         handle = self.handle
         cache = self.__dict__.setdefault("_ws_bytes", {})
@@ -600,7 +609,7 @@
         return self._merged
 
     def destroy(self) -> None:
-        for memo in ("_regions", "_mask_ptrs", "_row_mask_ptrs"):
+        for memo in ("_regions", "_mask_ptrs", "_row_mask_ptrs", "_row_order_ptrs"):
             self.__dict__.pop(memo, None)
         for key in [k for k, hit in _GRAPH_CACHE.items() if hit[0] is self]:
             del _GRAPH_CACHE[key]
@@ -715,7 +724,7 @@
         return self._handle is not None and self.parent.alive
 
     def destroy(self) -> None:
-        for memo in ("_regions", "_mask_ptrs", "_row_mask_ptrs"):
+        for memo in ("_regions", "_mask_ptrs", "_row_mask_ptrs", "_row_order_ptrs"):
             self.__dict__.pop(memo, None)
         self._handle = None
 
@@ -1093,12 +1102,19 @@
     return _lib.MODE_SPARSE_ROWS
 
 
+def _order_bit(row_order: bool, graph: Optional[BucketedGraph], transposed: bool, split) -> int:
+    if (not row_order or split != 1 or graph is None or graph.bipartite or graph.num_relations > 32
+            or graph.tile_mask_ptr(transposed) is None or graph.row_order_ptr(transposed) is None):
+        return 0
+    return _lib.MODE_ROW_ORDER
+
+
 def transform_fwd(agg, x, weight, root=None, bias=None, relu: bool = False,
                   graph: Optional[BucketedGraph] = None, half: bool = False, amax=None,
                   amax_out: Optional[torch.Tensor] = None, precision: Optional[str] = None,
                   packed: Optional[SplitWeights] = None, amax_mul: float = 1.0,
                   out: Optional[torch.Tensor] = None, hubs: Optional[DeferredHubs] = None,
-                  sparse: bool = False) -> torch.Tensor:
+                  sparse: bool = False, row_order: bool = False) -> torch.Tensor:
     n, r, d_in, d_out = _check_layer(agg, x, weight, root, bias)
     lib = _L()
     _check_amax("amax_out", amax_out, x.device)
@@ -1118,6 +1134,7 @@
     elif hubs is not None:
         raise ValueError("deferred hub tails need the split-precision transform (finish them with aggregate instead)")
     mode = _sparse_bit(sparse, graph, False, split, _pair(amax, 2)[0] if split else None)
+    mode |= _order_bit(row_order, graph, False, split)
     k = (r + (root is not None)) * d_in
     with _on(x.device):
         if out is None:
@@ -1155,7 +1172,7 @@
                         graph: Optional[BucketedGraph] = None, amax=None, amax_out: Optional[torch.Tensor] = None,
                         precision: Optional[str] = None, packed: Optional[SplitWeights] = None,
                         amax_mul: float = 1.0, hubs: Optional[DeferredHubs] = None,
-                        out_scale: float = 1.0, sparse: bool = False) -> torch.Tensor:
+                        out_scale: float = 1.0, sparse: bool = False, row_order: bool = False) -> torch.Tensor:
     n, r, d_in, d_out = _check_bwd_input(gagg, g, weight, root, relu_mask)
     lib = _L()
     _check_amax("amax_out", amax_out, g.device)
@@ -1163,6 +1180,7 @@
         raise ValueError("in/out channels must be multiples of 4")
     split = _use_split(precision, d_out, 32)
     mode = _sparse_bit(sparse, graph, True, split and n > 0, _pair(amax, 2)[0])
+    mode |= _order_bit(row_order, graph, True, split)
     if split and n > 0:
         a1, a2 = _pair(amax, 2)
         _check_amax("gagg_amax", a1, g.device)
@@ -1208,7 +1226,7 @@
 def transform_bwd_input_chain(gagg, g, weight, root, relu_mask, packed: SplitWeights, packed1: SplitWeights,
                               graph: Optional[BucketedGraph] = None, amax=None, amax_out: Optional[torch.Tensor] = None,
                               amax_mul: float = 1.0, hubs: Optional[DeferredHubs] = None, out_scale: float = 1.0,
-                              sparse: bool = False):
+                              sparse: bool = False, row_order: bool = False):
     n, r, d_in, d_out = _check_bwd_input(gagg, g, weight, root, relu_mask)
     r1, d_in1, _ = packed1.shape
     if not packed.matches(weight, root) or packed1.shape[2] != d_in:
@@ -1219,7 +1237,7 @@
     _check_amax("amax_out", amax_out, g.device)
     if a1 is None or a2 is None:
         raise ValueError("the chained transform needs the operand maxima (amax=)")
-    mode = _sparse_bit(sparse, graph, True, True, a1)
+    mode = _sparse_bit(sparse, graph, True, True, a1) | _order_bit(row_order, graph, True, 1)
     lib = _L()
     cols = (r1 + (1 if packed1.has_root else 0)) * d_in1
     with _on(g.device):
@@ -3062,7 +3080,7 @@
 
 
 _SEQ_INDEX = {name: i for i, name in enumerate(_lib.SEQ_FUNCTIONS)}
-_SEQ_PURE = ("rgcn_graph_tile_mask", "rgcn_graph_row_mask", "rgcn_graph_num_levels", "rgcn_graph_weight_bound", "rgcn_aggregate_deferrable",
+_SEQ_PURE = ("rgcn_graph_tile_mask", "rgcn_graph_row_mask", "rgcn_graph_row_order", "rgcn_graph_num_levels", "rgcn_graph_weight_bound", "rgcn_aggregate_deferrable",
              "rgcn_graph_num_edges", "rgcn_graph_num_nodes", "rgcn_graph_num_relations", "rgcn_abi_version", "rgcn_strerror")
 REGIONS = True
 
```

Measured after the change: 7.161 billion edges/s (median of 6 runs). +1.1%, better.
